# 1812598631/Amos-slam

Measured on AMD Instinct MI355X. Metric: front-end frames/sec (ORB extract+match+mask) at 640x480, higher is better.
Workload: dtype u8 (ORB, gate, matcher) + fp32 (mask network); 1 GPU; configs[2]: 640x480 L8 N1000 full front-end: YOLACT-R50 fp32 mask + ORB detect + gate + describe + match; lanes_per_gpu=2, frames_per_launch=64, width=640, height=480, n_features=1000, n_levels=8, ini_th_fast=20, min_th_fast=7, match=frame k vs k-1, N x N best-2, synthetic_stream_seed=stream = rank, frame k seeded 1000*rank+k (amos-slam_amd/synth.py), parallelism=frames sharded 1 ways, one process per GPU, no data-path collective

## Files before the change

amos-slam_amd/__init__.py:

```python
import ctypes as C
import os

import numpy as np

_HERE = os.path.dirname(os.path.abspath(__file__))
LIB_PATH = os.environ.get("AMOS_FRONTEND_LIB", os.path.join(_HERE, "csrc", "libamos_frontend.so"))

KP_DTYPE = np.dtype([("x", "<f4"), ("y", "<f4"), ("size", "<f4"), ("angle", "<f4"),
                     ("response", "<f4"), ("octave", "<i4"), ("class_id", "<i4")])
BEST2_DTYPE = np.dtype([("best_idx", "<i4"), ("best_dist", "<i4"), ("second_idx", "<i4"),
                        ("second_dist", "<i4")])

TH_HIGH, TH_LOW, HISTO_LENGTH = 100, 50, 30

_v, _i, _z, _f, _d, _q, _u = C.c_void_p, C.c_int, C.c_size_t, C.c_float, C.c_double, C.c_longlong, C.c_uint32
PROTOTYPES = {
    "amos_last_error": (C.c_char_p, ()),
    "amos_device_count": (_i, ()),
    "amos_current_device": (_i, ()),
    "amos_build_variant": (C.c_char_p, ()),
    "amos_orb_create": (_i, (_v, _i, _i, _i, _i, _v, _v)),
    "amos_orb_destroy": (None, (_v,)),
    "amos_orb_geometry_probe": (_i, (_v, _i, _i, _i, _i, _v, _v)),
    "amos_orb_tables": (_i, (_v, _v, _v, _v, _v, _v, _v)),
    "amos_orb_tables_host": (_i, (_v, _v, _v, _v, _v, _v, _v)),
    "amos_orb_level_sizes": (_i, (_v, _i, _i, _v, _v)),
    "amos_orb_detect": (_i, (_v, _v, _z, _i, _i)),
    "amos_orb_level_count": (_i, (_v, _i, _i)),
    "amos_orb_level_keypoints": (_i, (_v, _i, _i, _v, _i)),
    "amos_orb_set_level_keypoints": (_i, (_v, _i, _i, _v, _i)),
    "amos_orb_level_layout": (_i, (_v, _v, _v, _v)),
    "amos_orb_fetch_levels": (_i, (_v, _i, _v, _v, _i)),
    "amos_orb_store_levels": (_i, (_v, _i, _v, _v, _i)),
    "amos_orb_gate": (_i, (_v, _v, _z, _v, _z, _v, _i, _v, _i, _v, _i, _v)),
    "amos_orb_closed_mask": (_i, (_v, _v, _z)),
    "amos_orb_describe": (_i, (_v, _v, _v, _i, _v)),
    "amos_orb_extract": (_i, (_v, _v, _z, _i, _i, _v, _v, _i, _v)),
    "amos_orb_level_image": (_i, (_v, _i, _i, _v, _z, _i)),
    "amos_orb_pyramid_images": (_i, (_v, _i, _v, _v, _i)),
    "amos_orb_blurred_image": (_i, (_v, _i, _i, _v, _z)),
    "amos_orb_level_candidates": (_i, (_v, _i, _i, _v, _i)),
    "amos_orb_extract_batch_device": (_i, (_v, _v, _z, _z, _i, _i, _i)),
    "amos_orb_detect_batch_device": (_i, (_v, _v, _z, _z, _i, _i, _i)),
    "amos_orb_gate_batch_device": (_i, (_v, _v, _z, _z)),
    "amos_orb_gate_labels_batch_device": (_i, (_v, _v, _z, _z, _v, _z, _z, _v, _z, _i, _v, _z, _i, _v)),
    "amos_orb_describe_batch_device": (_i, (_v,)),
    "amos_orb_extract_batch_device_color": (_i, (_v, _v, _z, _z, _i, _i, _i, _i, _i)),
    "amos_frame_rgbd_glue_batch_device": (_i, (_v, _v, _i, _f, _z, _z, _f, _f, _f, _f, _f, _v, _v, _v, _v)),
    "amos_frame_stereo_match": (_i, (_v, _v, _f, _f, _v, _v, _i)),
    "amos_frame_stereo_match_batch_device": (_i, (_v, _v, _i, _f, _f, _v, _v, _v, _v)),
    "amos_frame_stereo_match_arrays_device": (_i, (_v, _v, _i, _v, _v, _v, _i, _v, _v, _v, _i, _f, _f, _v, _v, _v, _v)),
    "amos_frame_undistort_batch_device": (_i, (_v, _f, _f, _f, _f, _v, _i, _v)),
    "amos_frame_image_bounds": (_i, (_i, _i, _f, _f, _f, _f, _v, _i, _v)),
    "amos_orb_batch_results_device": (_i, (_v, _v, _v, _v, _v)),
    "amos_orb_batch_fetch": (_i, (_v, _i, _v, _v, _i, _v)),
    "amos_orb_sync": (_i, (_v,)),
    "amos_orb_timing_enable": (_i, (_v, _i)),
    "amos_orb_timing_collect": (_i, (_v, _v, _v)),
    "amos_orb_stream": (_v, (_v,)),
    "amos_match_create": (_i, (_i, _v, _v)),
    "amos_match_destroy": (None, (_v,)),
    "amos_match_sync": (_i, (_v,)),
    "amos_match_stream": (_v, (_v,)),
    "amos_match_distances": (_i, (_v, _v, _i, _v, _i, _v)),
    "amos_match_list_distances": (_i, (_v, _v, _i, _v, _i, _v, _v, _v)),
    "amos_match_list_best2": (_i, (_v, _v, _i, _v, _i, _v, _v, _i, _v)),
    "amos_match_bruteforce_best2": (_i, (_v, _v, _i, _v, _i, _i, _v)),
    "amos_match_set_bruteforce_kernel": (_i, (_v, _i)),
    "amos_match_bruteforce_best2_batch_device": (_i, (_v, _v, _z, _v, _v, _v, _i, _i, _i, _v)),
    "amos_frame_grid_build_batch_device": (_i, (_v, _v, _v, _i, _i, _v, _v)),
    "amos_match_window_best2_batch_device": (_i, (_v, _v, _v)),
    "amos_match_local_points_batch_device": (_i, (_v, _v)),
    "amos_match_local_points": (_i, (_v, _v, _v, _v, _i, _v, _i, _v, _v, _v, _i, _f, _f, _f, _f, _v, _v, _v, _v)),
    "amos_match_motion_model_batch_device": (_i, (_v, _v)),
    "amos_match_motion_model": (_i, (_v, _v, _v, _v, _i, _v, _i, _v, _v, _i, _f, _f, _f, _f, _v, _v, _v, _v)),
    "amos_bow_create": (_i, (_i, _v, _i, _i, _i, _i, _i, _v, _v, _v, _v, _v)),
    "amos_bow_destroy": (None, (_v,)),
    "amos_bow_sync": (_i, (_v,)),
    "amos_bow_stream": (_v, (_v,)),
    "amos_bow_check": (_i, (_i, _i, _i, _i, _i, _v, _v, _v)),
    "amos_bow_transform_batch_device": (_i, (_v, _v, _v, _i, _i, _i, _v, _v, _v, _v, _v, _v, _v, _v, _v, _v)),
    "amos_bow_transform": (_i, (_v, _v, _i, _i, _v, _v, _v, _v, _v, _v, _v, _v)),
    "amos_match_bow_batch_device": (_i, (_v, _v)),
    "amos_match_bow": (_i, (_v, _v, _v, _f, _i, _v, _v)),
    "amos_match_bow_kf_batch_device": (_i, (_v, _v, _f, _i)),
    "amos_match_triangulation_batch_device": (_i, (_v, _v, _v, _v, _v, _i, _i, _i)),
    "amos_match_bow_kf": (_i, (_v, _v, _v, _f, _i, _v, _v)),
    "amos_match_triangulation": (_i, (_v, _v, _v, _i, _v, _v, _v, _i, _i, _i, _v, _v)),
    "amos_match_fuse_batch_device": (_i, (_v, _v)),
    "amos_match_fuse": (_i, (_v, _v, _i, _v, _i, _i, _v, _v, _v, _v, _v, _v, _i, _v, _v, _i, _i, _i, _v, _v, _v, _v, _v)),
    "amos_mask_pre_create": (_i, (_i, _v, _i, _i, _i, _v)),
    "amos_mask_pre_destroy": (None, (_v,)),
    "amos_mask_pre_stream": (_v, (_v,)),
    "amos_mask_preprocess_batch_device": (_i, (_v, _v, _i, _v)),
    "amos_orb_detect_color_with_mask_pre_batch_device": (_i, (_v, _v, _v, _z, _z, _i, _i, _i, _i, _i, _v)),
    "amos_mask_bias_act_device": (_i, (_v, _v, _v, _v, _z, _i, _i)),
    "amos_mask_bias_relu_maxpool_device": (_i, (_v, _v, _v, _v, _i, _i, _i, _i)),
    "amos_mask_stem_weight_floats": (_i, ()),
    "amos_mask_stem_weights_device": (_i, (_v, _v, _q, _q, _q, _q, _v)),
    "amos_mask_stem_device": (_i, (_v, _v, _q, _q, _q, _q, _v, _v, _v, _i, _i, _i)),
    "amos_mask_conv_supported": (_i, (_i, _i, _i, _i, _i, _i)),
    "amos_mask_conv_device": (_i, (_v, _v, _v, _v, _v, _v, _i, _i, _i, _i, _i, _i, _i, _i, _i, _i)),
    "amos_mask_conv_workspace_bytes": (_z, (_i, _i, _i, _i, _i, _i, _i, _i, _i)),
    "amos_mask_conv_ws_device": (_i, (_v, _v, _v, _v, _v, _v, _i, _i, _i, _i, _i, _i, _i, _i, _i, _i, _v, _z)),
    "amos_mask_conv_tile_mode": (_i, (_i,)),
    "amos_mask_conv_kernel_name": (_i, (_i, _i, _i, _i, _i, _i, _i, _i, _i, _v, _i)),
    "amos_mask_conv_chain_supported": (_i, (_i, _i, _i, _i, _i, _i, _i)),
    "amos_mask_conv_chain_device": (_i, (_v, _v, _v, _v, _v, _v, _v, _v, _i, _i, _i, _i, _i, _i, _i)),
    "amos_mask_conv1x1_supported": (_i, (_i, _i, _i)),
    "amos_mask_winograd_supported": (_i, (_i, _i)),
    "amos_mask_winograd_weight_floats": (_z, (_i, _i)),
    "amos_mask_winograd_weights_device": (_i, (_v, _v, _v, _i, _i)),
    "amos_mask_winograd_conv_device": (_i, (_v, _v, _v, _v, _v, _v, _i, _i, _i, _i, _i, _i)),
    "amos_mask_winograd24_weight_floats": (_z, (_i, _i)),
    "amos_mask_winograd24_weights_device": (_i, (_v, _v, _v, _i, _i)),
    "amos_mask_winograd24_conv_device": (_i, (_v, _v, _v, _v, _v, _v, _i, _i, _i, _i, _i, _i)),
    "amos_mask_winograd24_conv_layout_device": (_i, (_v, _v, _v, _v, _v, _v, _i, _i, _i, _i, _i, _i, _i, _i)),
    "amos_mask_winograd24_persistent_mode": (_i, (_i,)),
    "amos_mask_winograd24_narrow_mode": (_i, (_i,)),
    "amos_mask_conv1x1_device": (_i, (_v, _v, _v, _v, _v, _v, _i, _i, _i, _i, _i, _i, _i)),
    "amos_mask_bilinear_nhwc_device": (_i, (_v, _v, _v, _i, _i, _i, _i, _i, _i, _f, _f)),
    "amos_mask_bilinear_nhwc_act_device": (_i, (_v, _v, _v, _i, _i, _i, _i, _i, _i, _f, _f, _i)),
    "amos_mask_bilinear_x2_mode": (_i, (_i,)),
    "amos_mask_nms_column_max_device": (_i, (_v, _v, _v, _i, _i)),
    "amos_mask_class_scores_device": (_i, (_v, _v, _v, _i, _i, _i, _f)),
    "amos_mask_person_mask_device": (_i, (_v, _v, _v, _v, _i, _i, _i, _i, _i, _i)),
    "amos_mask_head_outputs_device": (_i, (_v, _v, _v, _v, _v, _v, _i, _i, _i, _i, _i, _i, _i, _i)),
    "amos_mask_head_outputs_scores_device": (_i, (_v, _v, _v, _v, _v, _v, _v, _f, _i, _i, _i, _i, _i, _i, _i, _i)),
    "amos_mask_topk_rows_device": (_i, (_v, _v, _v, _v, _i, _i, _i)),
    "amos_mask_topk_rows_sparse_device": (_i, (_v, _v, _v, _v, _i, _i, _i, _f)),
    "amos_mask_post_workspace_bytes": (_z, (_i, _i, _i, _i, _i, _i)),
    "amos_mask_person_masks_device": (_i, (_v, _v, _v, _v, _v, _v, _i, _i, _i, _i, _i, _i, _i, _i, _v, _z, _v, _v)),
    "amos_mask_person_masks_scores_device": (_i, (_v, _v, _v, _v, _v, _v, _i, _i, _i, _i, _i, _i, _i, _i, _v, _z, _v, _v)),
    "amos_mask_coef_at_priors_device": (_i, (_v, _v, _v, _v, _v, _v, _i, _i, _v, _v, _v, _i, _i, _i, _i, _v)),
    "amos_mask_person_masks_at_priors_device": (_i, (_v, _v, _v, _v, _v, _v, _v, _v, _i, _i, _i, _v, _v, _v, _v, _i, _i, _i, _i, _i, _i, _i, _i, _v, _z, _v, _v)),
    "amos_mask_person_masks_scores_at_priors_device": (_i, (_v, _v, _v, _v, _v, _v, _v, _v, _i, _i, _i, _v, _v, _v, _v, _i, _i, _i, _i, _i, _i, _i, _i, _v, _z, _v, _v)),
    "amos_mask_candidates_bytes": (_z, (_i, _i, _i)),
    "amos_mask_candidates_reset_device": (_i, (_v, _v, _i, _i)),
    "amos_mask_head_candidates_device": (_i, (_v, _v, _v, _v, _v, _v, _f, _i, _i, _i, _i, _i, _i, _i, _i)),
    "amos_mask_topk_lists_device": (_i, (_v, _v, _v, _i, _v, _v, _i, _i)),
    "amos_mask_person_masks_candidates_device": (_i, (_v, _v, _v, _v, _v, _v, _i, _i, _i, _i, _i, _i, _i, _i, _v, _z, _v, _v)),
    "amos_mask_person_masks_candidates_at_priors_device": (_i, (_v, _v, _v, _v, _v, _v, _v, _v, _i, _i, _i, _v, _v, _v, _v, _i, _i, _i, _i, _i, _i, _i, _i, _v, _z, _v, _v)),
    "amos_slic_center_count": (_i, (_i, _i, _i, _v, _v)),
    "amos_slic_create": (_i, (_i, _v, _i, _i, _i, _v)),
    "amos_slic_destroy": (None, (_v,)),
    "amos_slic_stream": (_v, (_v,)),
    "amos_slic_run": (_i, (_v, _v, _v, _i, _i, _i, _i, _i, _v, _v, _v)),
    "amos_slic_batch_device": (_i, (_v, _v, _v, _i, _i, _i, _i, _i, _i, _v, _v)),
    "amos_cluster_bgr2lab_batch_device": (_i, (_v, _v, _z, _i, _v)),
    "amos_cluster_kmeans_batch_device": (_i, (_v, _v, _i, _i, _i, _u, _i, _v)),
    "amos_cluster_kmeans": (_i, (_v, _v, _i, _i, _u, _i, _v)),
    "amos_flow_check_device": (_i, (_v, _v, _z, _v, _z, _i, _i, _v, _v, _v, _i, _v)),
    "amos_flow_epipolar_device": (_i, (_v, _v, _v, _v, _v, _i, _v)),
    "amos_flow_scene_flow_device": (_i, (_v, _v, _z, _v, _z, _v, _v, _i, _v, _v)),
    "amos_flow_fundamental_score_device": (_i, (_v, _v, _i, _v, _v, _i, _d, _v, _v, _v)),
    "amos_flow_pnp_score_device": (_i, (_v, _v, _i, _v, _v, _i, _d, _d, _d, _d, _d, _v, _v, _v)),
    "amos_lk_create": (_i, (_i, _v, _i, _i, _i, _i, _v)),
    "amos_lk_destroy": (None, (_v,)),
    "amos_lk_stream": (_v, (_v,)),
    "amos_lk_levels": (_i, (_v,)),
    "amos_lk_track_device": (_i, (_v, _v, _z, _v, _z, _v, _i, _i, _d, _f, _v, _v, _v)),
    "amos_corners_create": (_i, (_i, _v, _i, _i, _v)),
    "amos_corners_destroy": (None, (_v,)),
    "amos_corners_stream": (_v, (_v,)),
    "amos_corners_good_features_device": (_i, (_v, _v, _z, _i, _i, _i, _d, _d, _d, _v, _i, _v, _v)),
    "amos_corners_candidate_count": (_i, (_v, _v)),
    "amos_corners_subpix_device": (_i, (_v, _v, _z, _i, _i, _v, _v, _i, _i, _i, _d)),
    "amos_fmat_create": (_i, (_i, _v, _i, _i, _v)),
    "amos_fmat_destroy": (None, (_v,)),
    "amos_fmat_stream": (_v, (_v,)),
    "amos_fmat_ransac_device": (_i, (_v, _i, _v, _v, _v, _v, _v, _d, _d, _i, _v, _v, _v)),
    "amos_fmat_scene_flow_pair_device": (_i, (_v, _v, _v, _v, _v, _v, _v, _v, _v)),
    "amos_fmat_ransac": (_i, (_v, _i, _v, _v, _d, _d, _i, _v, _v, _v)),
    "amos_pnp_create": (_i, (_i, _v, _i, _i, _v)),
    "amos_pnp_destroy": (None, (_v,)),
    "amos_pnp_stream": (_v, (_v,)),
    "amos_pnp_ransac_device": (_i, (_v, _i, _v, _v, _v, _v, _v, _d, _d, _d, _d, _d, _d, _i, _v, _v, _v)),
# ... 130 lines not shown
        n = _check(self.L.amos_orb_level_count(self.h, frame, level), "amos_orb_level_count")
        out = np.zeros(max(n, 1), KP_DTYPE)
        _check(self.L.amos_orb_level_keypoints(self.h, frame, level, _p(out), len(out)), "amos_orb_level_keypoints")
        return out[:n]

    def set_level_keypoints(self, level, kps, frame=0):
        kps = np.ascontiguousarray(kps, KP_DTYPE)
        _check(self.L.amos_orb_set_level_keypoints(self.h, frame, level, _p(kps), len(kps)), "amos_orb_set_level_keypoints")

    def level_candidates(self, level, frame=0, cap=1 << 20):
        out = np.zeros(cap, KP_DTYPE)
        n = _check(self.L.amos_orb_level_candidates(self.h, frame, level, _p(out), cap), "amos_orb_level_candidates")
        return out[:n].copy()

    def level_image(self, level, padded=False, frame=0):
        lw, lh = self.level_sizes(self.shape[1], self.shape[0])
        w, h = int(lw[level]), int(lh[level])
        if padded:
            w, h = w + 38, h + 38
        out = np.zeros((h, w), np.uint8)
        _check(self.L.amos_orb_level_image(self.h, frame, level, _p(out), w, int(padded)), "amos_orb_level_image")
        return out

    def blurred_image(self, level, frame=0):
        lw, lh = self.level_sizes(self.shape[1], self.shape[0])
        out = np.zeros((int(lh[level]), int(lw[level])), np.uint8)
        _check(self.L.amos_orb_blurred_image(self.h, frame, level, _p(out), out.shape[1]), "amos_orb_blurred_image")
        return out

    def gate(self, mask, labels=None, center_ids=None, rm_vector=None):
        mask = np.ascontiguousarray(mask, np.uint8)
        removed = np.zeros(self.capacity + 1, KP_DTYPE)
        nrem = C.c_int(0)
        if labels is not None:
            labels = np.ascontiguousarray(labels, np.float64)
            center_ids = np.ascontiguousarray(center_ids, np.int32)
            rm_vector = np.ascontiguousarray(rm_vector, np.int32)
            rc = self.L.amos_orb_gate(self.h, _p(mask), mask.strides[0], _p(labels), labels.shape[1], _p(center_ids), len(center_ids), _p(rm_vector), len(rm_vector),
                                      _p(removed), len(removed), C.byref(nrem))
        else:
            rc = self.L.amos_orb_gate(self.h, _p(mask), mask.strides[0], None, 0, None, 0, None, 0, _p(removed), len(removed), C.byref(nrem))
        _check(rc, "amos_orb_gate")
        return removed[:nrem.value].copy()

    def closed_mask(self):
        out = np.zeros(self.shape, np.uint8)
        _check(self.L.amos_orb_closed_mask(self.h, _p(out), out.shape[1]), "amos_orb_closed_mask")
        return out

    def describe(self):
        kps = np.zeros(self.capacity + 1, KP_DTYPE)
        desc = np.zeros((self.capacity + 1, 32), np.uint8)
        n = C.c_int(0)
        _check(self.L.amos_orb_describe(self.h, _p(kps), _p(desc), len(kps), C.byref(n)), "amos_orb_describe")
        return kps[:n.value].copy(), desc[:n.value].copy()

    def extract(self, gray):
        gray = np.ascontiguousarray(gray, np.uint8)
        h, w = gray.shape
        self.shape = (h, w)
        kps = np.zeros(self.capacity + 1, KP_DTYPE)
        desc = np.zeros((self.capacity + 1, 32), np.uint8)
        n = C.c_int(0)
        _check(self.L.amos_orb_extract(self.h, _p(gray), gray.strides[0], w, h, _p(kps), _p(desc), len(kps), C.byref(n)), "amos_orb_extract")
        return kps[:n.value].copy(), desc[:n.value].copy()

    def extract_batch_device(self, d_ptr, frame_stride, row_stride, width, height, n_frames):
        self.shape = (height, width)
        _check(self.L.amos_orb_extract_batch_device(self.h, d_ptr, frame_stride, row_stride, width, height, n_frames), "amos_orb_extract_batch_device")

    def detect_batch_device(self, d_ptr, frame_stride, row_stride, width, height, n_frames):
        self.shape = (height, width)
        _check(self.L.amos_orb_detect_batch_device(self.h, d_ptr, frame_stride, row_stride, width, height, n_frames), "amos_orb_detect_batch_device")

    def gate_batch_device(self, d_masks, mask_frame_stride, mask_row_stride):
        _check(self.L.amos_orb_gate_batch_device(self.h, d_masks, mask_frame_stride, mask_row_stride), "amos_orb_gate_batch_device")

    def gate_labels_batch_device(self, d_masks, mask_frame_stride, mask_row_stride, d_labels, label_frame_stride, label_row_stride, d_centers,
                                 centers_frame_stride, n_centers, d_rm, rm_frame_stride, n_rm, d_status):
        _check(self.L.amos_orb_gate_labels_batch_device(self.h, d_masks, mask_frame_stride, mask_row_stride, d_labels, label_frame_stride, label_row_stride,
                                                        d_centers, centers_frame_stride, n_centers, d_rm, rm_frame_stride, n_rm, d_status),
               "amos_orb_gate_labels_batch_device")

    def describe_batch_device(self):
        _check(self.L.amos_orb_describe_batch_device(self.h), "amos_orb_describe_batch_device")

    def extract_batch_device_color(self, d_ptr, frame_stride, row_stride, width, height, n_frames, channels=3, rgb_order=False):
        self.shape = (height, width)
        _check(self.L.amos_orb_extract_batch_device_color(self.h, d_ptr, frame_stride, row_stride, width, height, n_frames, channels, int(rgb_order)),
               "amos_orb_extract_batch_device_color")

    def detect_color_with_mask_pre_batch_device(self, pre, d_ptr, frame_stride, row_stride, width, height, n_frames, d_net_input, channels=3,
                                                rgb_order=False):
        self.shape = (height, width)
        _check(self.L.amos_orb_detect_color_with_mask_pre_batch_device(self.h, pre.h, d_ptr, frame_stride, row_stride, width, height, n_frames, channels,
                                                                       int(rgb_order), d_net_input), "amos_orb_detect_color_with_mask_pre_batch_device")

    def rgbd_glue_batch_device(self, d_depth, depth_is_u16, depth_map_factor, depth_frame_stride, depth_row_stride, mbf, bounds,
                               d_u_right, d_depth_out, d_grid_cell, d_kps_un=None):
        _check(self.L.amos_frame_rgbd_glue_batch_device(self.h, d_depth, int(depth_is_u16), depth_map_factor, depth_frame_stride, depth_row_stride, mbf, bounds[0],
                                                        bounds[1], bounds[2], bounds[3], d_kps_un, d_u_right, d_depth_out, d_grid_cell),
               "amos_frame_rgbd_glue_batch_device")

    def stereo_match_batch_device(self, right, n_pairs, mbf, min_z, d_u_right, d_depth, d_sad=None, d_status=None):
        r = self if right is None else right
        _check(self.L.amos_frame_stereo_match_batch_device(self.h, r.h, n_pairs, mbf, min_z, d_u_right, d_depth, d_sad, d_status),
               "amos_frame_stereo_match_batch_device")

    def stereo_match(self, right, mbf, min_z, n):
        r = self if right is None else right
        ur, dep = np.zeros(max(n, 1), np.float32), np.zeros(max(n, 1), np.float32)
        _check(self.L.amos_frame_stereo_match(self.h, r.h, mbf, min_z, _p(ur), _p(dep), n), "amos_frame_stereo_match")
        return ur[:n], dep[:n]

    def stereo_match_arrays_device(self, right, n_pairs, d_kps_l, d_desc_l, d_counts_l, capacity_l, d_kps_r, d_desc_r, d_counts_r, capacity_r, mbf, min_z,
                                   d_u_right, d_depth, d_sad=None, d_status=None):
        r = self if right is None else right
        _check(self.L.amos_frame_stereo_match_arrays_device(self.h, r.h, n_pairs, d_kps_l, d_desc_l, d_counts_l, capacity_l, d_kps_r, d_desc_r, d_counts_r,
                                                            capacity_r, mbf, min_z, d_u_right, d_depth, d_sad, d_status),
               "amos_frame_stereo_match_arrays_device")

    def undistort_batch_device(self, fx, fy, cx, cy, dist_coef, d_kps_un):
        dc = np.ascontiguousarray(dist_coef, np.float32)
        _check(self.L.amos_frame_undistort_batch_device(self.h, fx, fy, cx, cy, _p(dc), len(dc), d_kps_un), "amos_frame_undistort_batch_device")

    def batch_results_device(self):
        kps, desc, cnt, cap = C.c_void_p(), C.c_void_p(), C.c_void_p(), C.c_int(0)
        _check(self.L.amos_orb_batch_results_device(self.h, C.byref(kps), C.byref(desc), C.byref(cnt), C.byref(cap)), "amos_orb_batch_results_device")
        return kps.value, desc.value, cnt.value, cap.value

    def batch_fetch(self, frame):
        kps = np.zeros(self.capacity + 1, KP_DTYPE)
        desc = np.zeros((self.capacity + 1, 32), np.uint8)
        n = C.c_int(0)
        _check(self.L.amos_orb_batch_fetch(self.h, frame, _p(kps), _p(desc), len(kps), C.byref(n)), "amos_orb_batch_fetch")
        return kps[:n.value].copy(), desc[:n.value].copy()

    def sync(self):
        _check(self.L.amos_orb_sync(self.h), "amos_orb_sync")

    def pyramid_launches(self):
        return self.n_levels - 1

    STAGES = ("import", "pyramid", "fast", "octree", "orient", "blur", "describe")

    def timing_enable(self, max_records):
        _check(self.L.amos_orb_timing_enable(self.h, max_records), "amos_orb_timing_enable")

    def timing_collect(self):
        ms = np.zeros(len(self.STAGES), np.float32)
        n = C.c_int(0)
        _check(self.L.amos_orb_timing_collect(self.h, _p(ms), C.byref(n)), "amos_orb_timing_collect")
        return dict(zip(self.STAGES, ms.tolist())), n.value


SLIC_CENTER_DTYPE = np.dtype([("x", "<i4"), ("y", "<i4"), ("L", "<i4"), ("A", "<i4"), ("B", "<i4"), ("D", "<i4"), ("label", "<i4"), ("id", "<i4")])


class Slic(_Handle):

    _kind = "slic"

    def __init__(self, max_width=640, max_height=480, max_batch=1, device=0, stream=None):
        self._open(device, stream, max_width, max_height, max_batch)

    @staticmethod
    def center_count(width, height, length=5):
        nx, ny = C.c_int(0), C.c_int(0)
        n = lib().amos_slic_center_count(width, height, length, C.byref(nx), C.byref(ny))
        return n, nx.value, ny.value

    def run(self, lab, depth, length=5, m=10, iterations=5):
        lab = np.ascontiguousarray(lab, np.uint8)
        depth = np.ascontiguousarray(depth, np.uint16)
        h, w = depth.shape
        assert lab.shape == (h, w, 3)
        n = self.center_count(w, h, length)[0]
        labels = np.zeros((h, w), np.float64)
        centers = np.zeros(max(n, 1), SLIC_CENTER_DTYPE)
        nc = C.c_int(0)
        _check(self.L.amos_slic_run(self.h, _p(lab), _p(depth), w, h, length, m, iterations, _p(labels), _p(centers), C.byref(nc)), "amos_slic_run")
        return labels, centers[:nc.value]

    def run_batch_device(self, d_lab, d_depth, width, height, n_frames, d_labels, d_centers, length=5, m=10, iterations=5):
        _check(self.L.amos_slic_batch_device(self.h, d_lab, d_depth, width, height, n_frames, length, m, iterations, d_labels, d_centers), "amos_slic_batch_device")

    def bgr2lab_batch_device(self, d_bgr, n_pixels, d_lab, rgb_order=False):
        _check(self.L.amos_cluster_bgr2lab_batch_device(self.h, d_bgr, n_pixels, int(rgb_order), d_lab), "amos_cluster_bgr2lab_batch_device")

    def kmeans(self, centers, k=15, seed=1, max_iter=1000):
        c = np.ascontiguousarray(centers, SLIC_CENTER_DTYPE).copy()
        passes = C.c_int(0)
        _check(self.L.amos_cluster_kmeans(self.h, _p(c), len(c), k, seed, max_iter, C.byref(passes)), "amos_cluster_kmeans")
        return c, passes.value

    def kmeans_batch_device(self, d_centers, n_centers, n_frames, k=15, seed=1, max_iter=1000, d_passes=None):
        _check(self.L.amos_cluster_kmeans_batch_device(self.h, d_centers, n_centers, n_frames, k, seed, max_iter, d_passes), "amos_cluster_kmeans_batch_device")

    def sync(self):
        import torch
        torch.cuda.ExternalStream(self.stream).synchronize()


class MaskPreprocessor(_Handle):

    _kind = "mask_pre"

    def __init__(self, width=640, height=480, max_batch=16, device=0, stream=None):
        self._open(device, stream, width, height, max_batch)
        self.max_batch, self.shape = max_batch, (height, width)

    def run(self, d_bgr, n_frames, d_out):
        _check(self.L.amos_mask_preprocess_batch_device(self.h, d_bgr, n_frames, d_out), "amos_mask_preprocess_batch_device")


def mask_bias_act(stream_ptr, y_ptr, bias_ptr, residual_ptr, n, channels, relu):
    _check(lib().amos_mask_bias_act_device(stream_ptr, y_ptr, bias_ptr, residual_ptr, n, channels, int(relu)), "amos_mask_bias_act_device")


class SceneFlowCamera(C.Structure):
    _fields_ = [("cx", C.c_float), ("cy", C.c_float), ("invfx", C.c_float), ("invfy", C.c_float), ("Tlw", C.c_float * 12), ("Rwc", C.c_float * 9),
                ("Ow", C.c_float * 3)]


def flow_check(stream, d_last, last_stride, d_cur, cur_stride, cols, rows, d_pre, d_next, d_state_in, n, d_state_out):
    _check(lib().amos_flow_check_device(stream, d_last, last_stride, d_cur, cur_stride, cols, rows, d_pre, d_next, d_state_in, n, d_state_out),
           "amos_flow_check_device")


def flow_epipolar(stream, d_F, d_pre, d_next, d_state, n, d_dd):
    _check(lib().amos_flow_epipolar_device(stream, d_F, d_pre, d_next, d_state, n, d_dd), "amos_flow_epipolar_device")


def flow_scene_flow(stream, d_depth_last, last_stride, d_depth_cur, cur_stride, d_match_pre, d_match_cur, n, cam, d_out):
    _check(lib().amos_flow_scene_flow_device(stream, d_depth_last, last_stride, d_depth_cur, cur_stride, d_match_pre, d_match_cur, n, C.byref(cam), d_out),
           "amos_flow_scene_flow_device")


def flow_fundamental_score(stream, d_F, n_hyp, d_p1, d_p2, n, threshold, d_err, d_inliers, d_mask):
    _check(lib().amos_flow_fundamental_score_device(stream, d_F, n_hyp, d_p1, d_p2, n, threshold, d_err, d_inliers, d_mask), "amos_flow_fundamental_score_device")


def flow_pnp_score(stream, d_Rt, n_hyp, d_obj, d_img, n, fx, fy, cx, cy, reprojection_error, d_err, d_inliers, d_mask):
    _check(lib().amos_flow_pnp_score_device(stream, d_Rt, n_hyp, d_obj, d_img, n, fx, fy, cx, cy, reprojection_error, d_err, d_inliers, d_mask),
           "amos_flow_pnp_score_device")


def mask_bias_relu_maxpool(stream_ptr, x_ptr, bias_ptr, y_ptr, n, in_h, in_w, channels):
    _check(lib().amos_mask_bias_relu_maxpool_device(stream_ptr, x_ptr, bias_ptr, y_ptr, n, in_h, in_w, channels), "amos_mask_bias_relu_maxpool_device")


def mask_stem_weight_floats():
    return int(lib().amos_mask_stem_weight_floats())


def mask_stem_weights(stream_ptr, w_ptr, w_strides, packed_ptr):
    sn, sc, sy, sx = (int(v) for v in w_strides)
    _check(lib().amos_mask_stem_weights_device(stream_ptr, w_ptr, sn, sc, sy, sx, packed_ptr), "amos_mask_stem_weights_device")


def mask_stem(stream_ptr, x_ptr, x_strides, packed_ptr, bias_ptr, y_ptr, batch, height, width):
    sb, sc, sy, sx = (int(v) for v in x_strides)
    _check(lib().amos_mask_stem_device(stream_ptr, x_ptr, sb, sc, sy, sx, packed_ptr, bias_ptr, y_ptr, batch, height, width), "amos_mask_stem_device")


def mask_bilinear_x2_mode(mode=-1):
    return int(lib().amos_mask_bilinear_x2_mode(mode))


def mask_conv1x1_supported(cin, cout, stride):
    return lib().amos_mask_conv1x1_supported(cin, cout, stride) == 0


def mask_conv1x1(stream_ptr, x_ptr, w_ptr, bias_ptr, residual_ptr, y_ptr, batch, in_h, in_w, cin, cout, stride, relu):
    _check(lib().amos_mask_conv1x1_device(stream_ptr, x_ptr, w_ptr, bias_ptr, residual_ptr, y_ptr, batch, in_h, in_w, cin, cout, stride, int(relu)),
           "amos_mask_conv1x1_device")


def mask_conv_supported(cin, cout, kh, kw, stride, pad):
    return lib().amos_mask_conv_supported(cin, cout, kh, kw, stride, pad) == 0


def mask_winograd_supported(cin, cout):
    return lib().amos_mask_winograd_supported(cin, cout) == 0


def mask_winograd_weights(stream_ptr, w_ptr, u_ptr, cin, cout):
    _check(lib().amos_mask_winograd_weights_device(stream_ptr, w_ptr, u_ptr, cin, cout), "amos_mask_winograd_weights_device")


def mask_winograd_conv(stream_ptr, x_ptr, u_ptr, bias_ptr, residual_ptr, y_ptr, batch, h, w, cin, cout, relu):
    _check(lib().amos_mask_winograd_conv_device(stream_ptr, x_ptr, u_ptr, bias_ptr, residual_ptr, y_ptr, batch, h, w, cin, cout, int(relu)),
           "amos_mask_winograd_conv_device")


def mask_winograd24_weights(stream_ptr, w_ptr, u_ptr, cin, cout):
    _check(lib().amos_mask_winograd24_weights_device(stream_ptr, w_ptr, u_ptr, cin, cout), "amos_mask_winograd24_weights_device")


def mask_winograd24_conv(stream_ptr, x_ptr, u_ptr, bias_ptr, residual_ptr, y_ptr, batch, h, w, cin, cout, relu):
    _check(lib().amos_mask_winograd24_conv_device(stream_ptr, x_ptr, u_ptr, bias_ptr, residual_ptr, y_ptr, batch, h, w, cin, cout, int(relu)),
           "amos_mask_winograd24_conv_device")


def mask_winograd24_conv_layout(stream_ptr, x_ptr, u_ptr, bias_ptr, residual_ptr, y_ptr, batch, h, w, cin, cout, relu, in_blocked, out_blocked):
    _check(lib().amos_mask_winograd24_conv_layout_device(stream_ptr, x_ptr, u_ptr, bias_ptr, residual_ptr, y_ptr, batch, h, w, cin, cout, int(relu), int(in_blocked),
                                                         int(out_blocked)), "amos_mask_winograd24_conv_layout_device")


def mask_winograd24_persistent_mode(mode=-2):
    return int(lib().amos_mask_winograd24_persistent_mode(mode))


def mask_winograd24_narrow_mode(mode=-2):
    return int(lib().amos_mask_winograd24_narrow_mode(mode))


def mask_conv_tile_mode(mode=-2):
    return int(lib().amos_mask_conv_tile_mode(mode))


def mask_conv_kernel_name(batch, in_h, in_w, cin, cout, kh, kw, stride, pad):
    buf = C.create_string_buffer(96)
    _check(lib().amos_mask_conv_kernel_name(batch, in_h, in_w, cin, cout, kh, kw, stride, pad, buf, 96), "amos_mask_conv_kernel_name")
    return buf.value.decode()


def mask_conv(stream_ptr, x_ptr, w_ptr, bias_ptr, residual_ptr, y_ptr, batch, in_h, in_w, cin, cout, kh, kw, stride, pad, relu):
    _check(lib().amos_mask_conv_device(stream_ptr, x_ptr, w_ptr, bias_ptr, residual_ptr, y_ptr, batch, in_h, in_w, cin, cout, kh, kw, stride, pad, int(relu)),
           "amos_mask_conv_device")


def mask_conv_chain_supported(batch, in_h, in_w, cin, planes, cout, stride):
    return lib().amos_mask_conv_chain_supported(batch, in_h, in_w, cin, planes, cout, stride) == 0


def mask_conv_chain(stream_ptr, x_ptr, wd_ptr, bd_ptr, yc_ptr, w3_ptr, b3_ptr, y_ptr, batch, in_h, in_w, cin, planes, cout, stride):
    _check(lib().amos_mask_conv_chain_device(stream_ptr, x_ptr, wd_ptr, bd_ptr, yc_ptr, w3_ptr, b3_ptr, y_ptr, batch, in_h, in_w, cin, planes, cout, stride),
           "amos_mask_conv_chain_device")


def mask_conv_workspace_bytes(batch, in_h, in_w, cin, cout, kh, kw, stride, pad):
    return int(lib().amos_mask_conv_workspace_bytes(batch, in_h, in_w, cin, cout, kh, kw, stride, pad))


def mask_conv_ws(stream_ptr, x_ptr, w_ptr, bias_ptr, residual_ptr, y_ptr, batch, in_h, in_w, cin, cout, kh, kw, stride, pad, relu, workspace_ptr, workspace_bytes):
# ... 695 lines not shown
```

amos-slam_amd/csrc/amos_common.h:

```cpp
#pragma once
#include <hip/hip_runtime.h>
#include <stdint.h>
#include <stdio.h>
#include <atomic>
#include <string>

#include "../../include/amos_frontend.h"

namespace amos {

void set_error(const char *fmt, ...);

#define AMOS_HIP_CHECK(expr)                                                                   \
    do {                                                                                       \
        hipError_t _e = (expr);                                                                \
        if (_e != hipSuccess) {                                                                \
            amos::set_error("%s failed: %s (%s:%d)", #expr, hipGetErrorString(_e), __FILE__,   \
                            __LINE__);                                                         \
            (void)hipGetLastError();  \
            return AMOS_ERR_DEVICE;                                                            \
        }                                                                                      \
    } while (0)

struct DeviceOnce {
// ... 61 lines not shown
    int w, h;
    int stride;
    int planeOff;
    int maxBX, maxBY;
    int nCols, nRows, wCell, hCell;
    int cellStart, nCells;
    int ptsOff, ptsCap;
    int quota;
    int nIni;
    int nodeCap;
    int kpOff;
    int tabX, tabY;
    int blurGroups, blurItemStart;
    float scale;
    float patchSize;
};

struct Geom {
    int nLevels;
    int W, H;
    int totalCells;
    int slotTotal;
    int ptsTotal;
    int kpLevelTotal;
    int kpCap;
    int iniTh, minTh;
    int blurItems;
    int fastTileStrideDw, fastTileRows, fastMapRows, fastKeptCap, fastWaveBytes;
    unsigned long long frameBytes;
    LevelGeom lv[AMOS_MAX_LEVELS];
};

struct Cell {
    short level;
    short x0, y0;
    short tw, th;
    short ndw;
    int slotOff;
    unsigned magicDw, magicG;
    short groups;
    short pad[3];
};

struct ResizeTap {
    short ofs;
    short ofs1;
    short a0, a1;
};

constexpr int kMaskMidW = 480, kMaskMidH = 640;
struct FixTap { int s0, s1, a0, a1; };
struct MaskPreStageA {
    const FixTap *tx, *ty;
    const int *firstX, *firstY;
    const float *lut;
    float *mid;
    int width, height, maxBatch;
};

}

struct amos_mask_pre;
namespace amos {
struct OrbStereoView {
    int device;
    hipStream_t stream;
    hipEvent_t event;
    amos_orb_params p;
    int width, height, nFrames;
    bool detected, described;
    const Geom *dGeom;
    const uint8_t *dPyr;
    unsigned long long frameBytes;
    const amos_keypoint *dKps;
    const uint8_t *dDesc;
    const int *dCounts;
    int capacity;
    const float *scale, *invScale;
    int *dSadScratch;
    float *dOutHostForm;
    uint8_t *hStage;
};
int orb_stereo_view(amos_orb *h, size_t sadScratchInts, OrbStereoView *out);
int mask_pre_stage_a(amos_mask_pre *p, MaskPreStageA *out);
int mask_pre_finish(amos_mask_pre *p, hipStream_t stream, int n_frames, float *d_out);
const char *w24_variant_tag();
}
```

amos-slam_amd/csrc/amos_mask_pre.hip:

```cpp
#include "amos_common.h"

#include <cmath>
#include <vector>

namespace amos {

constexpr int kNetSize = 550;
constexpr int kMidW = kMaskMidW, kMidH = kMaskMidH;
constexpr int kBackW = 640, kBackH = 480;

struct FltTap { int s0, s1; float f0, f1; };

__global__ __launch_bounds__(256) void k_mask_pre_a(const uint8_t *__restrict__ bgr, int srcW, int srcH, const FixTap *__restrict__ tx,
                                                   const FixTap *__restrict__ ty, const float *__restrict__ lut, float *__restrict__ mid)
{
    const int p = blockIdx.x * 256 + threadIdx.x, frame = blockIdx.y;
    if (p >= kMidW * kMidH) return;
    const int y = p / kMidW, x = p - y * kMidW;
    const FixTap ax = tx[x], ay = ty[y];
    const uint8_t *r0 = bgr + ((size_t)frame * srcH + ay.s0) * srcW * 3, *r1 = bgr + ((size_t)frame * srcH + ay.s1) * srcW * 3;
    float *o = mid + ((size_t)frame * kMidH * kMidW + p) * 3;
#pragma unroll
    for (int c = 0; c < 3; c++) {
        const int h0 = r0[ax.s0 * 3 + c] * ax.a0 + r0[ax.s1 * 3 + c] * ax.a1;
        const int h1 = r1[ax.s0 * 3 + c] * ax.a0 + r1[ax.s1 * 3 + c] * ax.a1;
        const int v = (((ay.a0 * (h0 >> 4)) >> 16) + ((ay.a1 * (h1 >> 4)) >> 16) + 2) >> 2;
        o[c] = lut[v];
    }
}

__global__ __launch_bounds__(256) void k_mask_pre_b(const float *__restrict__ mid, const FltTap *__restrict__ tx, const FltTap *__restrict__ ty,
                                                   float *__restrict__ back)
{
    const int p = blockIdx.x * 256 + threadIdx.x, frame = blockIdx.y;
    if (p >= kBackW * kBackH) return;
    const int y = p / kBackW, x = p - y * kBackW;
    const FltTap ax = tx[x], ay = ty[y];
    const float *r0 = mid + ((size_t)frame * kMidH + ay.s0) * kMidW * 3, *r1 = mid + ((size_t)frame * kMidH + ay.s1) * kMidW * 3;
    float *o = back + ((size_t)frame * kBackH * kBackW + p) * 3;
#pragma unroll
    for (int c = 0; c < 3; c++) {
        const float h0 = __fadd_rn(__fmul_rn(r0[ax.s0 * 3 + c], ax.f0), __fmul_rn(r0[ax.s1 * 3 + c], ax.f1));
        const float h1 = __fadd_rn(__fmul_rn(r1[ax.s0 * 3 + c], ax.f0), __fmul_rn(r1[ax.s1 * 3 + c], ax.f1));
        o[c] = __fadd_rn(__fmul_rn(h0, ay.f0), __fmul_rn(h1, ay.f1));
    }
}

__global__ __launch_bounds__(256) void k_mask_pre_c(const float *__restrict__ back, float *__restrict__ out)
{
    const int p = blockIdx.x * 256 + threadIdx.x, frame = blockIdx.y;
    if (p >= kNetSize * kNetSize) return;
    const int oy = p / kNetSize, ox = p - oy * kNetSize;
    const float sh = (float)kBackH / (float)kNetSize, sw = (float)kBackW / (float)kNetSize;
    const float hr = fmaxf(__fsub_rn(__fmul_rn(sh, __fadd_rn((float)oy, 0.5f)), 0.5f), 0.f);
    const float wr = fmaxf(__fsub_rn(__fmul_rn(sw, __fadd_rn((float)ox, 0.5f)), 0.5f), 0.f);
    const int h1 = (int)hr, w1 = (int)wr;
    const int h1p = h1 < kBackH - 1 ? 1 : 0, w1p = w1 < kBackW - 1 ? 1 : 0;
    const float hl1 = __fsub_rn(hr, (float)h1), hl0 = __fsub_rn(1.f, hl1);
    const float wl1 = __fsub_rn(wr, (float)w1), wl0 = __fsub_rn(1.f, wl1);
    const float *b = back + (size_t)frame * kBackH * kBackW * 3;
    const float *p00 = b + ((size_t)h1 * kBackW + w1) * 3, *p01 = p00 + w1p * 3, *p10 = p00 + (size_t)h1p * kBackW * 3, *p11 = p10 + w1p * 3;
    const float mean[3] = {103.94f, 116.78f, 123.68f}, stdv[3] = {57.38f, 57.12f, 58.40f};
    float *o = out + (size_t)frame * 3 * kNetSize * kNetSize + p;
#pragma unroll
    for (int c = 0; c < 3; c++) {
        const float top = __fadd_rn(__fmul_rn(wl0, p00[c]), __fmul_rn(wl1, p01[c]));
        const float bot = __fadd_rn(__fmul_rn(wl0, p10[c]), __fmul_rn(wl1, p11[c]));
        const float v = __fadd_rn(__fmul_rn(hl0, top), __fmul_rn(hl1, bot));
        o[(size_t)(2 - c) * kNetSize * kNetSize] = __fdiv_rn(__fsub_rn(v, mean[c]), stdv[c]);
    }
}


template <bool kVec, bool kPow2>
__global__ __launch_bounds__(256) void k_bias_act(float *__restrict__ y, const float *__restrict__ bias, const float *__restrict__ res, size_t n,
                                                 int channels, int relu)
{
    const size_t i = ((size_t)blockIdx.x * 256 + threadIdx.x) * 4;
    if (i >= n) return;
    if (kVec) {
        const unsigned c = kPow2 ? ((unsigned)i & (unsigned)(channels - 1)) : (unsigned)(i % (size_t)channels);
        float4 v = *reinterpret_cast<const float4 *>(y + i);
        const float4 b = *reinterpret_cast<const float4 *>(bias + c);
        v.x = __fadd_rn(v.x, b.x); v.y = __fadd_rn(v.y, b.y); v.z = __fadd_rn(v.z, b.z); v.w = __fadd_rn(v.w, b.w);
        if (res) {
            const float4 r = *reinterpret_cast<const float4 *>(res + i);
            v.x = __fadd_rn(v.x, r.x); v.y = __fadd_rn(v.y, r.y); v.z = __fadd_rn(v.z, r.z); v.w = __fadd_rn(v.w, r.w);
        }
        if (relu) { v.x = fmaxf(v.x, 0.f); v.y = fmaxf(v.y, 0.f); v.z = fmaxf(v.z, 0.f); v.w = fmaxf(v.w, 0.f); }
        *reinterpret_cast<float4 *>(y + i) = v;
    } else {
        for (size_t k = i; k < n && k < i + 4; k++) {
            float v = __fadd_rn(y[k], bias[k % (size_t)channels]);
            if (res) v = __fadd_rn(v, res[k]);
            y[k] = relu ? fmaxf(v, 0.f) : v;
        }
    }
}

template <bool kRelu>
__global__ __launch_bounds__(256) void k_bilinear_nhwc_x2(const float *__restrict__ x, float *__restrict__ y, int inH, int inW, int outH, int outW, int c4,
                                                         float scaleH, float scaleW)
{
    const int t = blockIdx.x * 256 + threadIdx.x, bw = (outW + 1) / 2, bh = (outH + 1) / 2, perRow = bw * c4;
    if (t >= bh * perRow) return;
    const int by = t / perRow, tr = t - by * perRow;
    const int bx = tr / c4, q = tr - bx * c4, n = blockIdx.z;
    int yy[2][2], xx[2][2];
    float wy[2][2], wx[2][2];
#pragma unroll
    for (int e = 0; e < 2; e++) {
        float fy = __fsub_rn(__fmul_rn(scaleH, __fadd_rn((float)(2 * by + e), 0.5f)), 0.5f);
        float fx = __fsub_rn(__fmul_rn(scaleW, __fadd_rn((float)(2 * bx + e), 0.5f)), 0.5f);
        fy = fy < 0.f ? 0.f : fy;
        fx = fx < 0.f ? 0.f : fx;
        yy[e][0] = min((int)fy, inH - 1);
        xx[e][0] = min((int)fx, inW - 1);
        yy[e][1] = yy[e][0] + (yy[e][0] < inH - 1 ? 1 : 0);
        xx[e][1] = xx[e][0] + (xx[e][0] < inW - 1 ? 1 : 0);
        wy[e][1] = __fsub_rn(fy, (float)(int)fy); wy[e][0] = __fsub_rn(1.f, wy[e][1]);
        wx[e][1] = __fsub_rn(fx, (float)(int)fx); wx[e][0] = __fsub_rn(1.f, wx[e][1]);
    }
    const float4 *src = reinterpret_cast<const float4 *>(x) + (size_t)n * inH * inW * c4;
    auto at = [&](int r, int c) { return src[((size_t)r * inW + c) * c4 + q]; };
    float4 s[4][4];
    const bool shareY = yy[1][0] == yy[0][1], shareX = xx[1][0] == xx[0][1];
    const int ry[4] = {yy[0][0], yy[0][1], yy[1][0], yy[1][1]}, cx[4] = {xx[0][0], xx[0][1], xx[1][0], xx[1][1]};
#pragma unroll
    for (int r = 0; r < 4; r++) {
        if (r == 2 && shareY) {
#pragma unroll
            for (int c = 0; c < 4; c++) s[2][c] = s[1][c];
            continue;
        }
#pragma unroll
        for (int c = 0; c < 4; c++) {
            if (c == 2 && shareX) s[r][2] = s[r][1];
            else s[r][c] = at(ry[r], cx[c]);
        }
    }
    float4 *dst = reinterpret_cast<float4 *>(y);
#pragma unroll
    for (int ey = 0; ey < 2; ey++)
#pragma unroll
        for (int ex = 0; ex < 2; ex++) {
            const int oy = 2 * by + ey, ox = 2 * bx + ex;
            if (oy >= outH || ox >= outW) continue;
            const float hy = wy[ey][0], ly = wy[ey][1], hx = wx[ex][0], lx = wx[ex][1];
            const float4 a = s[2 * ey][2 * ex], b = s[2 * ey][2 * ex + 1], c = s[2 * ey + 1][2 * ex], d = s[2 * ey + 1][2 * ex + 1];
            auto mix = [&](float p, float r, float u, float v2) {
                const float v = __fadd_rn(__fmul_rn(hy, __fadd_rn(__fmul_rn(hx, p), __fmul_rn(lx, r))), __fmul_rn(ly, __fadd_rn(__fmul_rn(hx, u), __fmul_rn(lx, v2))));
                return kRelu ? (v < 0.f ? 0.f : v) : v;
// ... 29 lines not shown
    float4 r = {fmaxf(__fadd_rn(m.x, b.x), 0.f), fmaxf(__fadd_rn(m.y, b.y), 0.f), fmaxf(__fadd_rn(m.z, b.z), 0.f), fmaxf(__fadd_rn(m.w, b.w), 0.f)};
    if (nan) {
        float *rp = &r.x;
        for (int e = 0; e < 4; e++) {
            bool cn = false;
            for (int dy = -1; dy <= 1; dy++)
                for (int dx = -1; dx <= 1; dx++) {
                    const int iy = 2 * oy + dy, ix = 2 * ox + dx;
                    if ((unsigned)iy < (unsigned)inH && (unsigned)ix < (unsigned)inW) {
                        const float v = (&src[((size_t)iy * inW + ix) * c4 + q].x)[e];
                        cn = cn || v != v;
                    }
                }
            if (cn) rp[e] = __builtin_nanf("");
        }
    }
    reinterpret_cast<float4 *>(y)[(((size_t)n * outH + oy) * outW + ox) * c4 + q] = r;
}

template <bool kRelu>
__global__ __launch_bounds__(256) void k_bilinear_nhwc(const float *__restrict__ x, float *__restrict__ y, int inH, int inW, int outH, int outW, int c4,
                                                      float scaleH, float scaleW)
{
    const int t = blockIdx.x * 256 + threadIdx.x;
    if (t >= outW * c4) return;
    const int ox = t / c4, q = t - ox * c4, oy = blockIdx.y, n = blockIdx.z;
    float fy = __fsub_rn(__fmul_rn(scaleH, __fadd_rn((float)oy, 0.5f)), 0.5f), fx = __fsub_rn(__fmul_rn(scaleW, __fadd_rn((float)ox, 0.5f)), 0.5f);
    fy = fy < 0.f ? 0.f : fy;
    fx = fx < 0.f ? 0.f : fx;
    const int y0 = (int)fy, x0 = (int)fx;
    const int y1 = y0 + (y0 < inH - 1 ? 1 : 0), x1 = x0 + (x0 < inW - 1 ? 1 : 0);
    const float ly = __fsub_rn(fy, (float)y0), lx = __fsub_rn(fx, (float)x0), hy = __fsub_rn(1.f, ly), hx = __fsub_rn(1.f, lx);
    const float4 *src = reinterpret_cast<const float4 *>(x) + (size_t)n * inH * inW * c4;
    const float4 a = src[((size_t)y0 * inW + x0) * c4 + q], b = src[((size_t)y0 * inW + x1) * c4 + q];
    const float4 c = src[((size_t)y1 * inW + x0) * c4 + q], d = src[((size_t)y1 * inW + x1) * c4 + q];
    auto mix = [&](float p, float r, float s, float u) {
        const float v = __fadd_rn(__fmul_rn(hy, __fadd_rn(__fmul_rn(hx, p), __fmul_rn(lx, r))), __fmul_rn(ly, __fadd_rn(__fmul_rn(hx, s), __fmul_rn(lx, u))));
        return kRelu ? (v < 0.f ? 0.f : v) : v;
    };
    reinterpret_cast<float4 *>(y)[(((size_t)n * outH + oy) * outW + ox) * c4 + q] =
        make_float4(mix(a.x, b.x, c.x, d.x), mix(a.y, b.y, c.y, d.y), mix(a.z, b.z, c.z, d.z), mix(a.w, b.w, c.w, d.w));
}

__global__ __launch_bounds__(256) void k_nms_column_max(const float4 *__restrict__ boxes, float *__restrict__ out, int k)
{
    __shared__ float4 sb[256];
    __shared__ float sarea[256];
    const int j = threadIdx.x;
    const float4 *b = boxes + (size_t)blockIdx.x * k;
    float4 me = {0.f, 0.f, 0.f, 0.f};
    float myArea = 0.f;
    if (j < k) {
        me = b[j];
        myArea = __fmul_rn(__fsub_rn(me.z, me.x), __fsub_rn(me.w, me.y));
        sb[j] = me;
        sarea[j] = myArea;
    }
    __syncthreads();
    if (j >= k) return;
    float best = 0.f;
    bool nan = false;
    for (int i = 0; i < j; i++) {
        const float4 o = sb[i];
        float w = __fsub_rn(fminf(o.z, me.z), fmaxf(o.x, me.x)), h = __fsub_rn(fminf(o.w, me.w), fmaxf(o.y, me.y));
        w = w < 0.f ? 0.f : w;
        h = h < 0.f ? 0.f : h;
        const float inter = __fmul_rn(w, h);
        const float uni = __fsub_rn(__fadd_rn(sarea[i], myArea), inter);
        const float iou = (float)((double)inter / (double)uni);
        nan = nan || iou != iou;
        best = iou > best ? iou : best;
    }
    out[(size_t)blockIdx.x * k + j] = nan ? __builtin_nanf("") : best;
}

}

using namespace amos;

struct amos_mask_pre : StreamHandle {
    int width = 0, height = 0, maxBatch = 0;
    FixTap *dFixX = nullptr, *dFixY = nullptr;
    FltTap *dFltX = nullptr, *dFltY = nullptr;
    float *dLut = nullptr, *dMid = nullptr, *dBack = nullptr;
    int *dFirstX = nullptr, *dFirstY = nullptr;
};

static void axis_taps(int srcN, int dstN, bool clampFraction, std::vector<int> &s0, std::vector<int> &s1, std::vector<float> &f)
{
    const double scale = 1.0 / ((double)dstN / (double)srcN);
    s0.resize(dstN); s1.resize(dstN); f.resize(dstN);
    for (int d = 0; d < dstN; d++) {
        float fx = (float)((d + 0.5) * scale - 0.5);
        int s = (int)std::floor(fx);
        fx -= (float)s;
        if (clampFraction) {
            if (s < 0) { fx = 0; s = 0; }
            if (s >= srcN - 1) { fx = 0; s = srcN - 1; }
        }
        s0[d] = std::min(std::max(s, 0), srcN - 1);
        s1[d] = std::min(std::max(s + 1, 0), srcN - 1);
        f[d] = fx;
    }
}

static int round_even(float v) { return (int)std::nearbyintf(v); }

namespace amos {
int mask_pre_stage_a(amos_mask_pre *p, MaskPreStageA *out)
{
    if (!p || !out) { set_error("mask pre-processing handle missing"); return AMOS_ERR_INVALID; }
    *out = MaskPreStageA{p->dFixX, p->dFixY, p->dFirstX, p->dFirstY, p->dLut, p->dMid, p->width, p->height, p->maxBatch};
    return AMOS_OK;
}
int mask_pre_finish(amos_mask_pre *p, hipStream_t stream, int n_frames, float *d_out)
{
    hipLaunchKernelGGL(k_mask_pre_b, dim3((kBackW * kBackH + 255) / 256, n_frames), dim3(256), 0, stream, p->dMid, p->dFltX, p->dFltY, p->dBack);
    hipLaunchKernelGGL(k_mask_pre_c, dim3((kNetSize * kNetSize + 255) / 256, n_frames), dim3(256), 0, stream, p->dBack, d_out);
    AMOS_HIP_CHECK(hipGetLastError());
    return AMOS_OK;
}
}

extern "C" {

int amos_mask_pre_create(int device, void *stream, int width, int height, int max_batch, amos_mask_pre **out)
{
    if (!out || width < 2 || height < 2 || max_batch < 1) { set_error("amos_mask_pre_create: invalid argument"); return AMOS_ERR_INVALID; }
    amos_mask_pre *p = new amos_mask_pre();
    p->width = width; p->height = height; p->maxBatch = max_batch;
    const int rc = p->open(device, stream);
    if (rc != AMOS_OK) { delete p; return rc; }
    std::vector<int> s0, s1;
    std::vector<float> f;
    auto fix = [&](int srcN, int dstN, bool clamp, FixTap **dst, int **first) -> hipError_t {
        axis_taps(srcN, dstN, clamp, s0, s1, f);
        std::vector<FixTap> t(dstN);
        for (int d = 0; d < dstN; d++) t[d] = FixTap{s0[d], s1[d], round_even((1.f - f[d]) * 2048.f), round_even(f[d] * 2048.f)};
        std::vector<int> inv(srcN + 1);
        for (int X = 0, d = 0; X <= srcN; X++) {
            while (d < dstN && s0[d] < X) d++;
            inv[X] = d;
        }
        hipError_t e = hipMalloc((void **)dst, sizeof(FixTap) * dstN);
        if (e == hipSuccess) e = hipMemcpy(*dst, t.data(), sizeof(FixTap) * dstN, hipMemcpyHostToDevice);
        if (e == hipSuccess) e = hipMalloc((void **)first, sizeof(int) * inv.size());
        if (e == hipSuccess) e = hipMemcpy(*first, inv.data(), sizeof(int) * inv.size(), hipMemcpyHostToDevice);
        return e;
    };
    auto flt = [&](int srcN, int dstN, bool clamp, FltTap **dst) -> hipError_t {
        axis_taps(srcN, dstN, clamp, s0, s1, f);
        std::vector<FltTap> t(dstN);
        for (int d = 0; d < dstN; d++) t[d] = FltTap{s0[d], s1[d], 1.0f - f[d], f[d]};
        hipError_t e = hipMalloc((void **)dst, sizeof(FltTap) * dstN);
        if (e != hipSuccess) return e;
        return hipMemcpy(*dst, t.data(), sizeof(FltTap) * dstN, hipMemcpyHostToDevice);
    };
    float lut[256];
    for (int v = 0; v < 256; v++) lut[v] = (float)((double)v / 255.0) * 255.0f;
    hipError_t e = fix(width, kMidW, true, &p->dFixX, &p->dFirstX);
    if (e == hipSuccess) e = fix(height, kMidH, false, &p->dFixY, &p->dFirstY);
    if (e == hipSuccess) e = flt(kMidW, kBackW, true, &p->dFltX);
    if (e == hipSuccess) e = flt(kMidH, kBackH, false, &p->dFltY);
    if (e == hipSuccess) e = hipMalloc((void **)&p->dLut, sizeof(lut));
    if (e == hipSuccess) e = hipMemcpy(p->dLut, lut, sizeof(lut), hipMemcpyHostToDevice);
    if (e == hipSuccess) e = hipMalloc((void **)&p->dMid, sizeof(float) * 3 * kMidW * kMidH * (size_t)max_batch);
    if (e == hipSuccess) e = hipMalloc((void **)&p->dBack, sizeof(float) * 3 * kBackW * kBackH * (size_t)max_batch);
    if (e != hipSuccess) {
        set_error("amos_mask_pre_create: %s", hipGetErrorString(e));
        amos_mask_pre_destroy(p);
        return AMOS_ERR_DEVICE;
    }
    *out = p;
    return AMOS_OK;
}

void amos_mask_pre_destroy(amos_mask_pre *p)
{
    if (!p) return;
    p->close();
    void *ptrs[] = {p->dFixX, p->dFixY, p->dFltX, p->dFltY, p->dLut, p->dMid, p->dBack, p->dFirstX, p->dFirstY};
    for (void *q : ptrs) if (q) (void)hipFree(q);
    delete p;
}

void *amos_mask_pre_stream(amos_mask_pre *p) { return p ? (void *)p->stream : nullptr; }

int amos_mask_preprocess_batch_device(amos_mask_pre *p, const uint8_t *d_bgr, int n_frames, float *d_out)
{
    if (!p || !d_bgr || !d_out || n_frames < 1) { set_error("amos_mask_preprocess_batch_device: invalid argument"); return AMOS_ERR_INVALID; }
    if (n_frames > p->maxBatch) { set_error("amos_mask_preprocess_batch_device: %d frames, handle made for %d", n_frames, p->maxBatch); return AMOS_ERR_CAPACITY; }
    AMOS_HIP_CHECK(hipSetDevice(p->device));
    hipLaunchKernelGGL(k_mask_pre_a, dim3((kMidW * kMidH + 255) / 256, n_frames), dim3(256), 0, p->stream, d_bgr, p->width, p->height, p->dFixX,
                       p->dFixY, p->dLut, p->dMid);
    hipLaunchKernelGGL(k_mask_pre_b, dim3((kBackW * kBackH + 255) / 256, n_frames), dim3(256), 0, p->stream, p->dMid, p->dFltX, p->dFltY, p->dBack);
    hipLaunchKernelGGL(k_mask_pre_c, dim3((kNetSize * kNetSize + 255) / 256, n_frames), dim3(256), 0, p->stream, p->dBack, d_out);
    AMOS_HIP_CHECK(hipGetLastError());
    return AMOS_OK;
}


int amos_mask_bias_act_device(void *stream, float *d_y, const float *d_bias, const float *d_residual, size_t n, int channels, int relu)
{
    if (!d_y || !d_bias || channels < 1 || n % (size_t)channels != 0) { set_error("amos_mask_bias_act_device: invalid argument"); return AMOS_ERR_INVALID; }
    if (n == 0) return AMOS_OK;
    const bool vec = channels % 4 == 0 && ((uintptr_t)d_y | (uintptr_t)d_bias | (uintptr_t)d_residual) % 16 == 0;
    const dim3 grid((unsigned)((n / 4 + 256) / 256)), block(256);
    const bool pow2 = (channels & (channels - 1)) == 0;
    if (vec && pow2) hipLaunchKernelGGL((k_bias_act<true, true>), grid, block, 0, (hipStream_t)stream, d_y, d_bias, d_residual, n, channels, relu);
    else if (vec) hipLaunchKernelGGL((k_bias_act<true, false>), grid, block, 0, (hipStream_t)stream, d_y, d_bias, d_residual, n, channels, relu);
    else hipLaunchKernelGGL((k_bias_act<false, false>), grid, block, 0, (hipStream_t)stream, d_y, d_bias, d_residual, n, channels, relu);
    AMOS_HIP_CHECK(hipGetLastError());
    return AMOS_OK;
}


int amos_mask_bias_relu_maxpool_device(void *stream, const float *d_x, const float *d_bias, float *d_y, int n, int in_h, int in_w, int channels)
{
    if (!d_x || !d_bias || !d_y || n < 1 || in_h < 1 || in_w < 1 || channels < 4 || channels % 4 != 0 ||
        ((uintptr_t)d_x | (uintptr_t)d_y | (uintptr_t)d_bias) % 16 != 0 || n > 65535 || in_h > 2 * 65535) {
        set_error("amos_mask_bias_relu_maxpool_device: invalid argument (channels % 4 == 0, 16-byte aligned tensors)");
        return AMOS_ERR_INVALID;
    }
    const int oh = (in_h + 2 - 3) / 2 + 1, ow = (in_w + 2 - 3) / 2 + 1, c4 = channels / 4;
    hipLaunchKernelGGL(k_bias_relu_maxpool, dim3((ow * c4 + 255) / 256, oh, n), dim3(256), 0, (hipStream_t)stream, d_x, d_bias, d_y, in_h, in_w, oh, ow, c4);
    AMOS_HIP_CHECK(hipGetLastError());
    return AMOS_OK;
}


static std::atomic<int> g_bilinear_x2{1};
int amos_mask_bilinear_x2_mode(int mode)
{
    const int before = g_bilinear_x2.load();
    if (mode == 0 || mode == 1) g_bilinear_x2.store(mode);
    return before;
}

int amos_mask_bilinear_nhwc_act_device(void *stream, const float *d_x, float *d_y, int n, int in_h, int in_w, int out_h, int out_w, int channels,
                                       float scale_h, float scale_w, int relu)
{
    if (!d_x || !d_y || n < 1 || in_h < 1 || in_w < 1 || out_h < 1 || out_w < 1 || channels < 4 || channels % 4 != 0 ||
        ((uintptr_t)d_x | (uintptr_t)d_y) % 16 != 0 || out_h > 65535 || n > 65535) {
        set_error("amos_mask_bilinear_nhwc_device: invalid argument (channels % 4 == 0, 16-byte aligned tensors)");
        return AMOS_ERR_INVALID;
    }
    const int c4 = channels / 4;
    if (g_bilinear_x2 && out_h == 2 * in_h && out_w == 2 * in_w && scale_h == 0.5f && scale_w == 0.5f) {
        const dim3 grid2((unsigned)(((long long)((out_h + 1) / 2) * ((out_w + 1) / 2) * c4 + 255) / 256), 1, n);
        if (relu) hipLaunchKernelGGL(k_bilinear_nhwc_x2<true>, grid2, dim3(256), 0, (hipStream_t)stream, d_x, d_y, in_h, in_w, out_h, out_w, c4, scale_h, scale_w);
        else hipLaunchKernelGGL(k_bilinear_nhwc_x2<false>, grid2, dim3(256), 0, (hipStream_t)stream, d_x, d_y, in_h, in_w, out_h, out_w, c4, scale_h, scale_w);
        AMOS_HIP_CHECK(hipGetLastError());
        return AMOS_OK;
    }
    const dim3 grid((out_w * c4 + 255) / 256, out_h, n), block(256);
    if (relu) hipLaunchKernelGGL(k_bilinear_nhwc<true>, grid, block, 0, (hipStream_t)stream, d_x, d_y, in_h, in_w, out_h, out_w, c4, scale_h, scale_w);
    else hipLaunchKernelGGL(k_bilinear_nhwc<false>, grid, block, 0, (hipStream_t)stream, d_x, d_y, in_h, in_w, out_h, out_w, c4, scale_h, scale_w);
    AMOS_HIP_CHECK(hipGetLastError());
    return AMOS_OK;
}

int amos_mask_bilinear_nhwc_device(void *stream, const float *d_x, float *d_y, int n, int in_h, int in_w, int out_h, int out_w, int channels,
                                   float scale_h, float scale_w)
{
    return amos_mask_bilinear_nhwc_act_device(stream, d_x, d_y, n, in_h, in_w, out_h, out_w, channels, scale_h, scale_w, 0);
}

int amos_mask_nms_column_max_device(void *stream, const float *d_boxes, float *d_out, int n_lists, int k)
{
    if (!d_boxes || !d_out || n_lists < 0 || k < 1 || k > 256 || (uintptr_t)d_boxes % 16 != 0) {
        set_error("amos_mask_nms_column_max_device: invalid argument (1 <= k <= 256, 16-byte aligned boxes)");
        return AMOS_ERR_INVALID;
    }
    if (n_lists == 0) return AMOS_OK;
    hipLaunchKernelGGL(k_nms_column_max, dim3(n_lists), dim3(256), 0, (hipStream_t)stream, reinterpret_cast<const float4 *>(d_boxes), d_out, k);
// ... 6 lines not shown
```

amos-slam_amd/csrc/amos_orb.hip:

```cpp
#include "orb_kernels.h"

#include <cmath>
#include <cstdlib>
#include <cstdarg>
#include <cstring>
#include <vector>

#ifndef AMOS_FAST_LDS_PAD
#define AMOS_FAST_LDS_PAD 0
#endif
namespace amos {

static thread_local std::string g_error;

void set_error(const char *fmt, ...)
{
    char buf[512];
    va_list ap;
    va_start(ap, fmt);
    vsnprintf(buf, sizeof(buf), fmt, ap);
    va_end(ap);
    g_error = buf;
}

static inline int align_up(int v, int a) { return (v + a - 1) / a * a; }
static inline size_t align_up_sz(size_t v, size_t a) { return (v + a - 1) / a * a; }
static inline int cv_round(float v) { return (int)lrintf(v); }

constexpr int kTimingEvents = 9;

}

using namespace amos;

struct amos_orb : StreamHandle {
    amos_orb_params p{};
    int maxW = 0, maxH = 0, maxB = 0;
    hipStream_t streamB = nullptr;
    hipEvent_t evFork = nullptr, evJoin = nullptr, evBlur0 = nullptr, evBlur1 = nullptr;
    hipEvent_t evStereo = nullptr;
    bool blurDone = false;
    size_t octLdsAttr = 0;
    float scale[AMOS_MAX_LEVELS]{}, invScale[AMOS_MAX_LEVELS]{}, sigma2[AMOS_MAX_LEVELS]{}, invSigma2[AMOS_MAX_LEVELS]{};
    int quota[AMOS_MAX_LEVELS]{};
    int umax[16]{};
    Geom geom{};
    std::vector<Cell> cells;
    std::vector<ResizeTap> taps;
    int curW = 0, curH = 0;
    Geom capGeom{};
    size_t capCells = 0, capTaps = 0;
    int octNC = 0, octSC = 0;
    Geom *dGeom = nullptr;
    Cell *dCells = nullptr;
    ResizeTap *dTaps = nullptr;
    uint8_t *dPyr = nullptr, *dBlur = nullptr, *dInput = nullptr;
    int *dSlotCount = nullptr;
    uint32_t *dSlots = nullptr, *dPts = nullptr;
    uint16_t *dNodeOf = nullptr;
    uint8_t *dQuadOf = nullptr;
    int *dCandCount = nullptr, *dLvCount = nullptr, *dOutCount = nullptr;
    amos_keypoint *dLvKps = nullptr, *dOutKps = nullptr, *dRemoved = nullptr, *dScratchKps = nullptr;
    uint8_t *dOutDesc = nullptr;
    int *dStereoSad = nullptr;
    float *dStereoOut = nullptr;
    uint8_t *dMask = nullptr, *dMaskTmp = nullptr, *dMaskClosed = nullptr;
    uint8_t *hStage = nullptr;
    uint8_t *hPyrStage = nullptr;
    double *dLabels = nullptr;
    int *dCenterIds = nullptr, *dRm = nullptr, *dNRemoved = nullptr, *dErr = nullptr;
    int capCenters = 0, capRm = 0;
    int inputPitch = 0, maskPitch = 0;
    int nFrames = 0;
    std::vector<hipEvent_t> events;
    int maxRecords = 0, nRecords = 0;
    bool detected = false, described = false, gated = false;
};

static int build_tables(amos_orb *h)
{
    const int L = h->p.n_levels;
    h->scale[0] = 1.0f;
    h->sigma2[0] = 1.0f;
    for (int i = 1; i < L; i++) {
        h->scale[i] = h->scale[i - 1] * h->p.scale_factor;
        h->sigma2[i] = h->scale[i] * h->scale[i];
    }
    for (int i = 0; i < L; i++) {
        h->invScale[i] = 1.0f / h->scale[i];
        h->invSigma2[i] = 1.0f / h->sigma2[i];
    }
    const float factor = 1.0f / h->p.scale_factor;
    float nDesired = (float)h->p.n_features * (1.0f - factor) / (1.0f - (float)std::pow((double)factor, (double)L));
    int sum = 0;
    for (int l = 0; l < L - 1; l++) {
        h->quota[l] = cv_round(nDesired);
        sum += h->quota[l];
        nDesired *= factor;
    }
    h->quota[L - 1] = std::max(h->p.n_features - sum, 0);
    const int vmax = (int)std::floor(kHalfPatch * std::sqrt(2.f) / 2 + 1);
    const int vmin = (int)std::ceil(kHalfPatch * std::sqrt(2.f) / 2);
    const double hp2 = kHalfPatch * kHalfPatch;
    for (int v = 0; v <= vmax; ++v) h->umax[v] = (int)lrint(std::sqrt(hp2 - v * v));
    for (int v = kHalfPatch, v0 = 0; v >= vmin; --v) {
        while (h->umax[v0] == h->umax[v0 + 1]) ++v0;
        h->umax[v] = v0;
        ++v0;
    }
    return AMOS_OK;
}

static void build_taps(int srcN, int dstN, bool horizontal, ResizeTap *out)
{
    const double inv_scale = (double)dstN / srcN;
    const double scale = 1. / inv_scale;
    for (int d = 0; d < dstN; d++) {
        float f = (float)((d + 0.5) * scale - 0.5);
        int s = (int)std::floor(f);
        f -= s;
        int s0 = s, s1 = s + 1;
        if (horizontal) {
            if (s < 0) { f = 0; s = 0; }
            if (s >= srcN - 1) { f = 0; s = srcN - 1; }
            s0 = s;
            s1 = std::min(s + 1, srcN - 1);
        } else {
            s0 = std::min(std::max(s0, 0), srcN - 1);
            s1 = std::min(std::max(s1, 0), srcN - 1);
        }
        auto sat = [](float v) { int i = cv_round(v); return (short)std::min(std::max(i, -32768), 32767); };
        out[d].ofs = (short)s0;
        out[d].ofs1 = (short)s1;
        out[d].a0 = sat((1.f - f) * 2048);
        out[d].a1 = sat(f * 2048);
    }
}

static int build_geometry(const amos_orb *h, int W, int Hh, Geom &g, std::vector<Cell> *cells,
                          std::vector<ResizeTap> *taps)
{
    const int L = h->p.n_levels;
    std::memset(&g, 0, sizeof(g));
    g.nLevels = L;
    g.W = W;
    g.H = Hh;
    g.iniTh = h->p.ini_th_fast;
    g.minTh = h->p.min_th_fast;
    size_t off = 0;
    int cellIdx = 0, slotOff = 0, ptsOff = 0, kpOff = 0, tabOff = 0, blurOff = 0, maxTw = 1, maxTh = 1;
    if (cells) cells->clear();
    if (taps) taps->clear();
    for (int l = 0; l < L; l++) {
        LevelGeom &lg = g.lv[l];
        lg.w = cv_round((float)W * h->invScale[l]);
        lg.h = cv_round((float)Hh * h->invScale[l]);
        if (lg.w > 4000 || lg.h > 4000) { set_error("level %d too large (%dx%d)", l, lg.w, lg.h); return AMOS_ERR_INVALID; }
        lg.stride = align_up(kPadLeft + lg.w + kEdge, 128);
        lg.planeOff = (int)off;
// ... 98 lines not shown
    }
    g.fastTileStrideDw = fastStrideNeeded <= 16 ? 16 : 20;
    g.fastTileRows = maxTh + 6;
    g.fastMapRows = maxTh + 2;
    g.fastKeptCap = ((maxTw + 1) / 2) * ((maxTh + 1) / 2);
    g.fastWaveBytes = (int)align_up_sz(align_up_sz((size_t)g.fastTileRows * g.fastTileStrideDw * 4, 16) + (size_t)g.fastMapRows * kFastMapStride +
                                       fast_list_bytes(g.fastKeptCap) + AMOS_FAST_LDS_PAD, 16);
    return AMOS_OK;
}

static int compute_capacity(amos_orb *h)
{
    const int max_width = h->maxW, max_height = h->maxH;
    std::vector<Cell> cells;
    std::vector<ResizeTap> taps;
    int rc = build_geometry(h, max_width, max_height, h->capGeom, &cells, &taps);
    if (rc != AMOS_OK) return rc;
    {
        Geom &cg = h->capGeom;
        long long slots = 0, ncell = 0, kpl = 0;
        const int nIniMax = std::max(1, (int)std::lround((double)max_width / 48.0));
        for (int l = 0; l < cg.nLevels; l++) {
            const long long w = cg.lv[l].w, hh = cg.lv[l].h;
            slots += (w * hh * 27 + 99) / 100 + 64;
            ncell += (w / 30 + 2) * (hh / 30 + 2);
            kpl += std::max(cg.lv[l].quota, 4 * nIniMax) + 4;
        }
        cg.slotTotal = (int)std::max<long long>(cg.slotTotal, slots);
        cg.ptsTotal = (int)std::max<long long>(cg.ptsTotal, slots);
        cg.kpLevelTotal = (int)std::max<long long>(cg.kpLevelTotal, kpl);
        cg.kpCap = cg.kpLevelTotal;
        h->capCells = (size_t)std::max<long long>((long long)cells.size(), ncell) + 64;
        cg.totalCells = (int)h->capCells;
    }
    h->capTaps = taps.size() + 64 + 8 * (size_t)h->capGeom.nLevels;
    return AMOS_OK;
}

static bool geometry_fits(const amos_orb *h, const Geom &g, size_t nTaps)
{
    const Geom &c = h->capGeom;
    return g.frameBytes <= c.frameBytes && g.totalCells <= c.totalCells && (size_t)g.totalCells <= h->capCells && g.slotTotal <= c.slotTotal &&
           g.ptsTotal <= c.ptsTotal && g.kpLevelTotal <= c.kpLevelTotal && nTaps <= h->capTaps;
}

static int set_geometry(amos_orb *h, int W, int Hh)
{
    if (W == h->curW && Hh == h->curH) return AMOS_OK;
    if (W > h->maxW || Hh > h->maxH) { set_error("frame %dx%d exceeds the handle's %dx%d", W, Hh, h->maxW, h->maxH); return AMOS_ERR_CAPACITY; }
    Geom g;
    std::vector<Cell> cells;
    std::vector<ResizeTap> taps;
    int rc = build_geometry(h, W, Hh, g, &cells, &taps);
    if (rc != AMOS_OK) return rc;
    AMOS_HIP_CHECK(hipStreamSynchronize(h->streamB));
    const Geom &c = h->capGeom;
    if (!geometry_fits(h, g, taps.size())) {
        set_error("frame %dx%d needs more scratch than the handle's %dx%d allocation", W, Hh, h->maxW, h->maxH);
        return AMOS_ERR_CAPACITY;
    }
    int nc = 0, sc = 0;
    for (int l = 0; l < g.nLevels; l++) { nc = std::max(nc, g.lv[l].nodeCap); sc = std::max(sc, g.lv[l].nCells); }
    g.kpCap = c.kpCap;
    h->octNC = align_up(nc, 4);
    h->octSC = align_up(std::max(sc, h->octNC), 4);
    {
        const size_t lds = oct_lds_bytes(h->octNC, h->octSC);
        if (lds > 160 * 1024) { set_error("quad-tree needs %zu B of LDS for a %dx%d frame", lds, W, Hh); return AMOS_ERR_INVALID; }
        if (lds > 48 * 1024 && lds > h->octLdsAttr) {
            AMOS_HIP_CHECK(hipFuncSetAttribute(reinterpret_cast<const void *>(k_octree), hipFuncAttributeMaxDynamicSharedMemorySize, (int)lds));
            h->octLdsAttr = lds;
        }
    }
    h->geom = g;
    h->cells.swap(cells);
    h->taps.swap(taps);
    AMOS_HIP_CHECK(hipMemcpyAsync(h->dGeom, &h->geom, sizeof(Geom), hipMemcpyHostToDevice, h->stream));
    AMOS_HIP_CHECK(hipMemcpyAsync(h->dCells, h->cells.data(), sizeof(Cell) * h->cells.size(), hipMemcpyHostToDevice, h->stream));
    if (!h->taps.empty())
        AMOS_HIP_CHECK(hipMemcpyAsync(h->dTaps, h->taps.data(), sizeof(ResizeTap) * h->taps.size(), hipMemcpyHostToDevice, h->stream));
    AMOS_HIP_CHECK(hipStreamSynchronize(h->stream));
    h->curW = W;
    h->curH = Hh;
    h->detected = h->described = h->gated = false;
    return AMOS_OK;
}

static int launch_detect(amos_orb *h, const uint8_t *dSrc, size_t frameStride, size_t rowStride, int nFrames, int channels = 1, int rgbOrder = 0,
                         const MaskPreStageA *fuse = nullptr)
{
    const Geom &g = h->geom;
    hipEvent_t *ev = (h->maxRecords > 0 && h->nRecords < h->maxRecords) ? &h->events[(size_t)h->nRecords * (kTimingEvents)] : nullptr;
    if (h->blurDone) AMOS_HIP_CHECK(hipStreamWaitEvent(h->stream, h->evJoin, 0));
    if (ev) (void)hipEventRecord(ev[0], h->stream);
    for (int l = 0; l < g.nLevels; l++) {
        const LevelGeom &lg = g.lv[l];
        const int groups = (kPadLeft + lg.w + kEdge + 3) / 4;
        dim3 grid((groups + 63) / 64, (lg.h + 2 * kEdge + 4 * kPyrRows - 1) / (4 * kPyrRows), nFrames), block(64, 4);
        if (l == 0 && fuse)
            hipLaunchKernelGGL(k_import_color_mask, dim3((lg.w + kFuseTileW - 1) / kFuseTileW, (lg.h + kFuseTileH - 1) / kFuseTileH, nFrames), dim3(256), 0,
                               h->stream, dSrc, frameStride, rowStride, h->dPyr, h->dGeom, channels, rgbOrder, *fuse);
        else if (l == 0 && channels > 1)
            hipLaunchKernelGGL(k_pyramid_level0_color, grid, block, 0, h->stream, dSrc, frameStride, rowStride, h->dPyr, h->dGeom, channels, rgbOrder);
        else if (l == 0) {
            hipLaunchKernelGGL(k_pyramid_level0_wide, dim3((import_threads(lg.w, lg.h) + 255) / 256, 1, nFrames), dim3(256), 0, h->stream, dSrc,
                               frameStride, rowStride, h->dPyr, h->dGeom);
        }
        else if (h->p.scale_factor < 1.99f)
            hipLaunchKernelGGL(k_pyramid_level<true>, dim3(xcd_grid((int)(grid.x * grid.y), nFrames)), block, 0, h->stream, h->dPyr, h->dGeom, h->dTaps, l, nFrames);
        else
            hipLaunchKernelGGL(k_pyramid_level<false>, dim3(xcd_grid((int)(grid.x * grid.y), nFrames)), block, 0, h->stream, h->dPyr, h->dGeom, h->dTaps, l, nFrames);
        if (ev && l == 0) (void)hipEventRecord(ev[1], h->stream);
    }
    if (ev) (void)hipEventRecord(ev[2], h->stream);
    AMOS_HIP_CHECK(hipEventRecord(h->evFork, h->stream));
    AMOS_HIP_CHECK(hipStreamWaitEvent(h->streamB, h->evFork, 0));
    if (ev) (void)hipEventRecord(h->evBlur0, h->streamB);
    hipLaunchKernelGGL(k_blur, dim3(xcd_grid((g.blurItems + 255) / 256, nFrames)), dim3(256), 0, h->streamB, h->dPyr, h->dBlur, h->dGeom, nFrames);
    if (ev) (void)hipEventRecord(h->evBlur1, h->streamB);
    AMOS_HIP_CHECK(hipEventRecord(h->evJoin, h->streamB));
    h->blurDone = true;
    if (ev) (void)hipEventRecord(ev[3], h->stream);
    {
        const dim3 fgrid(xcd_grid((g.totalCells + kFastCellsPerGroup - 1) / kFastCellsPerGroup, nFrames)), fblock(64 * kFastCellsPerGroup);
        const size_t flds = kFastCellsPerGroup * (size_t)g.fastWaveBytes;
        if (g.fastTileStrideDw == 16)
            hipLaunchKernelGGL(k_fast_cells<16>, fgrid, fblock, flds, h->stream, h->dPyr, h->dGeom, h->dCells, h->dSlotCount, h->dSlots, nFrames);
        else
            hipLaunchKernelGGL(k_fast_cells<20>, fgrid, fblock, flds, h->stream, h->dPyr, h->dGeom, h->dCells, h->dSlotCount, h->dSlots, nFrames);
    }
    if (ev) (void)hipEventRecord(ev[4], h->stream);
    const size_t lds = oct_lds_bytes(h->octNC, h->octSC);
    hipLaunchKernelGGL(k_octree, dim3(nFrames * g.nLevels), dim3(256), lds, h->stream, h->dGeom, h->dCells, h->dSlotCount,
                       h->dSlots, h->dPts, h->dNodeOf, h->dQuadOf, h->dCandCount, h->dLvKps, h->dLvCount, h->octNC, h->octSC);
    if (ev) (void)hipEventRecord(ev[5], h->stream);
    hipLaunchKernelGGL(k_orient, dim3(xcd_grid((g.kpLevelTotal + 15) / 16, nFrames)), dim3(256), 0, h->stream, h->dPyr, h->dGeom,
                       h->dLvKps, h->dLvCount, nFrames);
    if (ev) (void)hipEventRecord(ev[6], h->stream);
    AMOS_HIP_CHECK(hipGetLastError());
    h->nFrames = nFrames;
    h->detected = true;
    h->described = h->gated = false;
    return AMOS_OK;
}

static int launch_describe(amos_orb *h, int nFrames)
{
    const Geom &g = h->geom;
    hipEvent_t *ev = (h->maxRecords > 0 && h->nRecords < h->maxRecords) ? &h->events[(size_t)h->nRecords * (kTimingEvents)] : nullptr;
    AMOS_HIP_CHECK(hipStreamWaitEvent(h->stream, h->evJoin, 0));
    if (ev) (void)hipEventRecord(ev[7], h->stream);
    hipLaunchKernelGGL(k_describe, dim3(xcd_grid((g.kpLevelTotal + kDescKps - 1) / kDescKps, nFrames)), dim3(kDescKps * 16), 0, h->stream, h->dBlur, h->dGeom,
                       h->dLvKps, h->dLvCount, h->dOutKps, h->dOutDesc, h->dOutCount, nFrames);
    if (ev) { (void)hipEventRecord(ev[8], h->stream); h->nRecords++; }
    AMOS_HIP_CHECK(hipGetLastError());
    h->described = true;
    return AMOS_OK;
}

static int fetch_frame(amos_orb *h, int frame, amos_keypoint *kps, uint8_t *desc, int cap, int *n)
{
    const size_t kc = (size_t)h->geom.kpCap, base = (size_t)frame * kc;
    uint8_t *st = h->hStage;
    int *stCount = reinterpret_cast<int *>(st);
    amos_keypoint *stKps = reinterpret_cast<amos_keypoint *>(st + 16);
    uint8_t *stDesc = st + 16 + kc * sizeof(amos_keypoint);
    AMOS_HIP_CHECK(hipMemcpyAsync(stCount, h->dOutCount + frame, sizeof(int), hipMemcpyDeviceToHost, h->stream));
    if (kps) AMOS_HIP_CHECK(hipMemcpyAsync(stKps, h->dOutKps + base, sizeof(amos_keypoint) * kc, hipMemcpyDeviceToHost, h->stream));
    if (desc) AMOS_HIP_CHECK(hipMemcpyAsync(stDesc, h->dOutDesc + base * 32, (size_t)32 * kc, hipMemcpyDeviceToHost, h->stream));
    AMOS_HIP_CHECK(hipStreamSynchronize(h->stream));
    const int count = *stCount;
    if (n) *n = count;
    if (count > cap) { set_error("result holds %d keypoints, caller capacity %d", count, cap); return AMOS_ERR_CAPACITY; }
    if (count > 0) {
        if (kps) std::memcpy(kps, stKps, sizeof(amos_keypoint) * count);
        if (desc) std::memcpy(desc, stDesc, (size_t)32 * count);
    }
    return AMOS_OK;
}

template <typename T>
static int dev_alloc(T **p, size_t count)
{
    AMOS_HIP_CHECK(hipMalloc((void **)p, std::max<size_t>(count, 1) * sizeof(T)));
    return AMOS_OK;
}

int amos::orb_stereo_view(amos_orb *h, size_t sadScratchInts, OrbStereoView *v)
{
    if (!h || !v) { set_error("orb_stereo_view: invalid argument"); return AMOS_ERR_INVALID; }
    if (sadScratchInts > (size_t)h->maxB * h->capGeom.kpCap) {
        set_error("stereo match without d_sad needs %zu ints of scratch, the handle holds %zu: pass d_sad", sadScratchInts, (size_t)h->maxB * h->capGeom.kpCap);
        return AMOS_ERR_CAPACITY;
    }
    v->device = h->device;
    v->stream = h->stream;
    v->event = h->evStereo;
    v->p = h->p;
    v->width = h->curW;
    v->height = h->curH;
    v->nFrames = h->nFrames;
    v->detected = h->detected;
    v->described = h->described;
    v->dGeom = h->dGeom;
    v->dPyr = h->dPyr;
    v->frameBytes = h->geom.frameBytes;
    v->dKps = h->dOutKps;
    v->dDesc = h->dOutDesc;
    v->dCounts = h->dOutCount;
    v->capacity = h->capGeom.kpCap;
    v->scale = h->scale;
    v->invScale = h->invScale;
    v->dSadScratch = h->dStereoSad;
    v->dOutHostForm = h->dStereoOut;
    v->hStage = h->hStage;
    return AMOS_OK;
}

extern "C" {

const char *amos_last_error(void) { return g_error.c_str(); }

int amos_device_count(void)
{
    int n = 0;
// ... 19 lines not shown
        tag = t.empty() ? "default" : t.substr(1);
    }
    return tag.c_str();
}

int amos_orb_tables_host(const amos_orb_params *params, float *scale_factor, float *inv_scale_factor, float *level_sigma2,
                         float *inv_level_sigma2, int32_t *features_per_level, int32_t *umax)
{
    if (!params || params->n_levels < 1 || params->n_levels > AMOS_MAX_LEVELS || params->n_features < 1 || !(params->scale_factor > 1.0f)) {
        set_error("amos_orb_tables_host: invalid argument");
        return AMOS_ERR_INVALID;
    }
    amos_orb h;
    h.p = *params;
    build_tables(&h);
    return amos_orb_tables(&h, scale_factor, inv_scale_factor, level_sigma2, inv_level_sigma2, features_per_level, umax);
}

int amos_orb_geometry_probe(const amos_orb_params *params, int max_width, int max_height, int width, int height, int32_t need[6], int32_t cap[6])
{
    if (!params || max_width < 1 || max_height < 1 || width < 1 || height < 1 || params->n_levels < 1 || params->n_levels > AMOS_MAX_LEVELS ||
        params->n_features < 1 || !(params->scale_factor > 1.0f) || !(params->scale_factor <= 2.0f)) {
        set_error("amos_orb_geometry_probe: invalid argument");
        return AMOS_ERR_INVALID;
    }
    amos_orb h;
    h.p = *params;
    h.maxW = max_width;
    h.maxH = max_height;
    build_tables(&h);
    int rc = compute_capacity(&h);
    if (rc != AMOS_OK) return rc;
    if (width > max_width || height > max_height) { set_error("frame %dx%d exceeds %dx%d", width, height, max_width, max_height); return AMOS_ERR_CAPACITY; }
    Geom g;
    std::vector<Cell> cells;
    std::vector<ResizeTap> taps;
    rc = build_geometry(&h, width, height, g, &cells, &taps);
    if (rc != AMOS_OK) return rc;
    const Geom &c = h.capGeom;
    const long long n[6] = {(long long)g.totalCells, g.slotTotal, g.ptsTotal, g.kpLevelTotal, (long long)taps.size(), (long long)(g.frameBytes >> 8)};
    const long long k[6] = {(long long)c.totalCells, c.slotTotal, c.ptsTotal, c.kpLevelTotal, (long long)h.capTaps, (long long)(c.frameBytes >> 8)};
    for (int i = 0; i < 6; i++) {
        if (need) need[i] = (int32_t)n[i];
        if (cap) cap[i] = (int32_t)k[i];
    }
    return geometry_fits(&h, g, taps.size()) ? AMOS_OK : AMOS_ERR_CAPACITY;
}

int amos_orb_create(const amos_orb_params *params, int max_width, int max_height, int max_batch, int device,
                    void *stream, amos_orb **out)
{
    if (!params || !out || max_width < 1 || max_height < 1 || max_batch < 1 || params->n_levels < 1 ||
        params->n_levels > AMOS_MAX_LEVELS || params->n_features < 1 || !(params->scale_factor > 1.0f) ||
        !(params->scale_factor <= 2.0f)) {
        set_error("amos_orb_create: invalid argument");
        return AMOS_ERR_INVALID;
    }
    amos_orb *h = new amos_orb();
    h->p = *params;
    h->maxW = max_width;
    h->maxH = max_height;
    h->maxB = max_batch;
    int rc = h->open(device, stream);
    if (rc != AMOS_OK) { delete h; return rc; }
    build_tables(h);
    static const int kUmax[16] = {15, 15, 15, 15, 14, 14, 14, 13, 13, 12, 11, 10, 9, 8, 6, 3};
    if (std::memcmp(kUmax, h->umax, sizeof(kUmax)) != 0) { set_error("umax table mismatch"); amos_orb_destroy(h); return AMOS_ERR_INVALID; }
    rc = compute_capacity(h);
    if (rc != AMOS_OK) { amos_orb_destroy(h); return rc; }
    const Geom &c = h->capGeom;
    if (hipStreamCreateWithFlags(&h->streamB, hipStreamNonBlocking) != hipSuccess ||
        hipEventCreateWithFlags(&h->evFork, hipEventDisableTiming) != hipSuccess ||
        hipEventCreateWithFlags(&h->evJoin, hipEventDisableTiming) != hipSuccess ||
        hipEventCreateWithFlags(&h->evStereo, hipEventDisableTiming) != hipSuccess || hipEventCreate(&h->evBlur0) != hipSuccess ||
        hipEventCreate(&h->evBlur1) != hipSuccess) {
        set_error("side stream / event creation failed");
        amos_orb_destroy(h);
        return AMOS_ERR_DEVICE;
    }
    const size_t B = (size_t)max_batch;
    const size_t slack = 4096;
    h->inputPitch = align_up(max_width, 128);
    h->maskPitch = align_up(max_width, 128);
#define ALLOC(ptr, count) do { rc = dev_alloc(&(ptr), (count)); if (rc != AMOS_OK) { amos_orb_destroy(h); return rc; } } while (0)
    ALLOC(h->dGeom, 1);
    ALLOC(h->dCells, h->capCells);
    ALLOC(h->dTaps, h->capTaps);
    ALLOC(h->dPyr, B * c.frameBytes + slack);
    ALLOC(h->dBlur, B * c.frameBytes + slack);
    ALLOC(h->dInput, (size_t)h->inputPitch * max_height);
    ALLOC(h->dSlotCount, B * c.totalCells);
    ALLOC(h->dSlots, B * c.slotTotal);
    ALLOC(h->dPts, B * c.ptsTotal);
    ALLOC(h->dNodeOf, B * c.ptsTotal);
    ALLOC(h->dQuadOf, B * c.ptsTotal);
    ALLOC(h->dCandCount, B * c.nLevels);
    ALLOC(h->dLvCount, B * c.nLevels);
    ALLOC(h->dOutCount, B);
    ALLOC(h->dLvKps, B * c.kpLevelTotal);
    ALLOC(h->dOutKps, B * c.kpCap);
    ALLOC(h->dOutDesc, B * c.kpCap * 32);
    ALLOC(h->dStereoSad, B * c.kpCap);
    ALLOC(h->dStereoOut, (size_t)2 * c.kpCap);
    ALLOC(h->dRemoved, B * c.kpLevelTotal);
    ALLOC(h->dScratchKps, (size_t)c.ptsTotal);
    ALLOC(h->dMask, (size_t)h->maskPitch * max_height);
    ALLOC(h->dMaskTmp, B * (size_t)h->maskPitch * max_height);
    ALLOC(h->dMaskClosed, B * (size_t)h->maskPitch * max_height);
    ALLOC(h->dLabels, (size_t)max_width * max_height);
    ALLOC(h->dNRemoved, B);
    ALLOC(h->dErr, 1);
#undef ALLOC
    if (hipHostMalloc((void **)&h->hStage, 16 + (size_t)c.kpCap * (sizeof(amos_keypoint) + 32), hipHostMallocDefault) != hipSuccess) {
        set_error("hipHostMalloc (result staging) failed");
        amos_orb_destroy(h);
        return AMOS_ERR_DEVICE;
    }
    (void)hipMemsetAsync(h->dPyr, 0, B * c.frameBytes + slack, h->stream);
    (void)hipMemsetAsync(h->dBlur, 0, B * c.frameBytes + slack, h->stream);
    (void)hipMemsetAsync(h->dLvCount, 0, sizeof(int) * B * c.nLevels, h->stream);
    (void)hipMemsetAsync(h->dOutCount, 0, sizeof(int) * B, h->stream);
    signed char pat[1024];
    std::memcpy(pat, amos_orb_pattern, 1024);
    int dx[31];
    {
        const int r = 15, cc = 15;
        const double inv_r2 = 1. / ((double)r * r);
        for (int i = 0; i < 31; i++) {
            const int dy = i - r;
            dx[i] = (int)lrint(cc * std::sqrt((r * r - dy * dy) * inv_r2));
        }
    }
    for (int i = 0; i < 31; i++)
        if (dx[i] != kMorphDx[std::abs(i - 15)]) { set_error("ellipse row %d: half-width %d, kernel expects %d", i, dx[i], kMorphDx[std::abs(i - 15)]); amos_orb_destroy(h); return AMOS_ERR_INVALID; }
    if (hipMemcpyToSymbol(HIP_SYMBOL(c_pattern), pat, sizeof(pat)) != hipSuccess ||
        hipMemcpyToSymbol(HIP_SYMBOL(c_umax), h->umax, sizeof(int) * 16) != hipSuccess ||
        hipMemcpyToSymbol(HIP_SYMBOL(c_ellipse_dx), dx, sizeof(dx)) != hipSuccess) {
        set_error("hipMemcpyToSymbol failed");
        amos_orb_destroy(h);
        return AMOS_ERR_DEVICE;
    }
    int maxNC = 0, maxSC = 0;
    for (int l = 0; l < c.nLevels; l++) { maxNC = std::max(maxNC, c.lv[l].nodeCap); maxSC = std::max(maxSC, c.lv[l].nCells); }
    const size_t maxLds = oct_lds_bytes(align_up(maxNC, 4), align_up(std::max(maxSC, maxNC), 4));
    if (maxLds > 160 * 1024) { set_error("quad-tree needs %zu B of LDS (n_features too large)", maxLds); amos_orb_destroy(h); return AMOS_ERR_INVALID; }
    if (maxLds > 48 * 1024) {
        hipError_t e = hipFuncSetAttribute(reinterpret_cast<const void *>(k_octree), hipFuncAttributeMaxDynamicSharedMemorySize, (int)maxLds);
        if (e != hipSuccess) { set_error("hipFuncSetAttribute: %s", hipGetErrorString(e)); amos_orb_destroy(h); return AMOS_ERR_DEVICE; }
        h->octLdsAttr = maxLds;
    }
    hipError_t e = hipStreamSynchronize(h->stream);
    if (e != hipSuccess) { set_error("create sync: %s", hipGetErrorString(e)); amos_orb_destroy(h); return AMOS_ERR_DEVICE; }
    *out = h;
    return AMOS_OK;
}

void amos_orb_destroy(amos_orb *h)
{
    if (!h) return;
    h->close();
    void *ptrs[] = {h->dGeom, h->dCells, h->dTaps, h->dPyr, h->dBlur, h->dInput, h->dSlotCount, h->dSlots, h->dPts,
                    h->dNodeOf, h->dQuadOf, h->dCandCount, h->dLvCount, h->dOutCount, h->dLvKps, h->dOutKps, h->dOutDesc,
                    h->dRemoved, h->dScratchKps, h->dMask, h->dMaskTmp, h->dMaskClosed, h->dLabels, h->dCenterIds, h->dRm,
                    h->dNRemoved, h->dErr, h->dStereoSad, h->dStereoOut};
    for (void *p : ptrs) if (p) (void)hipFree(p);
    if (h->hStage) (void)hipHostFree(h->hStage);
    if (h->hPyrStage) (void)hipHostFree(h->hPyrStage);
    for (hipEvent_t e : h->events) (void)hipEventDestroy(e);
    if (h->streamB) { (void)hipStreamSynchronize(h->streamB); (void)hipStreamDestroy(h->streamB); }
    for (hipEvent_t e : {h->evFork, h->evJoin, h->evBlur0, h->evBlur1, h->evStereo}) if (e) (void)hipEventDestroy(e);
    delete h;
}

int amos_orb_tables(const amos_orb *h, float *scale_factor, float *inv_scale_factor, float *level_sigma2,
                    float *inv_level_sigma2, int32_t *features_per_level, int32_t *umax)
{
    if (!h) return AMOS_ERR_INVALID;
    for (int i = 0; i < h->p.n_levels; i++) {
        if (scale_factor) scale_factor[i] = h->scale[i];
        if (inv_scale_factor) inv_scale_factor[i] = h->invScale[i];
        if (level_sigma2) level_sigma2[i] = h->sigma2[i];
        if (inv_level_sigma2) inv_level_sigma2[i] = h->invSigma2[i];
        if (features_per_level) features_per_level[i] = h->quota[i];
    }
    if (umax) for (int i = 0; i < 16; i++) umax[i] = h->umax[i];
    return AMOS_OK;
}

int amos_orb_level_sizes(const amos_orb *h, int width, int height, int32_t *level_w, int32_t *level_h)
{
    if (!h) return AMOS_ERR_INVALID;
    for (int l = 0; l < h->p.n_levels; l++) {
        if (level_w) level_w[l] = cv_round((float)width * h->invScale[l]);
        if (level_h) level_h[l] = cv_round((float)height * h->invScale[l]);
    }
    return h->p.n_levels;
}

int amos_orb_detect(amos_orb *h, const uint8_t *gray, size_t stride, int width, int height)
{
    if (!h || !gray || width < 1 || height < 1 || stride < (size_t)width) { set_error("amos_orb_detect: invalid argument"); return AMOS_ERR_INVALID; }
    AMOS_HIP_CHECK(hipSetDevice(h->device));
    int rc = set_geometry(h, width, height);
    if (rc != AMOS_OK) return rc;
    AMOS_HIP_CHECK(hipMemcpy2DAsync(h->dInput, h->inputPitch, gray, stride, width, height, hipMemcpyHostToDevice, h->stream));
    rc = launch_detect(h, h->dInput, 0, h->inputPitch, 1);
    if (rc != AMOS_OK) return rc;
    AMOS_HIP_CHECK(hipStreamSynchronize(h->stream));
    AMOS_HIP_CHECK(hipStreamSynchronize(h->streamB));
    return AMOS_OK;
}

int amos_orb_level_count(amos_orb *h, int frame, int level)
{
    if (!h || !h->detected || frame < 0 || frame >= h->nFrames || level < 0 || level >= h->geom.nLevels) { set_error("amos_orb_level_count: invalid argument or state"); return AMOS_ERR_INVALID; }
    int n = 0;
    AMOS_HIP_CHECK(hipMemcpyAsync(&n, h->dLvCount + frame * h->geom.nLevels + level, sizeof(int), hipMemcpyDeviceToHost, h->stream));
    AMOS_HIP_CHECK(hipStreamSynchronize(h->stream));
    return n;
}

int amos_orb_level_keypoints(amos_orb *h, int frame, int level, amos_keypoint *out, int cap)
{
    const int n = amos_orb_level_count(h, frame, level);
    if (n < 0) return n;
    if (n > cap || (!out && n > 0)) { set_error("level holds %d keypoints, caller capacity %d", n, cap); return AMOS_ERR_CAPACITY; }
    if (n > 0) {
        AMOS_HIP_CHECK(hipMemcpyAsync(out, h->dLvKps + (size_t)frame * h->geom.kpLevelTotal + h->geom.lv[level].kpOff,
                                      sizeof(amos_keypoint) * n, hipMemcpyDeviceToHost, h->stream));
        AMOS_HIP_CHECK(hipStreamSynchronize(h->stream));
    }
    return n;
}

int amos_orb_set_level_keypoints(amos_orb *h, int frame, int level, const amos_keypoint *kps, int n)
{
    if (!h || !h->detected || frame < 0 || frame >= h->nFrames || level < 0 || level >= h->geom.nLevels || n < 0 || (n > 0 && !kps)) {
        set_error("amos_orb_set_level_keypoints: invalid argument or state");
        return AMOS_ERR_INVALID;
    }
    if (n > h->geom.lv[level].nodeCap) { set_error("level %d list capacity %d < %d", level, h->geom.lv[level].nodeCap, n); return AMOS_ERR_CAPACITY; }
    if (n > 0)
        AMOS_HIP_CHECK(hipMemcpyAsync(h->dLvKps + (size_t)frame * h->geom.kpLevelTotal + h->geom.lv[level].kpOff, kps,
                                      sizeof(amos_keypoint) * n, hipMemcpyHostToDevice, h->stream));
    AMOS_HIP_CHECK(hipMemcpyAsync(h->dLvCount + frame * h->geom.nLevels + level, &n, sizeof(int), hipMemcpyHostToDevice, h->stream));
    AMOS_HIP_CHECK(hipStreamSynchronize(h->stream));
// ... 5 lines not shown
    if (!h || h->curW == 0) { set_error("amos_orb_level_layout: no frame geometry yet"); return AMOS_ERR_STATE; }
    for (int l = 0; l < h->geom.nLevels; l++) {
        if (offsets) offsets[l] = h->geom.lv[l].kpOff;
        if (caps) caps[l] = h->geom.lv[l].nodeCap;
    }
    if (total) *total = h->geom.kpLevelTotal;
    return AMOS_OK;
}

int amos_orb_fetch_levels(amos_orb *h, int frame, int32_t *counts, amos_keypoint *buf, int buf_len)
{
    if (!h || !h->detected || !counts || !buf || frame < 0 || frame >= h->nFrames) { set_error("amos_orb_fetch_levels: invalid argument or state"); return AMOS_ERR_INVALID; }
    if (buf_len < h->geom.kpLevelTotal) { set_error("amos_orb_fetch_levels: buffer holds %d keypoints, need %d", buf_len, h->geom.kpLevelTotal); return AMOS_ERR_CAPACITY; }
    AMOS_HIP_CHECK(hipMemcpyAsync(counts, h->dLvCount + frame * h->geom.nLevels, sizeof(int) * h->geom.nLevels, hipMemcpyDeviceToHost, h->stream));
    AMOS_HIP_CHECK(hipMemcpyAsync(buf, h->dLvKps + (size_t)frame * h->geom.kpLevelTotal, sizeof(amos_keypoint) * h->geom.kpLevelTotal,
                                  hipMemcpyDeviceToHost, h->stream));
    AMOS_HIP_CHECK(hipStreamSynchronize(h->stream));
    return AMOS_OK;
}

int amos_orb_store_levels(amos_orb *h, int frame, const int32_t *counts, const amos_keypoint *buf, int buf_len)
{
    if (!h || !h->detected || !counts || !buf || frame < 0 || frame >= h->nFrames) { set_error("amos_orb_store_levels: invalid argument or state"); return AMOS_ERR_INVALID; }
    if (buf_len < h->geom.kpLevelTotal) { set_error("amos_orb_store_levels: buffer holds %d keypoints, need %d", buf_len, h->geom.kpLevelTotal); return AMOS_ERR_CAPACITY; }
    for (int l = 0; l < h->geom.nLevels; l++)
        if (counts[l] < 0 || counts[l] > h->geom.lv[l].nodeCap) { set_error("level %d: %d keypoints exceed capacity %d", l, counts[l], h->geom.lv[l].nodeCap); return AMOS_ERR_CAPACITY; }
    AMOS_HIP_CHECK(hipMemcpyAsync(h->dLvCount + frame * h->geom.nLevels, counts, sizeof(int) * h->geom.nLevels, hipMemcpyHostToDevice, h->stream));
    AMOS_HIP_CHECK(hipMemcpyAsync(h->dLvKps + (size_t)frame * h->geom.kpLevelTotal, buf, sizeof(amos_keypoint) * h->geom.kpLevelTotal,
                                  hipMemcpyHostToDevice, h->stream));
    AMOS_HIP_CHECK(hipStreamSynchronize(h->stream));
    return AMOS_OK;
}

int amos_orb_level_candidates(amos_orb *h, int frame, int level, amos_keypoint *out, int cap)
{
    if (!h || !h->detected || frame < 0 || frame >= h->nFrames || level < 0 || level >= h->geom.nLevels) { set_error("amos_orb_level_candidates: invalid argument or state"); return AMOS_ERR_INVALID; }
    int n = 0;
    AMOS_HIP_CHECK(hipMemcpyAsync(&n, h->dCandCount + frame * h->geom.nLevels + level, sizeof(int), hipMemcpyDeviceToHost, h->stream));
    AMOS_HIP_CHECK(hipStreamSynchronize(h->stream));
    if (n > cap) { set_error("level holds %d candidates, caller capacity %d", n, cap); return AMOS_ERR_CAPACITY; }
    if (n > 0) {
        hipLaunchKernelGGL(k_unpack_candidates, dim3((n + 255) / 256), dim3(256), 0, h->stream,
                           h->dPts + (size_t)frame * h->geom.ptsTotal + h->geom.lv[level].ptsOff, n, h->dScratchKps);
        AMOS_HIP_CHECK(hipMemcpyAsync(out, h->dScratchKps, sizeof(amos_keypoint) * n, hipMemcpyDeviceToHost, h->stream));
        AMOS_HIP_CHECK(hipStreamSynchronize(h->stream));
    }
    return n;
}

int amos_orb_gate(amos_orb *h, const uint8_t *mask, size_t mask_stride, const double *labels, size_t lstride,
                  const int32_t *center_ids, int n_centers, const int32_t *rm_vector, int n_rm, amos_keypoint *removed,
                  int cap, int *n_removed)
{
    if (!h || !mask || !n_removed) { set_error("amos_orb_gate: invalid argument"); return AMOS_ERR_INVALID; }
    if (!h->detected) { set_error("amos_orb_gate before amos_orb_detect"); return AMOS_ERR_STATE; }
    if (labels && (!center_ids || !rm_vector || n_centers < 1 || n_rm < 1)) { set_error("amos_orb_gate: label gate needs center ids and rm_vector"); return AMOS_ERR_INVALID; }
    AMOS_HIP_CHECK(hipSetDevice(h->device));
    const Geom &g = h->geom;
    AMOS_HIP_CHECK(hipMemcpy2DAsync(h->dMask, h->maskPitch, mask, mask_stride, g.W, g.H, hipMemcpyHostToDevice, h->stream));
    if (labels) {
        AMOS_HIP_CHECK(hipMemcpy2DAsync(h->dLabels, sizeof(double) * g.W, labels, sizeof(double) * lstride, sizeof(double) * g.W, g.H,
                                        hipMemcpyHostToDevice, h->stream));
        if (n_centers > h->capCenters) {
            if (h->dCenterIds) (void)hipFree(h->dCenterIds);
            h->dCenterIds = nullptr;
            int rc = dev_alloc(&h->dCenterIds, n_centers);
            if (rc != AMOS_OK) return rc;
            h->capCenters = n_centers;
        }
        if (n_rm > h->capRm) {
            if (h->dRm) (void)hipFree(h->dRm);
            h->dRm = nullptr;
            int rc = dev_alloc(&h->dRm, n_rm);
            if (rc != AMOS_OK) return rc;
            h->capRm = n_rm;
        }
        AMOS_HIP_CHECK(hipMemcpyAsync(h->dCenterIds, center_ids, sizeof(int) * n_centers, hipMemcpyHostToDevice, h->stream));
        AMOS_HIP_CHECK(hipMemcpyAsync(h->dRm, rm_vector, sizeof(int) * n_rm, hipMemcpyHostToDevice, h->stream));
    }
    AMOS_HIP_CHECK(hipMemsetAsync(h->dErr, 0, sizeof(int), h->stream));
    dim3 grid((g.W + kMorphTileW - 1) / kMorphTileW, (g.H + kMorphTileH - 1) / kMorphTileH);
    hipLaunchKernelGGL(k_morph31<true>, grid, dim3(256), 0, h->stream, h->dMask, (size_t)0, h->maskPitch, h->dMaskTmp, (size_t)0, h->maskPitch, g.W, g.H);
    hipLaunchKernelGGL(k_morph31<false>, grid, dim3(256), 0, h->stream, h->dMaskTmp, (size_t)0, h->maskPitch, h->dMaskClosed, (size_t)0, h->maskPitch, g.W, g.H);
    hipLaunchKernelGGL(k_gate, dim3(1), dim3(256), 0, h->stream, h->dGeom, h->dLvKps, h->dLvCount, h->dMaskClosed, (size_t)0, h->maskPitch,
                       labels ? h->dLabels : nullptr, g.W, h->dCenterIds, n_centers, h->dRm, n_rm, h->dRemoved, h->dNRemoved, h->dErr);
    AMOS_HIP_CHECK(hipGetLastError());
    int nrem = 0, err = 0;
    AMOS_HIP_CHECK(hipMemcpyAsync(&nrem, h->dNRemoved, sizeof(int), hipMemcpyDeviceToHost, h->stream));
    AMOS_HIP_CHECK(hipMemcpyAsync(&err, h->dErr, sizeof(int), hipMemcpyDeviceToHost, h->stream));
    AMOS_HIP_CHECK(hipStreamSynchronize(h->stream));
    h->gated = true;
    if (err) { set_error("amos_orb_gate: %s", (err & 1) ? "keypoint outside the mask" : "label / cluster id out of range"); return AMOS_ERR_INVALID; }
    *n_removed = nrem;
    if (removed) {
        if (nrem > cap) { set_error("%d keypoints removed, caller capacity %d", nrem, cap); return AMOS_ERR_CAPACITY; }
        if (nrem > 0) {
            AMOS_HIP_CHECK(hipMemcpyAsync(removed, h->dRemoved, sizeof(amos_keypoint) * nrem, hipMemcpyDeviceToHost, h->stream));
            AMOS_HIP_CHECK(hipStreamSynchronize(h->stream));
        }
    }
    return AMOS_OK;
}

int amos_orb_closed_mask(amos_orb *h, uint8_t *dst, size_t dst_stride)
{
    if (!h || !dst || !h->gated) { set_error("amos_orb_closed_mask: no gate has run"); return AMOS_ERR_STATE; }
    AMOS_HIP_CHECK(hipMemcpy2DAsync(dst, dst_stride, h->dMaskClosed, h->maskPitch, h->geom.W, h->geom.H, hipMemcpyDeviceToHost, h->stream));
    AMOS_HIP_CHECK(hipStreamSynchronize(h->stream));
    return AMOS_OK;
}

int amos_orb_describe(amos_orb *h, amos_keypoint *kps, uint8_t *desc, int cap, int *n)
{
    if (!h || !n) { set_error("amos_orb_describe: invalid argument"); return AMOS_ERR_INVALID; }
    if (!h->detected) { set_error("amos_orb_describe before amos_orb_detect"); return AMOS_ERR_STATE; }
    AMOS_HIP_CHECK(hipSetDevice(h->device));
    int rc = launch_describe(h, 1);
    if (rc != AMOS_OK) return rc;
    return fetch_frame(h, 0, kps, desc, cap, n);
}

int amos_orb_extract(amos_orb *h, const uint8_t *gray, size_t stride, int width, int height, amos_keypoint *kps,
                     uint8_t *desc, int cap, int *n)
{
    if (!h || !gray || !n || width < 1 || height < 1 || stride < (size_t)width) { set_error("amos_orb_extract: invalid argument"); return AMOS_ERR_INVALID; }
    AMOS_HIP_CHECK(hipSetDevice(h->device));
    int rc = set_geometry(h, width, height);
    if (rc != AMOS_OK) return rc;
    AMOS_HIP_CHECK(hipMemcpy2DAsync(h->dInput, h->inputPitch, gray, stride, width, height, hipMemcpyHostToDevice, h->stream));
    rc = launch_detect(h, h->dInput, 0, h->inputPitch, 1);
    if (rc != AMOS_OK) return rc;
    rc = launch_describe(h, 1);
    if (rc != AMOS_OK) return rc;
    return fetch_frame(h, 0, kps, desc, cap, n);
}

static int pyr_stage(amos_orb *h)
{
    if (h->hPyrStage) return AMOS_OK;
    if (hipHostMalloc((void **)&h->hPyrStage, (size_t)h->capGeom.frameBytes + 4096, hipHostMallocDefault) != hipSuccess) {
        (void)hipGetLastError();
        set_error("hipHostMalloc (pyramid staging) failed");
        return AMOS_ERR_DEVICE;
    }
    return AMOS_OK;
}

static void cut_plane(const amos_orb *h, int level, const uint8_t *stagedPlane, uint8_t *dst, size_t dst_stride, int padded)
{
    const LevelGeom &lg = h->geom.lv[level];
    const uint8_t *origin = stagedPlane + (size_t)kEdge * lg.stride + kPadLeft;
    const int rows = padded ? lg.h + 2 * kEdge : lg.h, cols = padded ? lg.w + 2 * kEdge : lg.w;
    const uint8_t *src = padded ? origin - (size_t)kEdge * lg.stride - kEdge : origin;
    for (int y = 0; y < rows; y++) std::memcpy(dst + (size_t)y * dst_stride, src + (size_t)y * lg.stride, (size_t)cols);
}

static int copy_plane(amos_orb *h, const uint8_t *dBase, int frame, int level, uint8_t *dst, size_t dst_stride, int padded)
{
    const Geom &g = h->geom;
    const LevelGeom &lg = g.lv[level];
    int rc = pyr_stage(h);
    if (rc != AMOS_OK) return rc;
    const size_t bytes = (size_t)lg.stride * (lg.h + 2 * kEdge);
    AMOS_HIP_CHECK(hipMemcpyAsync(h->hPyrStage, dBase + (size_t)frame * g.frameBytes + lg.planeOff, bytes, hipMemcpyDeviceToHost, h->stream));
    AMOS_HIP_CHECK(hipStreamSynchronize(h->stream));
    cut_plane(h, level, h->hPyrStage, dst, dst_stride, padded);
    return AMOS_OK;
}

int amos_orb_pyramid_images(amos_orb *h, int frame, uint8_t *const *dst, const size_t *dst_strides, int padded)
{
    if (!h || !dst || !dst_strides || !h->detected || frame < 0 || frame >= h->nFrames) { set_error("amos_orb_pyramid_images: invalid argument or state"); return AMOS_ERR_INVALID; }
    AMOS_HIP_CHECK(hipSetDevice(h->device));
    const Geom &g = h->geom;
    int rc = pyr_stage(h);
    if (rc != AMOS_OK) return rc;
    AMOS_HIP_CHECK(hipMemcpyAsync(h->hPyrStage, h->dPyr + (size_t)frame * g.frameBytes, (size_t)g.frameBytes, hipMemcpyDeviceToHost, h->stream));
    AMOS_HIP_CHECK(hipStreamSynchronize(h->stream));
    for (int l = 0; l < g.nLevels; l++)
        if (dst[l]) cut_plane(h, l, h->hPyrStage + g.lv[l].planeOff, dst[l], dst_strides[l], padded);
    return AMOS_OK;
}

int amos_orb_level_image(amos_orb *h, int frame, int level, uint8_t *dst, size_t dst_stride, int padded)
{
    if (!h || !dst || !h->detected || frame < 0 || frame >= h->nFrames || level < 0 || level >= h->geom.nLevels) { set_error("amos_orb_level_image: invalid argument or state"); return AMOS_ERR_INVALID; }
    return copy_plane(h, h->dPyr, frame, level, dst, dst_stride, padded);
}

int amos_orb_blurred_image(amos_orb *h, int frame, int level, uint8_t *dst, size_t dst_stride)
{
    if (!h || !dst || !h->described || frame < 0 || frame >= h->nFrames || level < 0 || level >= h->geom.nLevels) { set_error("amos_orb_blurred_image: invalid argument or state"); return AMOS_ERR_INVALID; }
    return copy_plane(h, h->dBlur, frame, level, dst, dst_stride, 0);
}

int amos_orb_extract_batch_device(amos_orb *h, const uint8_t *d_gray, size_t frame_stride, size_t row_stride, int width,
                                  int height, int n_frames)
{
    if (!h || !d_gray || n_frames < 1 || width < 1 || height < 1 || row_stride < (size_t)width) { set_error("amos_orb_extract_batch_device: invalid argument"); return AMOS_ERR_INVALID; }
    if (n_frames > h->maxB) { set_error("batch of %d frames exceeds the handle's max_batch %d", n_frames, h->maxB); return AMOS_ERR_CAPACITY; }
    AMOS_HIP_CHECK(hipSetDevice(h->device));
    int rc = set_geometry(h, width, height);
    if (rc != AMOS_OK) return rc;
    rc = launch_detect(h, d_gray, frame_stride, row_stride, n_frames);
    if (rc != AMOS_OK) return rc;
    return launch_describe(h, n_frames);
}

int amos_orb_detect_batch_device(amos_orb *h, const uint8_t *d_gray, size_t frame_stride, size_t row_stride, int width,
                                 int height, int n_frames)
{
    if (!h || !d_gray || n_frames < 1 || width < 1 || height < 1 || row_stride < (size_t)width) { set_error("amos_orb_detect_batch_device: invalid argument"); return AMOS_ERR_INVALID; }
    if (n_frames > h->maxB) { set_error("batch of %d frames exceeds the handle's max_batch %d", n_frames, h->maxB); return AMOS_ERR_CAPACITY; }
    AMOS_HIP_CHECK(hipSetDevice(h->device));
    int rc = set_geometry(h, width, height);
    if (rc != AMOS_OK) return rc;
    return launch_detect(h, d_gray, frame_stride, row_stride, n_frames);
}

int amos_orb_gate_batch_device(amos_orb *h, const uint8_t *d_masks, size_t mask_frame_stride, size_t mask_row_stride)
{
    if (!h || !d_masks || mask_row_stride < 1) { set_error("amos_orb_gate_batch_device: invalid argument"); return AMOS_ERR_INVALID; }
    if (!h->detected) { set_error("amos_orb_gate_batch_device before detect"); return AMOS_ERR_STATE; }
    AMOS_HIP_CHECK(hipSetDevice(h->device));
    const Geom &g = h->geom;
    const size_t planeStride = (size_t)h->maskPitch * h->maxH;
    dim3 grid((g.W + kMorphTileW - 1) / kMorphTileW, (g.H + kMorphTileH - 1) / kMorphTileH, h->nFrames);
    AMOS_HIP_CHECK(hipMemsetAsync(h->dErr, 0, sizeof(int), h->stream));
    hipLaunchKernelGGL(k_morph31<true>, grid, dim3(256), 0, h->stream, d_masks, mask_frame_stride, (int)mask_row_stride, h->dMaskTmp, planeStride,
                       h->maskPitch, g.W, g.H);
    hipLaunchKernelGGL(k_morph31<false>, grid, dim3(256), 0, h->stream, h->dMaskTmp, planeStride, h->maskPitch, h->dMaskClosed, planeStride,
                       h->maskPitch, g.W, g.H);
    hipLaunchKernelGGL(k_gate, dim3(h->nFrames), dim3(256), 0, h->stream, h->dGeom, h->dLvKps, h->dLvCount, h->dMaskClosed, planeStride, h->maskPitch,
                       (const double *)nullptr, 0, (const int *)nullptr, 0, (const int *)nullptr, 0, h->dRemoved, h->dNRemoved, h->dErr);
    AMOS_HIP_CHECK(hipGetLastError());
    h->gated = true;
    return AMOS_OK;
}

int amos_orb_gate_labels_batch_device(amos_orb *h, const uint8_t *d_masks, size_t mask_frame_stride, size_t mask_row_stride, const double *d_labels,
                                      size_t label_frame_stride, size_t label_row_stride, const amos_slic_center *d_centers,
                                      size_t centers_frame_stride, int n_centers, const int32_t *d_rm, size_t rm_frame_stride, int n_rm, int32_t *d_status)
{
    if (!h || !d_masks || mask_row_stride < 1 || !d_labels || !d_centers || !d_rm || !d_status || n_centers < 1 || n_rm < 1 ||
        label_row_stride > (size_t)INT32_MAX) {
        set_error("amos_orb_gate_labels_batch_device: invalid argument");
        return AMOS_ERR_INVALID;
    }
    if (!h->detected) { set_error("amos_orb_gate_labels_batch_device before detect"); return AMOS_ERR_STATE; }
    const Geom &g = h->geom;
    if (label_row_stride < (size_t)g.W) { set_error("amos_orb_gate_labels_batch_device: label rows shorter than the frame"); return AMOS_ERR_INVALID; }
    AMOS_HIP_CHECK(hipSetDevice(h->device));
    const size_t planeStride = (size_t)h->maskPitch * h->maxH;
    dim3 grid((g.W + kMorphTileW - 1) / kMorphTileW, (g.H + kMorphTileH - 1) / kMorphTileH, h->nFrames);
    AMOS_HIP_CHECK(hipMemsetAsync(d_status, 0, sizeof(int32_t) * h->nFrames, h->stream));
    hipLaunchKernelGGL(k_morph31<true>, grid, dim3(256), 0, h->stream, d_masks, mask_frame_stride, (int)mask_row_stride, h->dMaskTmp, planeStride,
                       h->maskPitch, g.W, g.H);
    hipLaunchKernelGGL(k_morph31<false>, grid, dim3(256), 0, h->stream, h->dMaskTmp, planeStride, h->maskPitch, h->dMaskClosed, planeStride,
                       h->maskPitch, g.W, g.H);
    GateLabelStrides ls;
    constexpr int kRecInts = (int)(sizeof(amos_slic_center) / sizeof(int32_t));
    ls.labelFrame = label_frame_stride;
    ls.centerFrame = centers_frame_stride * kRecInts;
    ls.rmFrame = rm_frame_stride;
    ls.errFrame = 1;
    ls.centerStride = kRecInts;
    const int *ids = (const int *)d_centers + offsetof(amos_slic_center, id) / sizeof(int32_t);
    hipLaunchKernelGGL(k_gate, dim3(h->nFrames), dim3(256), 0, h->stream, h->dGeom, h->dLvKps, h->dLvCount, h->dMaskClosed, planeStride, h->maskPitch,
                       d_labels, (int)label_row_stride, ids, n_centers, (const int *)d_rm, n_rm, h->dRemoved, h->dNRemoved, (int *)d_status, ls);
    AMOS_HIP_CHECK(hipGetLastError());
    h->gated = true;
    return AMOS_OK;
}

int amos_orb_describe_batch_device(amos_orb *h)
{
    if (!h || !h->detected) { set_error("amos_orb_describe_batch_device before detect"); return AMOS_ERR_STATE; }
    AMOS_HIP_CHECK(hipSetDevice(h->device));
    return launch_describe(h, h->nFrames);
}

int amos_orb_extract_batch_device_color(amos_orb *h, const uint8_t *d_color, size_t frame_stride, size_t row_stride, int width,
                                        int height, int n_frames, int channels, int rgb_order)
{
    if (!h || !d_color || n_frames < 1 || width < 1 || height < 1 || (channels != 3 && channels != 4) || row_stride < (size_t)width * channels) {
        set_error("amos_orb_extract_batch_device_color: invalid argument");
        return AMOS_ERR_INVALID;
    }
    if (n_frames > h->maxB) { set_error("batch of %d frames exceeds the handle's max_batch %d", n_frames, h->maxB); return AMOS_ERR_CAPACITY; }
    AMOS_HIP_CHECK(hipSetDevice(h->device));
    int rc = set_geometry(h, width, height);
    if (rc != AMOS_OK) return rc;
    rc = launch_detect(h, d_color, frame_stride, row_stride, n_frames, channels, rgb_order != 0);
    if (rc != AMOS_OK) return rc;
    return launch_describe(h, n_frames);
}

int amos_orb_detect_color_with_mask_pre_batch_device(amos_orb *h, amos_mask_pre *pre, const uint8_t *d_color, size_t frame_stride, size_t row_stride,
                                                     int width, int height, int n_frames, int channels, int rgb_order, float *d_net_input)
{
    if (!h || !pre || !d_color || !d_net_input || n_frames < 1 || width < 1 || height < 1 || (channels != 3 && channels != 4) ||
        row_stride < (size_t)width * channels) {
        set_error("amos_orb_detect_color_with_mask_pre_batch_device: invalid argument");
        return AMOS_ERR_INVALID;
    }
    if (n_frames > h->maxB) { set_error("batch of %d frames exceeds the handle's max_batch %d", n_frames, h->maxB); return AMOS_ERR_CAPACITY; }
    MaskPreStageA a;
    int rc = mask_pre_stage_a(pre, &a);
    if (rc != AMOS_OK) return rc;
    if (a.width != width || a.height != height) { set_error("mask pre-processing handle made for %dx%d frames, got %dx%d", a.width, a.height, width, height); return AMOS_ERR_INVALID; }
    if (n_frames > a.maxBatch) { set_error("mask pre-processing handle made for %d frames, got %d", a.maxBatch, n_frames); return AMOS_ERR_CAPACITY; }
    if (width <= 2 * kEdge + 1 || height <= 2 * kEdge + 1) { set_error("frame too small for the fused import"); return AMOS_ERR_INVALID; }
    AMOS_HIP_CHECK(hipSetDevice(h->device));
    rc = set_geometry(h, width, height);
    if (rc != AMOS_OK) return rc;
    rc = launch_detect(h, d_color, frame_stride, row_stride, n_frames, channels, rgb_order != 0, &a);
    if (rc != AMOS_OK) return rc;
    return mask_pre_finish(pre, h->stream, n_frames, d_net_input);
}

static int make_undistort_args(float fx, float fy, float cx, float cy, const float *dist_coef, int n_dist, UndistortArgs &a, const char *who)
{
    if (!(fx != 0.f) || !(fy != 0.f) || n_dist < 0 || n_dist > 5 || (n_dist > 0 && !dist_coef)) { set_error("%s: invalid camera", who); return AMOS_ERR_INVALID; }
    a.fx = fx; a.fy = fy; a.cx = cx; a.cy = cy;
    for (int i = 0; i < 5; i++) a.k[i] = i < n_dist ? (double)dist_coef[i] : 0.;
    a.identity = n_dist == 0 || dist_coef[0] == 0.0f;
    return AMOS_OK;
}

int amos_frame_undistort_batch_device(amos_orb *h, float fx, float fy, float cx, float cy, const float *dist_coef, int n_dist,
                                      amos_keypoint *d_kps_un)
{
    if (!h || !d_kps_un) { set_error("amos_frame_undistort_batch_device: invalid argument"); return AMOS_ERR_INVALID; }
    if (!h->described) { set_error("amos_frame_undistort_batch_device before an extraction"); return AMOS_ERR_STATE; }
    UndistortArgs a;
    const int rc = make_undistort_args(fx, fy, cx, cy, dist_coef, n_dist, a, "amos_frame_undistort_batch_device");
    if (rc != AMOS_OK) return rc;
    AMOS_HIP_CHECK(hipSetDevice(h->device));
    hipLaunchKernelGGL(k_undistort, dim3((h->geom.kpCap + 255) / 256, h->nFrames), dim3(256), 0, h->stream, h->dGeom, h->dOutKps, h->dOutCount, a,
                       d_kps_un);
    AMOS_HIP_CHECK(hipGetLastError());
    return AMOS_OK;
}

int amos_frame_image_bounds(int width, int height, float fx, float fy, float cx, float cy, const float *dist_coef, int n_dist, float bounds[4])
{
    if (!bounds || width < 1 || height < 1) { set_error("amos_frame_image_bounds: invalid argument"); return AMOS_ERR_INVALID; }
    UndistortArgs a;
    const int rc = make_undistort_args(fx, fy, cx, cy, dist_coef, n_dist, a, "amos_frame_image_bounds");
    if (rc != AMOS_OK) return rc;
    if (a.identity) { bounds[0] = 0.f; bounds[1] = (float)width; bounds[2] = 0.f; bounds[3] = (float)height; return AMOS_OK; }
    const float px[4] = {0.f, (float)width, 0.f, (float)width}, py[4] = {0.f, 0.f, (float)height, (float)height};
    float ux[4], uy[4];
    for (int i = 0; i < 4; i++) undistort_point(px[i], py[i], a.fx, a.fy, a.cx, a.cy, a.k, ux[i], uy[i]);
    bounds[0] = std::min(ux[0], ux[2]);
    bounds[1] = std::max(ux[1], ux[3]);
    bounds[2] = std::min(uy[0], uy[1]);
    bounds[3] = std::max(uy[2], uy[3]);
    return AMOS_OK;
}

int amos_frame_rgbd_glue_batch_device(amos_orb *h, const void *d_depth, int depth_is_u16, float depth_map_factor,
                                      size_t depth_frame_stride_bytes, size_t depth_row_stride_bytes, float mbf, float min_x, float max_x,
                                      float min_y, float max_y, const amos_keypoint *d_kps_un, float *d_u_right, float *d_depth_out,
                                      int32_t *d_grid_cell)
{
    if (!h || !d_grid_cell || (d_depth && (!d_u_right || !d_depth_out)) || !(max_x > min_x) || !(max_y > min_y)) { set_error("amos_frame_rgbd_glue_batch_device: invalid argument"); return AMOS_ERR_INVALID; }
    if (!h->described) { set_error("amos_frame_rgbd_glue_batch_device before an extraction"); return AMOS_ERR_STATE; }
    AMOS_HIP_CHECK(hipSetDevice(h->device));
    const float wInv = static_cast<float>(AMOS_FRAME_GRID_COLS) / static_cast<float>(max_x - min_x);
    const float hInv = static_cast<float>(AMOS_FRAME_GRID_ROWS) / static_cast<float>(max_y - min_y);
    hipLaunchKernelGGL(k_rgbd_glue, dim3((h->geom.kpCap + 255) / 256, h->nFrames), dim3(256), 0, h->stream, h->dGeom, h->dOutKps, d_kps_un, h->dOutCount,
                       (const uint8_t *)d_depth, depth_is_u16, depth_map_factor, depth_frame_stride_bytes, depth_row_stride_bytes, mbf, min_x, min_y,
                       wInv, hInv, d_u_right, d_depth_out, d_grid_cell);
    AMOS_HIP_CHECK(hipGetLastError());
    return AMOS_OK;
}

int amos_orb_batch_results_device(amos_orb *h, const amos_keypoint **d_kps, const uint8_t **d_desc, const int32_t **d_counts,
                                  int *capacity)
{
    if (!h) return AMOS_ERR_INVALID;
    if (d_kps) *d_kps = h->dOutKps;
    if (d_desc) *d_desc = h->dOutDesc;
    if (d_counts) *d_counts = h->dOutCount;
    if (capacity) *capacity = h->capGeom.kpCap;
    return AMOS_OK;
}

int amos_orb_batch_fetch(amos_orb *h, int frame, amos_keypoint *kps, uint8_t *desc, int cap, int *n)
{
    if (!h || !h->described || frame < 0 || frame >= h->nFrames) { set_error("amos_orb_batch_fetch: invalid argument or state"); return AMOS_ERR_INVALID; }
    AMOS_HIP_CHECK(hipSetDevice(h->device));
    return fetch_frame(h, frame, kps, desc, cap, n);
}

int amos_orb_sync(amos_orb *h)
{
    if (!h) return AMOS_ERR_INVALID;
    AMOS_HIP_CHECK(hipStreamSynchronize(h->stream));
// ... 50 lines not shown
```

amos-slam_amd/csrc/orb_kernels.h:

```cpp
#pragma once
#include <type_traits>

#include "amos_common.h"
#include "amos_undistort.h"
#include "../../include/amos_orb_pattern.h"
#include "../../include/amos_host_types.h"

#ifndef AMOS_LATENCY_PRIO
#define AMOS_LATENCY_PRIO 0
#endif
#define AMOS_SET_LATENCY_PRIO() do { if (AMOS_LATENCY_PRIO > 0) __builtin_amdgcn_s_setprio(AMOS_LATENCY_PRIO); } while (0)

namespace amos {

__constant__ signed char c_pattern[1024];
__constant__ int c_umax[16];

__device__ __forceinline__ int reflect101(int i, int n)
{
    if (i < 0) i = -i;
    if (i >= n) i = 2 * n - 2 - i;
    return i;
}

// ... 1255 lines not shown
        if (j == 0) {
            amos_keypoint o = *kpSrc;
            if (level != 0) {
                o.x = __fmul_rn(o.x, lg.scale);
                o.y = __fmul_rn(o.y, lg.scale);
            }
            outKps[(size_t)frame * g->kpCap + dstIdx] = o;
        }
    }
}

__constant__ int c_ellipse_dx[31];

__device__ constexpr int kMorphDx[16] = {15, 15, 15, 15, 14, 14, 14, 13, 13, 12, 11, 10, 9, 7, 5, 0};
__device__ constexpr int kMorphPlane[16] = {8, 8, 8, 8, 7, 7, 7, 6, 6, 5, 4, 3, 2, 1, 0, -1};
constexpr int kMorphTileW = 64, kMorphTileH = 32, kMorphRows = kMorphTileH + 30, kMorphPitch = 96;

template <bool kDilate>
__global__ __launch_bounds__(256) void k_morph31(const uint8_t *__restrict__ src, size_t srcFrameStride, int srcStride,
                                                uint8_t *__restrict__ dst, size_t dstFrameStride, int stride, int w, int h)
{
    __shared__ __align__(16) uint8_t tile[kMorphRows][kMorphPitch];
    __shared__ __align__(16) uint8_t plane[9][kMorphRows][kMorphTileW];
    const int tid = threadIdx.x;
    const int x0 = blockIdx.x * kMorphTileW, y0 = blockIdx.y * kMorphTileH;
    src += (size_t)blockIdx.z * srcFrameStride;
    dst += (size_t)blockIdx.z * dstFrameStride;
    const int neutral = kDilate ? 0 : 255;
    auto pick = [](int a, int b, int c) { return kDilate ? max(a, max(b, c)) : min(a, min(b, c)); };
    __shared__ int sLo, sHi;
    if (tid == 0) { sLo = 255; sHi = 0; }
    __syncthreads();
    int lo = 255, hi = 0;
    for (int idx = tid; idx < kMorphRows * (kMorphTileW + 30); idx += 256) {
        const int r = idx / (kMorphTileW + 30), c = idx - r * (kMorphTileW + 30);
        const int y = y0 - 15 + r, x = x0 - 15 + c;
        const bool in = y >= 0 && y < h && x >= 0 && x < w;
        const int v = in ? src[(size_t)y * srcStride + x] : neutral;
        tile[r][c] = (uint8_t)v;
        lo = in ? min(lo, v) : lo;
        hi = in ? max(hi, v) : hi;
    }
#pragma unroll
    for (int d = 32; d > 0; d >>= 1) {
        lo = min(lo, __shfl_xor(lo, d, 64));
        hi = max(hi, __shfl_xor(hi, d, 64));
    }
    if ((tid & 63) == 0) { atomicMin(&sLo, lo); atomicMax(&sHi, hi); }
    __syncthreads();
    const int lx = tid & 63;
    if (sLo >= sHi) {
        const int v0 = sLo;
        for (int ly = tid >> 6; ly < kMorphTileH; ly += 4) {
            const int x = x0 + lx, y = y0 + ly;
            if (x < w && y < h) dst[(size_t)y * stride + x] = (uint8_t)v0;
        }
        return;
    }
    for (int r = tid >> 6; r < kMorphRows; r += 4) {
        const uint8_t *c = &tile[r][lx + 15];
        int m = pick(c[0], pick(c[-1], c[1], c[-2]), pick(c[2], c[-3], c[3]));
        m = pick(m, pick(c[-4], c[4], c[-5]), c[5]);
        plane[0][r][lx] = (uint8_t)m;
        m = pick(m, pick(c[-6], c[6], c[-7]), c[7]);
        plane[1][r][lx] = (uint8_t)m;
        m = pick(m, pick(c[-8], c[8], c[-9]), c[9]);
        plane[2][r][lx] = (uint8_t)m;
#pragma unroll
        for (int k = 10; k <= 15; k++) {
            m = pick(m, c[-k], c[k]);
            plane[k - 7][r][lx] = (uint8_t)m;
        }
    }
    __syncthreads();
    for (int ly = tid >> 6; ly < kMorphTileH; ly += 4) {
        const int x = x0 + lx, y = y0 + ly;
        int acc = pick(plane[8][ly + 15][lx], tile[ly][lx + 15], tile[ly + 30][lx + 15]);
#pragma unroll
        for (int dy = 1; dy <= 14; dy++) acc = pick(acc, plane[kMorphPlane[dy]][ly + 15 - dy][lx], plane[kMorphPlane[dy]][ly + 15 + dy][lx]);
        if (x < w && y < h) dst[(size_t)y * stride + x] = (uint8_t)acc;
    }
}

struct GateLabelStrides {
    size_t labelFrame = 0, centerFrame = 0, rmFrame = 0, errFrame = 0;
    int centerStride = 1;
};

__global__ __launch_bounds__(256) void k_gate(const Geom *__restrict__ g, amos_keypoint *__restrict__ lvKps,
                                             int *__restrict__ lvCount, const uint8_t *__restrict__ closedBase,
                                             size_t closedFrameStride, int maskStride, const double *__restrict__ labelBase,
                                             int labelStride,
                                             const int *__restrict__ centerIdBase, int nCenters,
                                             const int *__restrict__ rmBase, int nRm,
                                             amos_keypoint *__restrict__ removed, int *__restrict__ nRemoved,
                                             int *__restrict__ errBase, const GateLabelStrides ls = GateLabelStrides())
{
    __shared__ int wkeep[4], wrem[4];
    const int tid = threadIdx.x, lane = tid & 63, wave = tid >> 6;
    const int frame = blockIdx.x;
    const uint8_t *closed = closedBase + (size_t)frame * closedFrameStride;
    const double *labels = labelBase ? labelBase + (size_t)frame * ls.labelFrame : nullptr;
    const int *centerIds = centerIdBase ? centerIdBase + (size_t)frame * ls.centerFrame : nullptr;
    const int *rm = rmBase ? rmBase + (size_t)frame * ls.rmFrame : nullptr;
    int *errFlag = errBase + (size_t)frame * ls.errFrame;
    int remBase = 0;
    for (int level = 0; level < g->nLevels; level++) {
        const LevelGeom &lg = g->lv[level];
        amos_keypoint *kps = lvKps + (size_t)frame * g->kpLevelTotal + lg.kpOff;
        const int n = lvCount[frame * g->nLevels + level];
        const float scale = level != 0 ? lg.scale : 1.f;
        int keepBase = 0;
        for (int i0 = 0; i0 < n; i0 += 256) {
            const int i = i0 + tid;
            amos_keypoint kp;
            bool valid = i < n, drop = false;
            if (valid) {
                kp = kps[i];
                const int ix = (int)__fmul_rn(kp.x, scale), iy = (int)__fmul_rn(kp.y, scale);
                if (ix < 0 || iy < 0 || ix >= g->W || iy >= g->H) {
                    atomicOr(errFlag, 1);
                } else {
                    if (labels) {
                        const long ci = (long)(labels[(size_t)iy * labelStride + ix] - 1);
                        if (ci < 0 || ci >= nCenters) atomicOr(errFlag, 2);
                        else {
                            const int id = centerIds[(size_t)ci * ls.centerStride];
                            if (id < 0 || id >= nRm) atomicOr(errFlag, 2);
                            else if (rm[id] == 1) drop = true;
                        }
                    }
                    if (closed[(size_t)iy * maskStride + ix] != 0) drop = true;
                }
            }
            const unsigned long long bk = __ballot(valid && !drop), br = __ballot(valid && drop);
            if (lane == 0) { wkeep[wave] = __popcll(bk); wrem[wave] = __popcll(br); }
            __syncthreads();
            int ko = keepBase, ro = remBase;
            for (int w = 0; w < wave; w++) { ko += wkeep[w]; ro += wrem[w]; }
            const unsigned long long below = (1ull << lane) - 1ull;
            if (valid && !drop) kps[ko + __popcll(bk & below)] = kp;
            if (valid && drop) removed[(size_t)frame * g->kpLevelTotal + ro + __popcll(br & below)] = kp;
            keepBase += wkeep[0] + wkeep[1] + wkeep[2] + wkeep[3];
            remBase += wrem[0] + wrem[1] + wrem[2] + wrem[3];
            __syncthreads();
        }
        if (tid == 0) lvCount[frame * g->nLevels + level] = keepBase;
    }
    if (tid == 0) nRemoved[frame] = remBase;
}

struct UndistortArgs {
    double fx, fy, cx, cy;
    double k[5];
    int identity;
};

__global__ __launch_bounds__(256) void k_undistort(const Geom *__restrict__ g, const amos_keypoint *__restrict__ outKps,
                                                  const int *__restrict__ outCount, const UndistortArgs a,
                                                  amos_keypoint *__restrict__ kpsUn)
{
    const int i = blockIdx.x * 256 + threadIdx.x, frame = blockIdx.y;
    if (i >= outCount[frame] || i >= g->kpCap) return;
    const size_t o = (size_t)frame * g->kpCap + i;
    amos_keypoint kp = outKps[o];
    if (!a.identity) undistort_point(kp.x, kp.y, a.fx, a.fy, a.cx, a.cy, a.k, kp.x, kp.y);
    kpsUn[o] = kp;
}

__global__ __launch_bounds__(256) void k_rgbd_glue(const Geom *__restrict__ g, const amos_keypoint *__restrict__ outKps,
                                                  const amos_keypoint *__restrict__ kpsUn,
                                                  const int *__restrict__ outCount, const uint8_t *__restrict__ depth,
                                                  int depthIsU16, float depthFactor, size_t depthFrameStride,
                                                  size_t depthRowStride, float mbf, float minX, float minY,
                                                  float gridWInv, float gridHInv, float *__restrict__ uRight,
                                                  float *__restrict__ depthOut, int *__restrict__ gridCell)
{
    const int i = blockIdx.x * 256 + threadIdx.x, frame = blockIdx.y;
    if (i >= outCount[frame] || i >= g->kpCap) return;
    const size_t o = (size_t)frame * g->kpCap + i;
    const amos_keypoint kp = outKps[o];
    const amos_keypoint kpU = kpsUn ? kpsUn[o] : kp;
    const int u = (int)kp.x, v = (int)kp.y;
    float d = -1.f;
    if (depth != nullptr && u >= 0 && v >= 0 && u < g->W && v < g->H) {
        const uint8_t *row = depth + (size_t)frame * depthFrameStride + (size_t)v * depthRowStride;
        d = depthIsU16 ? __fmul_rn((float)reinterpret_cast<const uint16_t *>(row)[u], depthFactor)
                       : reinterpret_cast<const float *>(row)[u];
    }
    const bool ok = d > 0;
    if (depthOut) depthOut[o] = ok ? d : -1.f;
    if (uRight) uRight[o] = ok ? __fsub_rn(kpU.x, __fdiv_rn(mbf, d)) : -1.f;
    const int px = (int)roundf(__fmul_rn(__fsub_rn(kpU.x, minX), gridWInv));
    const int py = (int)roundf(__fmul_rn(__fsub_rn(kpU.y, minY), gridHInv));
    gridCell[o] = (px < 0 || px >= AMOS_FRAME_GRID_COLS || py < 0 || py >= AMOS_FRAME_GRID_ROWS) ? -1 : px * AMOS_FRAME_GRID_ROWS + py;
}

__global__ void k_unpack_candidates(const uint32_t *__restrict__ pts, int n, amos_keypoint *__restrict__ out)
{
    const int i = blockIdx.x * blockDim.x + threadIdx.x;
    if (i >= n) return;
    const uint32_t p = pts[i];
    amos_keypoint kp;
    kp.x = (float)(p & 0xfff);
    kp.y = (float)((p >> 12) & 0xfff);
    kp.size = 7.f;
    kp.angle = -1.f;
    kp.response = (float)(p >> 24);
    kp.octave = 0;
    kp.class_id = -1;
    out[i] = kp;
}

}
```

include/amos_frontend.h:

```cpp
#ifndef AMOS_FRONTEND_H
#define AMOS_FRONTEND_H

#include <stddef.h>
#include <stdint.h>

#ifdef __cplusplus
extern "C" {
#endif

#define AMOS_OK 0
#define AMOS_ERR_INVALID (-1)
#define AMOS_ERR_DEVICE (-2)
#define AMOS_ERR_CAPACITY (-3)
#define AMOS_ERR_STATE (-4)

#define AMOS_EDGE_THRESHOLD 19
#define AMOS_MAX_LEVELS 16
#define AMOS_FRAME_GRID_ROWS 48
#define AMOS_FRAME_GRID_COLS 64
#define AMOS_TH_HIGH 100
#define AMOS_TH_LOW 50
#define AMOS_HISTO_LENGTH 30

typedef struct amos_keypoint {
// ... 3 lines not shown
    float response;
    int32_t octave;
    int32_t class_id;
} amos_keypoint;

typedef struct amos_orb_params {
    int32_t n_features;
    float scale_factor;
    int32_t n_levels;
    int32_t ini_th_fast;
    int32_t min_th_fast;
} amos_orb_params;

typedef struct amos_orb amos_orb;
typedef struct amos_match amos_match;
typedef struct amos_mask_pre amos_mask_pre;

typedef struct amos_best2 {
    int32_t best_idx;
    int32_t best_dist;
    int32_t second_idx;
    int32_t second_dist;
} amos_best2;

const char *amos_last_error(void);
int amos_device_count(void);
int amos_current_device(void);
const char *amos_build_variant(void);


int amos_orb_create(const amos_orb_params *params, int max_width, int max_height, int max_batch,
                    int device, void *stream, amos_orb **out);
void amos_orb_destroy(amos_orb *h);

int amos_orb_geometry_probe(const amos_orb_params *params, int max_width, int max_height, int width,
                            int height, int32_t need[6], int32_t cap[6]);

int amos_orb_tables(const amos_orb *h, float *scale_factor, float *inv_scale_factor,
                    float *level_sigma2, float *inv_level_sigma2, int32_t *features_per_level,
                    int32_t *umax);
int amos_orb_tables_host(const amos_orb_params *params, float *scale_factor, float *inv_scale_factor,
                         float *level_sigma2, float *inv_level_sigma2, int32_t *features_per_level, int32_t *umax);
int amos_orb_level_sizes(const amos_orb *h, int width, int height, int32_t *level_w, int32_t *level_h);

int amos_orb_detect(amos_orb *h, const uint8_t *gray, size_t stride, int width, int height);

int amos_orb_level_count(amos_orb *h, int frame, int level);
int amos_orb_level_keypoints(amos_orb *h, int frame, int level, amos_keypoint *out, int cap);
int amos_orb_set_level_keypoints(amos_orb *h, int frame, int level, const amos_keypoint *kps, int n);

int amos_orb_level_layout(amos_orb *h, int32_t *offsets, int32_t *caps, int32_t *total);
int amos_orb_fetch_levels(amos_orb *h, int frame, int32_t *counts, amos_keypoint *buf, int buf_len);
int amos_orb_store_levels(amos_orb *h, int frame, const int32_t *counts, const amos_keypoint *buf, int buf_len);

int amos_orb_gate(amos_orb *h, const uint8_t *mask, size_t mask_stride, const double *labels,
                  size_t lstride, const int32_t *center_ids, int n_centers,
                  const int32_t *rm_vector, int n_rm, amos_keypoint *removed, int cap,
                  int *n_removed);
int amos_orb_closed_mask(amos_orb *h, uint8_t *dst, size_t dst_stride);

int amos_orb_describe(amos_orb *h, amos_keypoint *kps, uint8_t *desc, int cap, int *n);

int amos_orb_extract(amos_orb *h, const uint8_t *gray, size_t stride, int width, int height,
                     amos_keypoint *kps, uint8_t *desc, int cap, int *n);

int amos_orb_level_image(amos_orb *h, int frame, int level, uint8_t *dst, size_t dst_stride,
                         int padded);
int amos_orb_pyramid_images(amos_orb *h, int frame, uint8_t *const *dst, const size_t *dst_strides, int padded);
int amos_orb_blurred_image(amos_orb *h, int frame, int level, uint8_t *dst, size_t dst_stride);
int amos_orb_level_candidates(amos_orb *h, int frame, int level, amos_keypoint *out, int cap);

int amos_orb_extract_batch_device(amos_orb *h, const uint8_t *d_gray, size_t frame_stride,
                                  size_t row_stride, int width, int height, int n_frames);
int amos_orb_detect_batch_device(amos_orb *h, const uint8_t *d_gray, size_t frame_stride, size_t row_stride,
                                 int width, int height, int n_frames);
int amos_orb_gate_batch_device(amos_orb *h, const uint8_t *d_masks, size_t mask_frame_stride,
                               size_t mask_row_stride);
struct amos_slic_center;
int amos_orb_gate_labels_batch_device(amos_orb *h, const uint8_t *d_masks, size_t mask_frame_stride, size_t mask_row_stride,
                                      const double *d_labels, size_t label_frame_stride, size_t label_row_stride,
                                      const struct amos_slic_center *d_centers, size_t centers_frame_stride, int n_centers,
                                      const int32_t *d_rm, size_t rm_frame_stride, int n_rm, int32_t *d_status);
int amos_orb_describe_batch_device(amos_orb *h);

int amos_orb_extract_batch_device_color(amos_orb *h, const uint8_t *d_color, size_t frame_stride, size_t row_stride,
                                        int width, int height, int n_frames, int channels, int rgb_order);
int amos_frame_rgbd_glue_batch_device(amos_orb *h, const void *d_depth, int depth_is_u16, float depth_map_factor,
                                      size_t depth_frame_stride_bytes, size_t depth_row_stride_bytes, float mbf,
                                      float min_x, float max_x, float min_y, float max_y,
                                      const amos_keypoint *d_kps_un, float *d_u_right, float *d_depth_out,
                                      int32_t *d_grid_cell);
int amos_frame_stereo_match_batch_device(amos_orb *left, amos_orb *right, int n_pairs, float mbf, float min_z, float *d_u_right,
                                         float *d_depth, int32_t *d_sad, int32_t *d_status);
int amos_frame_stereo_match_arrays_device(amos_orb *left, amos_orb *right, int n_pairs, const amos_keypoint *d_kps_l,
                                          const uint8_t *d_desc_l, const int32_t *d_counts_l, int capacity_l,
                                          const amos_keypoint *d_kps_r, const uint8_t *d_desc_r, const int32_t *d_counts_r,
                                          int capacity_r, float mbf, float min_z, float *d_u_right, float *d_depth, int32_t *d_sad,
                                          int32_t *d_status);
int amos_frame_stereo_match(amos_orb *left, amos_orb *right, float mbf, float min_z, float *u_right, float *depth, int n);
int amos_frame_undistort_batch_device(amos_orb *h, float fx, float fy, float cx, float cy, const float *dist_coef,
                                      int n_dist, amos_keypoint *d_kps_un);
int amos_frame_image_bounds(int width, int height, float fx, float fy, float cx, float cy, const float *dist_coef,
                            int n_dist, float bounds[4]);

int amos_orb_batch_results_device(amos_orb *h, const amos_keypoint **d_kps, const uint8_t **d_desc,
                                  const int32_t **d_counts, int *capacity);
int amos_orb_batch_fetch(amos_orb *h, int frame, amos_keypoint *kps, uint8_t *desc, int cap, int *n);
int amos_orb_sync(amos_orb *h);

#define AMOS_ORB_STAGES 7
int amos_orb_timing_enable(amos_orb *h, int max_records);
int amos_orb_timing_collect(amos_orb *h, float *avg_ms, int *n_records);
void *amos_orb_stream(amos_orb *h);


int amos_match_create(int device, void *stream, amos_match **out);
void amos_match_destroy(amos_match *m);
int amos_match_sync(amos_match *m);
void *amos_match_stream(amos_match *m);

int amos_match_distances(amos_match *m, const uint8_t *q, int nq, const uint8_t *t, int nt,
                         uint16_t *out);
int amos_match_list_distances(amos_match *m, const uint8_t *q, int nq, const uint8_t *t, int nt,
                              const int32_t *cand_off, const int32_t *cand_idx, uint16_t *out);
int amos_match_list_best2(amos_match *m, const uint8_t *q, int nq, const uint8_t *t, int nt,
                          const int32_t *cand_off, const int32_t *cand_idx, int init_dist,
                          amos_best2 *out);
int amos_match_bruteforce_best2(amos_match *m, const uint8_t *q, int nq, const uint8_t *t, int nt,
                                int init_dist, amos_best2 *out);
int amos_match_set_bruteforce_kernel(amos_match *m, int mode);
int amos_match_bruteforce_best2_batch_device(amos_match *m, const uint8_t *d_desc,
                                             size_t frame_stride_bytes, const int32_t *d_counts,
                                             const int32_t *d_pairs_q, const int32_t *d_pairs_t,
                                             int n_pairs, int capacity, int init_dist,
                                             amos_best2 *d_out);


int amos_frame_grid_build_batch_device(amos_match *m, const int32_t *d_grid_cell, const int32_t *d_counts,
                                       int n_frames, int capacity, int32_t *d_cell_start,
                                       int32_t *d_items);

typedef struct amos_window_search {
    const amos_keypoint *d_kps;
    const uint8_t *d_desc;
    const int32_t *d_counts;
    const int32_t *d_cell_start;
    const int32_t *d_items;
    const float *d_query_uv;
    const float *d_query_invz;
    const float *d_u_right;
    const int32_t *d_pairs_q, *d_pairs_t;
    const float *scale_factors;
    int32_t n_pairs, capacity, n_levels;
    int32_t mode, init_dist;
    float th, mbf;
    float min_x, max_x, min_y, max_y;
} amos_window_search;
int amos_match_window_best2_batch_device(amos_match *m, const amos_window_search *w, amos_best2 *d_out);


typedef struct amos_map_point {
    float pos[3];
    float normal[3];
    float min_distance, max_distance;
    int32_t flags;
    uint8_t desc[32];
// ... 157 lines not shown
struct amos_bow_view;
int amos_match_bow(amos_match *m, const struct amos_bow_view *kf, const struct amos_bow_view *f, float nn_ratio, int check_orientation,
                   int32_t *matches_f, amos_bow_search_stats *stats);

typedef struct amos_kf_pair_search {
    const amos_keypoint *d_kps;
    const uint8_t *d_desc;
    const int32_t *d_counts;
    const int32_t *d_n_nodes;
    const uint32_t *d_node_ids;
    const int32_t *d_node_off;
    const int32_t *d_node_idx;
    const uint8_t *d_has_point;
    const float *d_u_right;
    const int32_t *d_pairs_1, *d_pairs_2;
    int32_t *d_match12;
    amos_bow_search_stats *d_stats;
    int32_t n_pairs, capacity;
} amos_kf_pair_search;
typedef struct amos_kf_geometry {
    float f12[9];
    float ex, ey;
} amos_kf_geometry;
int amos_match_bow_kf_batch_device(amos_match *m, const amos_kf_pair_search *s, float nn_ratio, int check_orientation);
int amos_match_triangulation_batch_device(amos_match *m, const amos_kf_pair_search *s, const amos_kf_geometry *d_geometry,
                                          const float *d_scale_factors, const float *d_level_sigma2, int n_levels, int only_stereo,
                                          int check_orientation);
int amos_match_bow_kf(amos_match *m, const struct amos_bow_view *k1, const struct amos_bow_view *k2, float nn_ratio, int check_orientation,
                      int32_t *match12, amos_bow_search_stats *stats);
int amos_match_triangulation(amos_match *m, const struct amos_bow_view *k1, const struct amos_bow_view *const *k2s, int n2,
                             const amos_kf_geometry *geometry, const float *scale_factors, const float *level_sigma2, int n_levels,
                             int only_stereo, int check_orientation, int32_t *match12, amos_bow_search_stats *stats);


#define AMOS_FUSE_LOCAL 0
#define AMOS_FUSE_SIM3 1
typedef struct amos_fuse_camera {
    float Rcw[9], tcw[3], Ow[3];
    float fx, fy, cx, cy, mbf;
    float th;
} amos_fuse_camera;
typedef struct amos_fuse_stats {
    int32_t n_in_view;
    int32_t n_accepted;
} amos_fuse_stats;
struct amos_window_query;
struct amos_frame_view;
typedef struct amos_fuse_search {
    const amos_keypoint *d_kps;
    const uint8_t *d_desc;
    const int32_t *d_counts;
    const int32_t *d_cell_start;
    const int32_t *d_items;
    const float *d_u_right;
    const float *scale_factors;
    const float *inv_level_sigma2;
    const amos_map_point *d_points;
    const int32_t *pair_frame;
    const int32_t *point_first, *point_count;
    const int32_t *out_off;
    const amos_fuse_camera *cameras;
    const uint8_t *d_skip;
    struct amos_window_query *d_query;
    uint8_t *d_in_view;
    int32_t *d_best_idx;
    int32_t *d_best_dist;
    amos_fuse_stats *d_stats;
    int32_t n_frames, n_pairs, n_points, capacity, n_levels;
    int32_t mode, max_dist;
    float min_x, max_x, min_y, max_y;
} amos_fuse_search;
int amos_match_fuse_batch_device(amos_match *m, const amos_fuse_search *s);
int amos_match_fuse(amos_match *m, const struct amos_frame_view *kfs, int n_kfs, const amos_map_point *points, int n_points, int n_pairs,
                    const int32_t *pair_frame, const int32_t *point_first, const int32_t *point_count, const int32_t *out_off,
                    const amos_fuse_camera *cameras, const uint8_t *skip, int n_out, const float *scale_factors, const float *inv_level_sigma2,
                    int n_levels, int mode, int max_dist, struct amos_window_query *query, uint8_t *in_view, int32_t *best_idx, int32_t *best_dist,
                    amos_fuse_stats *stats);


int amos_mask_pre_create(int device, void *stream, int width, int height, int max_batch, amos_mask_pre **out);
void amos_mask_pre_destroy(amos_mask_pre *p);
void *amos_mask_pre_stream(amos_mask_pre *p);
int amos_mask_preprocess_batch_device(amos_mask_pre *p, const uint8_t *d_bgr, int n_frames, float *d_out);

int amos_orb_detect_color_with_mask_pre_batch_device(amos_orb *h, amos_mask_pre *pre, const uint8_t *d_color,
                                                     size_t frame_stride, size_t row_stride, int width, int height,
                                                     int n_frames, int channels, int rgb_order, float *d_net_input);

int amos_mask_bias_act_device(void *stream, float *d_y, const float *d_bias, const float *d_residual, size_t n,
                              int channels, int relu);

int amos_mask_bias_relu_maxpool_device(void *stream, const float *d_x, const float *d_bias, float *d_y, int n, int in_h, int in_w,
                                       int channels);

int amos_mask_stem_weight_floats(void);
int amos_mask_stem_weights_device(void *stream, const float *d_w, long long stride_n, long long stride_c, long long stride_y, long long stride_x,
                                  float *d_packed);
int amos_mask_stem_device(void *stream, const float *d_x, long long stride_b, long long stride_c, long long stride_y, long long stride_x,
                          const float *d_packed, const float *d_bias, float *d_y, int batch, int height, int width);

int amos_mask_conv_supported(int cin, int cout, int kh, int kw, int stride, int pad);
int amos_mask_conv_device(void *stream, const float *d_x, const float *d_w, const float *d_bias, const float *d_residual,
                          float *d_y, int batch, int in_h, int in_w, int cin, int cout, int kh, int kw, int stride, int pad,
                          int relu);
size_t amos_mask_conv_workspace_bytes(int batch, int in_h, int in_w, int cin, int cout, int kh, int kw, int stride, int pad);
int amos_mask_conv_ws_device(void *stream, const float *d_x, const float *d_w, const float *d_bias, const float *d_residual, float *d_y,
                             int batch, int in_h, int in_w, int cin, int cout, int kh, int kw, int stride, int pad, int relu,
                             void *d_workspace, size_t workspace_bytes);
int amos_mask_conv_tile_mode(int mode);
int amos_mask_conv_kernel_name(int batch, int in_h, int in_w, int cin, int cout, int kh, int kw, int stride, int pad, char *name,
                               int name_len);
int amos_mask_conv_chain_supported(int batch, int in_h, int in_w, int cin, int planes, int cout, int stride);
int amos_mask_conv_chain_device(void *stream, const float *d_x, const float *d_wd, const float *d_bd, const float *d_yc, const float *d_w3,
                                const float *d_b3, float *d_y, int batch, int in_h, int in_w, int cin, int planes, int cout, int stride);
int amos_mask_conv1x1_supported(int cin, int cout, int stride);

int amos_mask_winograd_supported(int cin, int cout);
size_t amos_mask_winograd_weight_floats(int cin, int cout);
int amos_mask_winograd_weights_device(void *stream, const float *d_w, float *d_u, int cin, int cout);
int amos_mask_winograd_conv_device(void *stream, const float *d_x, const float *d_u, const float *d_bias, const float *d_residual,
                                   float *d_y, int batch, int h, int w, int cin, int cout, int relu);
size_t amos_mask_winograd24_weight_floats(int cin, int cout);
int amos_mask_winograd24_weights_device(void *stream, const float *d_w, float *d_u, int cin, int cout);
int amos_mask_winograd24_conv_device(void *stream, const float *d_x, const float *d_u, const float *d_bias, const float *d_residual,
                                     float *d_y, int batch, int h, int w, int cin, int cout, int relu);
int amos_mask_winograd24_conv_layout_device(void *stream, const float *d_x, const float *d_u, const float *d_bias, const float *d_residual,
                                            float *d_y, int batch, int h, int w, int cin, int cout, int relu, int in_blocked, int out_blocked);
int amos_mask_winograd24_persistent_mode(int mode);
int amos_mask_winograd24_narrow_mode(int mode);
int amos_mask_conv1x1_device(void *stream, const float *d_x, const float *d_w, const float *d_bias, const float *d_residual,
                             float *d_y, int batch, int in_h, int in_w, int cin, int cout, int stride, int relu);

int amos_mask_bilinear_nhwc_device(void *stream, const float *d_x, float *d_y, int n, int in_h, int in_w, int out_h,
                                   int out_w, int channels, float scale_h, float scale_w);

int amos_mask_bilinear_nhwc_act_device(void *stream, const float *d_x, float *d_y, int n, int in_h, int in_w, int out_h,
                                       int out_w, int channels, float scale_h, float scale_w, int relu);

int amos_mask_bilinear_x2_mode(int mode);

int amos_mask_nms_column_max_device(void *stream, const float *d_boxes, float *d_out, int n_lists, int k);

int amos_mask_class_scores_device(void *stream, const float *d_conf, float *d_scores, int batch, int n_priors,
                                  int n_classes_with_background, float threshold);

int amos_mask_person_mask_device(void *stream, const float *d_masks, const uint8_t *d_flags, uint8_t *d_out, int batch, int n_det,
                                 int mask_h, int mask_w, int out_h, int out_w);

int amos_mask_head_outputs_device(void *stream, const float *d_raw, const float *d_bias, float *d_loc, float *d_conf, float *d_coef,
                                  int batch, int cells, int channels_padded, int anchors, int n_classes_with_background, int mask_dim,
                                  int n_priors_total, int prior_offset);
int amos_mask_head_outputs_scores_device(void *stream, const float *d_raw, const float *d_bias, float *d_loc, float *d_conf, float *d_coef, float *d_scores,
                                         float threshold, int batch, int cells, int channels_padded, int anchors, int n_classes_with_background,
                                         int mask_dim, int n_priors_total, int prior_offset);

int amos_mask_topk_rows_device(void *stream, const float *d_x, float *d_values, long long *d_indices, int rows, int n, int k);
int amos_mask_topk_rows_sparse_device(void *stream, const float *d_x, float *d_values, long long *d_indices, int rows, int n, int k, float fill);

#define AMOS_MASK_NMS_TOP_K 200
#define AMOS_MASK_NMS_THRESH 0.5f
#define AMOS_MASK_CONF_THRESH 0.05f
#define AMOS_MASK_SCORE_THRESHOLD 0.15f
#define AMOS_MASK_TOP_K_DISPLAY 15
#define AMOS_MASK_PERSON_CLASS 0
size_t amos_mask_post_workspace_bytes(int batch, int n_priors, int n_classes_with_background, int mask_dim, int proto_h, int proto_w);
int amos_mask_person_masks_device(void *stream, const float *d_loc, const float *d_conf, const float *d_coef, const float *d_priors,
// ... 195 lines not shown
```

Measured before the change: 1646 frames/s.

## Fuse mask preprocessing into one tiled kernel and bit-pack gate closing mask

Adds a single-pass mask preprocessing kernel that loads a source window into LDS and performs the fixed-point resize, LUT, float resize and final normalized resize per 32x32 output tile. This replaces the multi-kernel chain that goes through mid and back intermediate buffers in global memory. The chain buffers are now allocated lazily, and the fused path is enabled by default when the windows fit in LDS. It also adds bit-packed mask and dilation kernels so the gate can evaluate the morphological closing per keypoint from bitmasks, along with mode switches and a removed-keypoint query.

```diff
diff --git a/amos-slam_amd/__init__.py b/amos-slam_amd/__init__.py
--- a/amos-slam_amd/__init__.py
+++ b/amos-slam_amd/__init__.py
@@ -44,6 +44,8 @@
     "amos_orb_detect_batch_device": (_i, (_v, _v, _z, _z, _i, _i, _i)),
     "amos_orb_gate_batch_device": (_i, (_v, _v, _z, _z)),
     "amos_orb_gate_labels_batch_device": (_i, (_v, _v, _z, _z, _v, _z, _z, _v, _z, _i, _v, _z, _i, _v)),
+    "amos_orb_gate_mode": (_i, (_i,)),
+    "amos_orb_batch_removed": (_i, (_v, _i, _v, _i, _v)),
     "amos_orb_describe_batch_device": (_i, (_v,)),
     "amos_orb_extract_batch_device_color": (_i, (_v, _v, _z, _z, _i, _i, _i, _i, _i)),
     "amos_frame_rgbd_glue_batch_device": (_i, (_v, _v, _i, _f, _z, _z, _f, _f, _f, _f, _f, _v, _v, _v, _v)),
@@ -93,6 +95,8 @@
     "amos_mask_pre_destroy": (None, (_v,)),
     "amos_mask_pre_stream": (_v, (_v,)),
     "amos_mask_preprocess_batch_device": (_i, (_v, _v, _i, _v)),
+    "amos_mask_pre_mode": (_i, (_i,)),
+    "amos_mask_pre_one_pass": (_i, (_v, _v)),
     "amos_orb_detect_color_with_mask_pre_batch_device": (_i, (_v, _v, _v, _z, _z, _i, _i, _i, _i, _i, _v)),
     "amos_mask_bias_act_device": (_i, (_v, _v, _v, _v, _z, _i, _i)),
     "amos_mask_bias_relu_maxpool_device": (_i, (_v, _v, _v, _v, _i, _i, _i, _i)),
@@ -389,6 +393,13 @@
                                                         d_centers, centers_frame_stride, n_centers, d_rm, rm_frame_stride, n_rm, d_status),
                "amos_orb_gate_labels_batch_device")
 
+    def batch_removed(self, frame):
+        total, n = C.c_int32(0), C.c_int(0)
+        _check(self.L.amos_orb_level_layout(self.h, None, None, C.byref(total)), "amos_orb_level_layout")
+        removed = np.zeros(total.value + 1, KP_DTYPE)
+        _check(self.L.amos_orb_batch_removed(self.h, frame, _p(removed), len(removed), C.byref(n)), "amos_orb_batch_removed")
+        return removed[:n.value].copy()
+
     def describe_batch_device(self):
         _check(self.L.amos_orb_describe_batch_device(self.h), "amos_orb_describe_batch_device")
 
@@ -520,6 +531,14 @@
     def run(self, d_bgr, n_frames, d_out):
         _check(self.L.amos_mask_preprocess_batch_device(self.h, d_bgr, n_frames, d_out), "amos_mask_preprocess_batch_device")
 
+    def one_pass(self):
+        need = C.c_int(0)
+        return bool(_check(self.L.amos_mask_pre_one_pass(self.h, C.byref(need)), "amos_mask_pre_one_pass")), need.value
+
+
+def mask_pre_mode(mode=-1):
+    return int(lib().amos_mask_pre_mode(mode))
+
 
 def mask_bias_act(stream_ptr, y_ptr, bias_ptr, residual_ptr, n, channels, relu):
     _check(lib().amos_mask_bias_act_device(stream_ptr, y_ptr, bias_ptr, residual_ptr, n, channels, int(relu)), "amos_mask_bias_act_device")
@@ -569,6 +588,10 @@
 def mask_stem(stream_ptr, x_ptr, x_strides, packed_ptr, bias_ptr, y_ptr, batch, height, width):
     sb, sc, sy, sx = (int(v) for v in x_strides)
     _check(lib().amos_mask_stem_device(stream_ptr, x_ptr, sb, sc, sy, sx, packed_ptr, bias_ptr, y_ptr, batch, height, width), "amos_mask_stem_device")
+
+
+def orb_gate_mode(mode=-1):
+    return int(lib().amos_orb_gate_mode(mode))
 
 
 def mask_bilinear_x2_mode(mode=-1):
diff --git a/amos-slam_amd/csrc/amos_common.h b/amos-slam_amd/csrc/amos_common.h
--- a/amos-slam_amd/csrc/amos_common.h
+++ b/amos-slam_amd/csrc/amos_common.h
@@ -167,7 +167,10 @@
     uint8_t *hStage;
 };
 int orb_stereo_view(amos_orb *h, size_t sadScratchInts, OrbStereoView *out);
-int mask_pre_stage_a(amos_mask_pre *p, MaskPreStageA *out);
+int mask_pre_stage_a(amos_mask_pre *p, MaskPreStageA *out, bool withChain);
 int mask_pre_finish(amos_mask_pre *p, hipStream_t stream, int n_frames, float *d_out);
+bool mask_pre_one_pass(const amos_mask_pre *p);
+int mask_pre_run_one_pass(amos_mask_pre *p, hipStream_t stream, const uint8_t *d_color, size_t frame_stride, size_t row_stride, int channels,
+                          int n_frames, float *d_out);
 const char *w24_variant_tag();
 }
diff --git a/amos-slam_amd/csrc/amos_mask_pre.hip b/amos-slam_amd/csrc/amos_mask_pre.hip
--- a/amos-slam_amd/csrc/amos_mask_pre.hip
+++ b/amos-slam_amd/csrc/amos_mask_pre.hip
@@ -1,6 +1,8 @@
 #include "amos_common.h"
 
+#include <algorithm>
 #include <cmath>
+#include <cstdlib>
 #include <vector>
 
 namespace amos {
@@ -68,6 +70,143 @@
         const float bot = __fadd_rn(__fmul_rn(wl0, p10[c]), __fmul_rn(wl1, p11[c]));
         const float v = __fadd_rn(__fmul_rn(hl0, top), __fmul_rn(hl1, bot));
         o[(size_t)(2 - c) * kNetSize * kNetSize] = __fdiv_rn(__fsub_rn(v, mean[c]), stdv[c]);
+    }
+}
+
+
+constexpr int kPreTile = 32, kPreBRows = 30, kPreBCols = 39, kPreARows = 41, kPreACols = 31, kPreSrcBytes = 16 * 1024;
+
+__host__ __device__ inline int pre_src_pitch(int cols) { return (cols * 3 + 3) & ~3; }
+
+struct PreTables { const FixTap *fixX, *fixY; const FltTap *fltX, *fltY; const float *lut; };
+
+__host__ __device__ inline void pre_c_tap(int o, float scale, int inN, int &i0, int &step, float &l0, float &l1)
+{
+#ifdef __HIP_DEVICE_COMPILE__
+    const float r = fmaxf(__fsub_rn(__fmul_rn(scale, __fadd_rn((float)o, 0.5f)), 0.5f), 0.f);
+    i0 = (int)r; step = i0 < inN - 1 ? 1 : 0;
+    l1 = __fsub_rn(r, (float)i0); l0 = __fsub_rn(1.f, l1);
+#else
+    volatile float a = (float)o + 0.5f, b = scale * a, c = b - 0.5f;
+    const float r = c > 0.f ? c : 0.f;
+    i0 = (int)r; step = i0 < inN - 1 ? 1 : 0;
+    l1 = r - (float)i0; l0 = 1.f - l1;
+#endif
+}
+
+struct PreAxisWindow { int b0, b1, m0, m1, s0, s1; };
+__host__ __device__ inline PreAxisWindow pre_axis_window(int o0, int o1, int backN, float scale, const FltTap *flt, const FixTap *fix)
+{
+    PreAxisWindow w;
+    int i, st;
+    float l0, l1;
+    pre_c_tap(o0, scale, backN, i, st, l0, l1);
+    w.b0 = i;
+    pre_c_tap(o1, scale, backN, i, st, l0, l1);
+    w.b1 = i + st;
+    w.m0 = flt[w.b0].s0; w.m1 = flt[w.b1].s1;
+    w.s0 = fix[w.m0].s0; w.s1 = fix[w.m1].s1;
+    return w;
+}
+
+__global__ __launch_bounds__(256) void k_mask_pre_fused(const uint8_t *__restrict__ src, size_t frameStride, size_t rowStride, int channels,
+                                                       const PreTables t, float *__restrict__ out)
+{
+    __shared__ __align__(16) uint8_t sSrc[kPreSrcBytes];
+    __shared__ float sA[kPreARows * kPreACols * 3];
+    __shared__ float sLut[256];
+    static_assert(kPreBRows * kPreBCols * 3 * sizeof(float) <= kPreSrcBytes, "B's window takes the source window's place");
+    float *sB = reinterpret_cast<float *>(sSrc);
+    const int tid = threadIdx.x, frame = blockIdx.z;
+    const int ox0 = blockIdx.x * kPreTile, oy0 = blockIdx.y * kPreTile;
+    const float sh = (float)kBackH / (float)kNetSize, sw = (float)kBackW / (float)kNetSize;
+    const PreAxisWindow wx = pre_axis_window(ox0, min(ox0 + kPreTile, kNetSize) - 1, kBackW, sw, t.fltX, t.fixX);
+    const PreAxisWindow wy = pre_axis_window(oy0, min(oy0 + kPreTile, kNetSize) - 1, kBackH, sh, t.fltY, t.fixY);
+    const int nSC = wx.s1 - wx.s0 + 1, nSR = wy.s1 - wy.s0 + 1, pitch = pre_src_pitch(nSC);
+    const int nAC = wx.m1 - wx.m0 + 1, nAR = wy.m1 - wy.m0 + 1, nBC = wx.b1 - wx.b0 + 1, nBR = wy.b1 - wy.b0 + 1;
+    auto magic = [](int n) { return n > 1 ? 0xffffffffu / (unsigned)n + 1u : 0u; };
+    auto div = [](int idx, unsigned m) { return m ? (int)__umulhi((unsigned)idx, m) : idx; };
+    sLut[tid] = t.lut[tid];
+    const uint8_t *s0 = src + (size_t)frame * frameStride + (size_t)wy.s0 * rowStride + (size_t)wx.s0 * channels;
+    if (channels == 3) {
+        const int nb = nSC * 3, nd = pitch >> 2;
+        const unsigned m = magic(nd);
+        for (int idx = tid; idx < nSR * nd; idx += 256) {
+            const int r = div(idx, m), j = 4 * (idx - r * nd);
+            const uint8_t *g = s0 + (size_t)r * rowStride + j;
+            unsigned v = 0;
+            if (j + 4 <= nb) __builtin_memcpy(&v, g, 4);
+            else
+                for (int k = 0; j + k < nb; k++) v |= (unsigned)g[k] << (8 * k);
+            *reinterpret_cast<unsigned *>(sSrc + r * pitch + j) = v;
+        }
+    } else {
+        const unsigned m = magic(nSC);
+        for (int idx = tid; idx < nSR * nSC; idx += 256) {
+            const int r = div(idx, m), c = idx - r * nSC;
+            unsigned v;
+            __builtin_memcpy(&v, s0 + (size_t)r * rowStride + (size_t)c * 4, 4);
+            uint8_t *d = sSrc + r * pitch + 3 * c;
+            d[0] = (uint8_t)v; d[1] = (uint8_t)(v >> 8); d[2] = (uint8_t)(v >> 16);
+        }
+    }
+    __syncthreads();
+    static_assert(kPreACols <= 32 && kPreBRows <= 32 && kPreTile == 32, "the thread layouts below");
+    const int lo = tid & 31, hi = tid >> 5;
+    if (lo < nAC) {
+        const FixTap ax = t.fixX[wx.m0 + lo];
+        const int xa = 3 * (ax.s0 - wx.s0), xb = 3 * (ax.s1 - wx.s0);
+        for (int r = hi; r < nAR; r += 8) {
+            const FixTap ay = t.fixY[wy.m0 + r];
+            const uint8_t *r0 = sSrc + (ay.s0 - wy.s0) * pitch, *r1 = sSrc + (ay.s1 - wy.s0) * pitch;
+            float *o = sA + (r * nAC + lo) * 3;
+#pragma unroll
+            for (int k = 0; k < 3; k++) {
+                const int h0 = r0[xa + k] * ax.a0 + r0[xb + k] * ax.a1;
+                const int h1 = r1[xa + k] * ax.a0 + r1[xb + k] * ax.a1;
+                const int v = (((ay.a0 * (h0 >> 4)) >> 16) + ((ay.a1 * (h1 >> 4)) >> 16) + 2) >> 2;
+                o[k] = sLut[v];
+            }
+        }
+    }
+    __syncthreads();
+    if (lo < nBR) {
+        const FltTap ay = t.fltY[wy.b0 + lo];
+        const float *r0 = sA + (ay.s0 - wy.m0) * nAC * 3, *r1 = sA + (ay.s1 - wy.m0) * nAC * 3;
+        for (int c = hi; c < nBC; c += 8) {
+            const FltTap ax = t.fltX[wx.b0 + c];
+            const int xa = 3 * (ax.s0 - wx.m0), xb = 3 * (ax.s1 - wx.m0);
+            float *o = sB + (lo * nBC + c) * 3;
+#pragma unroll
+            for (int k = 0; k < 3; k++) {
+                const float h0 = __fadd_rn(__fmul_rn(r0[xa + k], ax.f0), __fmul_rn(r0[xb + k], ax.f1));
+                const float h1 = __fadd_rn(__fmul_rn(r1[xa + k], ax.f0), __fmul_rn(r1[xb + k], ax.f1));
+                o[k] = __fadd_rn(__fmul_rn(h0, ay.f0), __fmul_rn(h1, ay.f1));
+            }
+        }
+    }
+    __syncthreads();
+    const int ox = ox0 + lo;
+    if (ox < kNetSize) {
+        const float mean[3] = {103.94f, 116.78f, 123.68f}, stdv[3] = {57.38f, 57.12f, 58.40f};
+        int w1, w1p;
+        float wl0, wl1;
+        pre_c_tap(ox, sw, kBackW, w1, w1p, wl0, wl1);
+        const float *col = sB + (w1 - wx.b0) * 3;
+        for (int oy = oy0 + hi; oy < min(oy0 + kPreTile, kNetSize); oy += 8) {
+            int h1, h1p;
+            float hl0, hl1;
+            pre_c_tap(oy, sh, kBackH, h1, h1p, hl0, hl1);
+            const float *p00 = col + (h1 - wy.b0) * nBC * 3, *p01 = p00 + w1p * 3, *p10 = p00 + h1p * nBC * 3, *p11 = p10 + w1p * 3;
+            float *o = out + (size_t)frame * 3 * kNetSize * kNetSize + (size_t)oy * kNetSize + ox;
+#pragma unroll
+            for (int k = 0; k < 3; k++) {
+                const float top = __fadd_rn(__fmul_rn(wl0, p00[k]), __fmul_rn(wl1, p01[k]));
+                const float bot = __fadd_rn(__fmul_rn(wl0, p10[k]), __fmul_rn(wl1, p11[k]));
+                const float v = __fadd_rn(__fmul_rn(hl0, top), __fmul_rn(hl1, bot));
+                o[(size_t)(2 - k) * kNetSize * kNetSize] = __fdiv_rn(__fsub_rn(v, mean[k]), stdv[k]);
+            }
+        }
     }
 }
 
@@ -263,9 +402,40 @@
     int width = 0, height = 0, maxBatch = 0;
     FixTap *dFixX = nullptr, *dFixY = nullptr;
     FltTap *dFltX = nullptr, *dFltY = nullptr;
-    float *dLut = nullptr, *dMid = nullptr, *dBack = nullptr;
+    float *dLut = nullptr;
+    float *dMid = nullptr, *dBack = nullptr;
     int *dFirstX = nullptr, *dFirstY = nullptr;
+    bool onePassFits = false;
+    int srcWindowBytes = 0;
 };
+
+static int g_pre_fused = -1;
+
+static int pre_fused_mode()
+{
+    if (g_pre_fused < 0) {
+        const char *env = getenv("AMOS_MASK_PRE_FUSED");
+        g_pre_fused = env && env[0] == '0' ? 0 : 1;
+    }
+    return g_pre_fused;
+}
+
+static int pre_chain_buffers(amos_mask_pre *p)
+{
+    if (p->dMid && p->dBack) return AMOS_OK;
+    AMOS_HIP_CHECK(hipSetDevice(p->device));
+    if (!p->dMid) AMOS_HIP_CHECK(hipMalloc((void **)&p->dMid, sizeof(float) * 3 * kMidW * kMidH * (size_t)p->maxBatch));
+    if (!p->dBack) AMOS_HIP_CHECK(hipMalloc((void **)&p->dBack, sizeof(float) * 3 * kBackW * kBackH * (size_t)p->maxBatch));
+    return AMOS_OK;
+}
+
+static void launch_pre_fused(amos_mask_pre *p, hipStream_t stream, const uint8_t *src, size_t frameStride, size_t rowStride, int channels, int n_frames,
+                             float *d_out)
+{
+    const PreTables t{p->dFixX, p->dFixY, p->dFltX, p->dFltY, p->dLut};
+    const int tiles = (kNetSize + kPreTile - 1) / kPreTile;
+    hipLaunchKernelGGL(k_mask_pre_fused, dim3(tiles, tiles, n_frames), dim3(256), 0, stream, src, frameStride, rowStride, channels, t, d_out);
+}
 
 static void axis_taps(int srcN, int dstN, bool clampFraction, std::vector<int> &s0, std::vector<int> &s1, std::vector<float> &f)
 {
@@ -288,10 +458,22 @@
 static int round_even(float v) { return (int)std::nearbyintf(v); }
 
 namespace amos {
-int mask_pre_stage_a(amos_mask_pre *p, MaskPreStageA *out)
+int mask_pre_stage_a(amos_mask_pre *p, MaskPreStageA *out, bool withChain)
 {
     if (!p || !out) { set_error("mask pre-processing handle missing"); return AMOS_ERR_INVALID; }
+    if (withChain) {
+        const int rc = pre_chain_buffers(p);
+        if (rc != AMOS_OK) return rc;
+    }
     *out = MaskPreStageA{p->dFixX, p->dFixY, p->dFirstX, p->dFirstY, p->dLut, p->dMid, p->width, p->height, p->maxBatch};
+    return AMOS_OK;
+}
+bool mask_pre_one_pass(const amos_mask_pre *p) { return p && p->onePassFits && pre_fused_mode() == 1; }
+int mask_pre_run_one_pass(amos_mask_pre *p, hipStream_t stream, const uint8_t *d_color, size_t frame_stride, size_t row_stride, int channels, int n_frames,
+                          float *d_out)
+{
+    launch_pre_fused(p, stream, d_color, frame_stride, row_stride, channels, n_frames, d_out);
+    AMOS_HIP_CHECK(hipGetLastError());
     return AMOS_OK;
 }
 int mask_pre_finish(amos_mask_pre *p, hipStream_t stream, int n_frames, float *d_out)
@@ -314,9 +496,12 @@
     if (rc != AMOS_OK) { delete p; return rc; }
     std::vector<int> s0, s1;
     std::vector<float> f;
+    std::vector<FixTap> hFix[2];
+    std::vector<FltTap> hFlt[2];
     auto fix = [&](int srcN, int dstN, bool clamp, FixTap **dst, int **first) -> hipError_t {
         axis_taps(srcN, dstN, clamp, s0, s1, f);
-        std::vector<FixTap> t(dstN);
+        std::vector<FixTap> &t = hFix[clamp ? 0 : 1];
+        t.resize(dstN);
         for (int d = 0; d < dstN; d++) t[d] = FixTap{s0[d], s1[d], round_even((1.f - f[d]) * 2048.f), round_even(f[d] * 2048.f)};
         std::vector<int> inv(srcN + 1);
         for (int X = 0, d = 0; X <= srcN; X++) {
@@ -331,7 +516,8 @@
     };
     auto flt = [&](int srcN, int dstN, bool clamp, FltTap **dst) -> hipError_t {
         axis_taps(srcN, dstN, clamp, s0, s1, f);
-        std::vector<FltTap> t(dstN);
+        std::vector<FltTap> &t = hFlt[clamp ? 0 : 1];
+        t.resize(dstN);
         for (int d = 0; d < dstN; d++) t[d] = FltTap{s0[d], s1[d], 1.0f - f[d], f[d]};
         hipError_t e = hipMalloc((void **)dst, sizeof(FltTap) * dstN);
         if (e != hipSuccess) return e;
@@ -345,12 +531,29 @@
     if (e == hipSuccess) e = flt(kMidH, kBackH, false, &p->dFltY);
     if (e == hipSuccess) e = hipMalloc((void **)&p->dLut, sizeof(lut));
     if (e == hipSuccess) e = hipMemcpy(p->dLut, lut, sizeof(lut), hipMemcpyHostToDevice);
-    if (e == hipSuccess) e = hipMalloc((void **)&p->dMid, sizeof(float) * 3 * kMidW * kMidH * (size_t)max_batch);
-    if (e == hipSuccess) e = hipMalloc((void **)&p->dBack, sizeof(float) * 3 * kBackW * kBackH * (size_t)max_batch);
     if (e != hipSuccess) {
         set_error("amos_mask_pre_create: %s", hipGetErrorString(e));
         amos_mask_pre_destroy(p);
         return AMOS_ERR_DEVICE;
+    }
+    {
+        bool fits = true;
+        auto rising = [&](auto &t) {
+            for (size_t d = 1; d < t.size(); d++) fits = fits && t[d].s0 >= t[d - 1].s0 && t[d].s1 >= t[d - 1].s1 && t[d].s1 >= t[d].s0;
+        };
+        rising(hFix[0]); rising(hFix[1]); rising(hFlt[0]); rising(hFlt[1]);
+        const float sh = (float)kBackH / (float)kNetSize, sw = (float)kBackW / (float)kNetSize;
+        int srcRows = 0, srcCols = 0;
+        for (int o0 = 0; fits && o0 < kNetSize; o0 += kPreTile) {
+            const int o1 = std::min(o0 + kPreTile, kNetSize) - 1;
+            const PreAxisWindow wx = pre_axis_window(o0, o1, kBackW, sw, hFlt[0].data(), hFix[0].data());
+            const PreAxisWindow wy = pre_axis_window(o0, o1, kBackH, sh, hFlt[1].data(), hFix[1].data());
+            fits = wx.b1 - wx.b0 < kPreBCols && wy.b1 - wy.b0 < kPreBRows && wx.m1 - wx.m0 < kPreACols && wy.m1 - wy.m0 < kPreARows;
+            srcCols = std::max(srcCols, wx.s1 - wx.s0 + 1);
+            srcRows = std::max(srcRows, wy.s1 - wy.s0 + 1);
+        }
+        p->srcWindowBytes = srcRows * pre_src_pitch(srcCols);
+        p->onePassFits = fits && p->srcWindowBytes <= kPreSrcBytes;
     }
     *out = p;
     return AMOS_OK;
@@ -367,11 +570,29 @@
 
 void *amos_mask_pre_stream(amos_mask_pre *p) { return p ? (void *)p->stream : nullptr; }
 
+int amos_mask_pre_mode(int mode)
+{
+    const int before = pre_fused_mode();
+    if (mode == 0 || mode == 1) g_pre_fused = mode;
+    return before;
+}
+
+int amos_mask_pre_one_pass(const amos_mask_pre *p, int *source_window_bytes)
+{
+    if (!p) { set_error("amos_mask_pre_one_pass: invalid argument"); return AMOS_ERR_INVALID; }
+    if (source_window_bytes) *source_window_bytes = p->srcWindowBytes;
+    return mask_pre_one_pass(p) ? 1 : 0;
+}
+
 int amos_mask_preprocess_batch_device(amos_mask_pre *p, const uint8_t *d_bgr, int n_frames, float *d_out)
 {
     if (!p || !d_bgr || !d_out || n_frames < 1) { set_error("amos_mask_preprocess_batch_device: invalid argument"); return AMOS_ERR_INVALID; }
     if (n_frames > p->maxBatch) { set_error("amos_mask_preprocess_batch_device: %d frames, handle made for %d", n_frames, p->maxBatch); return AMOS_ERR_CAPACITY; }
     AMOS_HIP_CHECK(hipSetDevice(p->device));
+    if (mask_pre_one_pass(p))
+        return mask_pre_run_one_pass(p, p->stream, d_bgr, (size_t)p->width * p->height * 3, (size_t)p->width * 3, 3, n_frames, d_out);
+    const int rc = pre_chain_buffers(p);
+    if (rc != AMOS_OK) return rc;
     hipLaunchKernelGGL(k_mask_pre_a, dim3((kMidW * kMidH + 255) / 256, n_frames), dim3(256), 0, p->stream, d_bgr, p->width, p->height, p->dFixX,
                        p->dFixY, p->dLut, p->dMid);
     hipLaunchKernelGGL(k_mask_pre_b, dim3((kBackW * kBackH + 255) / 256, n_frames), dim3(256), 0, p->stream, p->dMid, p->dFltX, p->dFltY, p->dBack);
diff --git a/amos-slam_amd/csrc/amos_orb.hip b/amos-slam_amd/csrc/amos_orb.hip
--- a/amos-slam_amd/csrc/amos_orb.hip
+++ b/amos-slam_amd/csrc/amos_orb.hip
@@ -65,6 +65,8 @@
     int *dStereoSad = nullptr;
     float *dStereoOut = nullptr;
     uint8_t *dMask = nullptr, *dMaskTmp = nullptr, *dMaskClosed = nullptr;
+    unsigned long long *dMaskBits = nullptr, *dMaskBitsDil = nullptr;
+    int maskWords = 0;
     uint8_t *hStage = nullptr;
     uint8_t *hPyrStage = nullptr;
     double *dLabels = nullptr;
@@ -75,6 +77,7 @@
     std::vector<hipEvent_t> events;
     int maxRecords = 0, nRecords = 0;
     bool detected = false, described = false, gated = false;
+    bool gatedBits = false;
 };
 
 static int build_tables(amos_orb *h)
@@ -339,7 +342,7 @@
     AMOS_HIP_CHECK(hipStreamSynchronize(h->stream));
     h->curW = W;
     h->curH = Hh;
-    h->detected = h->described = h->gated = false;
+    h->detected = h->described = h->gated = h->gatedBits = false;
     return AMOS_OK;
 }
 
@@ -397,7 +400,7 @@
     AMOS_HIP_CHECK(hipGetLastError());
     h->nFrames = nFrames;
     h->detected = true;
-    h->described = h->gated = false;
+    h->described = h->gated = h->gatedBits = false;
     return AMOS_OK;
 }
 
@@ -583,6 +586,7 @@
     const size_t slack = 4096;
     h->inputPitch = align_up(max_width, 128);
     h->maskPitch = align_up(max_width, 128);
+    h->maskWords = (max_width + 63) / 64;
 #define ALLOC(ptr, count) do { rc = dev_alloc(&(ptr), (count)); if (rc != AMOS_OK) { amos_orb_destroy(h); return rc; } } while (0)
     ALLOC(h->dGeom, 1);
     ALLOC(h->dCells, h->capCells);
@@ -608,6 +612,8 @@
     ALLOC(h->dMask, (size_t)h->maskPitch * max_height);
     ALLOC(h->dMaskTmp, B * (size_t)h->maskPitch * max_height);
     ALLOC(h->dMaskClosed, B * (size_t)h->maskPitch * max_height);
+    ALLOC(h->dMaskBits, B * (size_t)h->maskWords * max_height);
+    ALLOC(h->dMaskBitsDil, B * (size_t)h->maskWords * max_height);
     ALLOC(h->dLabels, (size_t)max_width * max_height);
     ALLOC(h->dNRemoved, B);
     ALLOC(h->dErr, 1);
@@ -662,7 +668,7 @@
     h->close();
     void *ptrs[] = {h->dGeom, h->dCells, h->dTaps, h->dPyr, h->dBlur, h->dInput, h->dSlotCount, h->dSlots, h->dPts,
                     h->dNodeOf, h->dQuadOf, h->dCandCount, h->dLvCount, h->dOutCount, h->dLvKps, h->dOutKps, h->dOutDesc,
-                    h->dRemoved, h->dScratchKps, h->dMask, h->dMaskTmp, h->dMaskClosed, h->dLabels, h->dCenterIds, h->dRm,
+                    h->dRemoved, h->dScratchKps, h->dMask, h->dMaskTmp, h->dMaskClosed, h->dMaskBits, h->dMaskBitsDil, h->dLabels, h->dCenterIds, h->dRm,
                     h->dNRemoved, h->dErr, h->dStereoSad, h->dStereoOut};
     for (void *p : ptrs) if (p) (void)hipFree(p);
     if (h->hStage) (void)hipHostFree(h->hStage);
@@ -834,7 +840,7 @@
     dim3 grid((g.W + kMorphTileW - 1) / kMorphTileW, (g.H + kMorphTileH - 1) / kMorphTileH);
     hipLaunchKernelGGL(k_morph31<true>, grid, dim3(256), 0, h->stream, h->dMask, (size_t)0, h->maskPitch, h->dMaskTmp, (size_t)0, h->maskPitch, g.W, g.H);
     hipLaunchKernelGGL(k_morph31<false>, grid, dim3(256), 0, h->stream, h->dMaskTmp, (size_t)0, h->maskPitch, h->dMaskClosed, (size_t)0, h->maskPitch, g.W, g.H);
-    hipLaunchKernelGGL(k_gate, dim3(1), dim3(256), 0, h->stream, h->dGeom, h->dLvKps, h->dLvCount, h->dMaskClosed, (size_t)0, h->maskPitch,
+    hipLaunchKernelGGL(k_gate<false>, dim3(1), dim3(256), 0, h->stream, h->dGeom, h->dLvKps, h->dLvCount, h->dMaskClosed, (size_t)0, h->maskPitch,
                        labels ? h->dLabels : nullptr, g.W, h->dCenterIds, n_centers, h->dRm, n_rm, h->dRemoved, h->dNRemoved, h->dErr);
     AMOS_HIP_CHECK(hipGetLastError());
     int nrem = 0, err = 0;
@@ -842,6 +848,7 @@
     AMOS_HIP_CHECK(hipMemcpyAsync(&err, h->dErr, sizeof(int), hipMemcpyDeviceToHost, h->stream));
     AMOS_HIP_CHECK(hipStreamSynchronize(h->stream));
     h->gated = true;
+    h->gatedBits = false;
     if (err) { set_error("amos_orb_gate: %s", (err & 1) ? "keypoint outside the mask" : "label / cluster id out of range"); return AMOS_ERR_INVALID; }
     *n_removed = nrem;
     if (removed) {
@@ -857,6 +864,7 @@
 int amos_orb_closed_mask(amos_orb *h, uint8_t *dst, size_t dst_stride)
 {
     if (!h || !dst || !h->gated) { set_error("amos_orb_closed_mask: no gate has run"); return AMOS_ERR_STATE; }
+    if (h->gatedBits) { set_error("amos_orb_closed_mask: the last gate was a batch gate on bit planes (amos_orb_gate_mode 1): there is no grey closed mask"); return AMOS_ERR_STATE; }
     AMOS_HIP_CHECK(hipMemcpy2DAsync(dst, dst_stride, h->dMaskClosed, h->maskPitch, h->geom.W, h->geom.H, hipMemcpyDeviceToHost, h->stream));
     AMOS_HIP_CHECK(hipStreamSynchronize(h->stream));
     return AMOS_OK;
@@ -970,6 +978,46 @@
     return launch_detect(h, d_gray, frame_stride, row_stride, n_frames);
 }
 
+static int g_gate_bits = -1;
+
+static int gate_bits_mode()
+{
+    if (g_gate_bits < 0) {
+        const char *env = getenv("AMOS_GATE_BITS");
+        g_gate_bits = env && env[0] == '0' ? 0 : 1;
+    }
+    return g_gate_bits;
+}
+
+int amos_orb_gate_mode(int mode)
+{
+    const int before = gate_bits_mode();
+    if (mode == 0 || mode == 1) g_gate_bits = mode;
+    return before;
+}
+
+static bool launch_batch_closing(amos_orb *h, const uint8_t *d_masks, size_t mask_frame_stride, size_t mask_row_stride)
+{
+    const Geom &g = h->geom;
+    const bool bits = gate_bits_mode() == 1;
+    if (bits) {
+        const int words = (g.W + 63) / 64;
+        const size_t bitsStride = (size_t)h->maskWords * h->maxH;
+        hipLaunchKernelGGL(k_bits_pack, dim3((words + 3) / 4, (g.H + kBitsPackRows - 1) / kBitsPackRows, h->nFrames), dim3(256), 0, h->stream, d_masks,
+                           mask_frame_stride, mask_row_stride, h->dMaskBits, bitsStride, words, g.W, g.H);
+        hipLaunchKernelGGL(k_bits_dilate, dim3((g.H * words + 255) / 256, 1, h->nFrames), dim3(256), 0, h->stream, h->dMaskBits, h->dMaskBitsDil,
+                           bitsStride, words, g.W, g.H);
+    } else {
+        const size_t planeStride = (size_t)h->maskPitch * h->maxH;
+        dim3 grid((g.W + kMorphTileW - 1) / kMorphTileW, (g.H + kMorphTileH - 1) / kMorphTileH, h->nFrames);
+        hipLaunchKernelGGL(k_morph31<true>, grid, dim3(256), 0, h->stream, d_masks, mask_frame_stride, (int)mask_row_stride, h->dMaskTmp, planeStride,
+                           h->maskPitch, g.W, g.H);
+        hipLaunchKernelGGL(k_morph31<false>, grid, dim3(256), 0, h->stream, h->dMaskTmp, planeStride, h->maskPitch, h->dMaskClosed, planeStride,
+                           h->maskPitch, g.W, g.H);
+    }
+    return bits;
+}
+
 int amos_orb_gate_batch_device(amos_orb *h, const uint8_t *d_masks, size_t mask_frame_stride, size_t mask_row_stride)
 {
     if (!h || !d_masks || mask_row_stride < 1) { set_error("amos_orb_gate_batch_device: invalid argument"); return AMOS_ERR_INVALID; }
@@ -977,16 +1025,18 @@
     AMOS_HIP_CHECK(hipSetDevice(h->device));
     const Geom &g = h->geom;
     const size_t planeStride = (size_t)h->maskPitch * h->maxH;
-    dim3 grid((g.W + kMorphTileW - 1) / kMorphTileW, (g.H + kMorphTileH - 1) / kMorphTileH, h->nFrames);
     AMOS_HIP_CHECK(hipMemsetAsync(h->dErr, 0, sizeof(int), h->stream));
-    hipLaunchKernelGGL(k_morph31<true>, grid, dim3(256), 0, h->stream, d_masks, mask_frame_stride, (int)mask_row_stride, h->dMaskTmp, planeStride,
-                       h->maskPitch, g.W, g.H);
-    hipLaunchKernelGGL(k_morph31<false>, grid, dim3(256), 0, h->stream, h->dMaskTmp, planeStride, h->maskPitch, h->dMaskClosed, planeStride,
-                       h->maskPitch, g.W, g.H);
-    hipLaunchKernelGGL(k_gate, dim3(h->nFrames), dim3(256), 0, h->stream, h->dGeom, h->dLvKps, h->dLvCount, h->dMaskClosed, planeStride, h->maskPitch,
-                       (const double *)nullptr, 0, (const int *)nullptr, 0, (const int *)nullptr, 0, h->dRemoved, h->dNRemoved, h->dErr);
+    const bool bits = launch_batch_closing(h, d_masks, mask_frame_stride, mask_row_stride);
+    if (bits)
+        hipLaunchKernelGGL(k_gate<true>, dim3(h->nFrames), dim3(256), 0, h->stream, h->dGeom, h->dLvKps, h->dLvCount, (const uint8_t *)nullptr, (size_t)0, 0,
+                           (const double *)nullptr, 0, (const int *)nullptr, 0, (const int *)nullptr, 0, h->dRemoved, h->dNRemoved, h->dErr,
+                           GateLabelStrides(), h->dMaskBitsDil, (size_t)h->maskWords * h->maxH, (g.W + 63) / 64);
+    else
+        hipLaunchKernelGGL(k_gate<false>, dim3(h->nFrames), dim3(256), 0, h->stream, h->dGeom, h->dLvKps, h->dLvCount, h->dMaskClosed, planeStride,
+                           h->maskPitch, (const double *)nullptr, 0, (const int *)nullptr, 0, (const int *)nullptr, 0, h->dRemoved, h->dNRemoved, h->dErr);
     AMOS_HIP_CHECK(hipGetLastError());
     h->gated = true;
+    h->gatedBits = bits;
     return AMOS_OK;
 }
 
@@ -1004,12 +1054,8 @@
     if (label_row_stride < (size_t)g.W) { set_error("amos_orb_gate_labels_batch_device: label rows shorter than the frame"); return AMOS_ERR_INVALID; }
     AMOS_HIP_CHECK(hipSetDevice(h->device));
     const size_t planeStride = (size_t)h->maskPitch * h->maxH;
-    dim3 grid((g.W + kMorphTileW - 1) / kMorphTileW, (g.H + kMorphTileH - 1) / kMorphTileH, h->nFrames);
     AMOS_HIP_CHECK(hipMemsetAsync(d_status, 0, sizeof(int32_t) * h->nFrames, h->stream));
-    hipLaunchKernelGGL(k_morph31<true>, grid, dim3(256), 0, h->stream, d_masks, mask_frame_stride, (int)mask_row_stride, h->dMaskTmp, planeStride,
-                       h->maskPitch, g.W, g.H);
-    hipLaunchKernelGGL(k_morph31<false>, grid, dim3(256), 0, h->stream, h->dMaskTmp, planeStride, h->maskPitch, h->dMaskClosed, planeStride,
-                       h->maskPitch, g.W, g.H);
+    const bool bits = launch_batch_closing(h, d_masks, mask_frame_stride, mask_row_stride);
     GateLabelStrides ls;
     constexpr int kRecInts = (int)(sizeof(amos_slic_center) / sizeof(int32_t));
     ls.labelFrame = label_frame_stride;
@@ -1018,10 +1064,36 @@
     ls.errFrame = 1;
     ls.centerStride = kRecInts;
     const int *ids = (const int *)d_centers + offsetof(amos_slic_center, id) / sizeof(int32_t);
-    hipLaunchKernelGGL(k_gate, dim3(h->nFrames), dim3(256), 0, h->stream, h->dGeom, h->dLvKps, h->dLvCount, h->dMaskClosed, planeStride, h->maskPitch,
-                       d_labels, (int)label_row_stride, ids, n_centers, (const int *)d_rm, n_rm, h->dRemoved, h->dNRemoved, (int *)d_status, ls);
+    if (bits)
+        hipLaunchKernelGGL(k_gate<true>, dim3(h->nFrames), dim3(256), 0, h->stream, h->dGeom, h->dLvKps, h->dLvCount, (const uint8_t *)nullptr, (size_t)0, 0,
+                           d_labels, (int)label_row_stride, ids, n_centers, (const int *)d_rm, n_rm, h->dRemoved, h->dNRemoved, (int *)d_status, ls,
+                           h->dMaskBitsDil, (size_t)h->maskWords * h->maxH, (g.W + 63) / 64);
+    else
+        hipLaunchKernelGGL(k_gate<false>, dim3(h->nFrames), dim3(256), 0, h->stream, h->dGeom, h->dLvKps, h->dLvCount, h->dMaskClosed, planeStride,
+                           h->maskPitch, d_labels, (int)label_row_stride, ids, n_centers, (const int *)d_rm, n_rm, h->dRemoved, h->dNRemoved,
+                           (int *)d_status, ls);
     AMOS_HIP_CHECK(hipGetLastError());
     h->gated = true;
+    h->gatedBits = bits;
+    return AMOS_OK;
+}
+
+int amos_orb_batch_removed(amos_orb *h, int frame, amos_keypoint *removed, int cap, int *n_removed)
+{
+    if (!h || !n_removed || frame < 0 || frame >= h->nFrames) { set_error("amos_orb_batch_removed: invalid argument"); return AMOS_ERR_INVALID; }
+    if (!h->gated) { set_error("amos_orb_batch_removed: no gate has run"); return AMOS_ERR_STATE; }
+    AMOS_HIP_CHECK(hipSetDevice(h->device));
+    int n = 0;
+    AMOS_HIP_CHECK(hipMemcpyAsync(&n, h->dNRemoved + frame, sizeof(int), hipMemcpyDeviceToHost, h->stream));
+    AMOS_HIP_CHECK(hipStreamSynchronize(h->stream));
+    *n_removed = n;
+    if (removed) {
+        if (n > cap) { set_error("%d keypoints removed, caller capacity %d", n, cap); return AMOS_ERR_CAPACITY; }
+        if (n > 0) {
+            AMOS_HIP_CHECK(hipMemcpyAsync(removed, h->dRemoved + (size_t)frame * h->geom.kpLevelTotal, sizeof(amos_keypoint) * n, hipMemcpyDeviceToHost, h->stream));
+            AMOS_HIP_CHECK(hipStreamSynchronize(h->stream));
+        }
+    }
     return AMOS_OK;
 }
 
@@ -1057,8 +1129,9 @@
         return AMOS_ERR_INVALID;
     }
     if (n_frames > h->maxB) { set_error("batch of %d frames exceeds the handle's max_batch %d", n_frames, h->maxB); return AMOS_ERR_CAPACITY; }
+    const bool onePass = mask_pre_one_pass(pre);
     MaskPreStageA a;
-    int rc = mask_pre_stage_a(pre, &a);
+    int rc = mask_pre_stage_a(pre, &a, !onePass);
     if (rc != AMOS_OK) return rc;
     if (a.width != width || a.height != height) { set_error("mask pre-processing handle made for %dx%d frames, got %dx%d", a.width, a.height, width, height); return AMOS_ERR_INVALID; }
     if (n_frames > a.maxBatch) { set_error("mask pre-processing handle made for %d frames, got %d", a.maxBatch, n_frames); return AMOS_ERR_CAPACITY; }
@@ -1066,8 +1139,9 @@
     AMOS_HIP_CHECK(hipSetDevice(h->device));
     rc = set_geometry(h, width, height);
     if (rc != AMOS_OK) return rc;
-    rc = launch_detect(h, d_color, frame_stride, row_stride, n_frames, channels, rgb_order != 0, &a);
-    if (rc != AMOS_OK) return rc;
+    rc = launch_detect(h, d_color, frame_stride, row_stride, n_frames, channels, rgb_order != 0, onePass ? nullptr : &a);
+    if (rc != AMOS_OK) return rc;
+    if (onePass) return mask_pre_run_one_pass(pre, h->stream, d_color, frame_stride, row_stride, channels, n_frames, d_net_input);
     return mask_pre_finish(pre, h->stream, n_frames, d_net_input);
 }
 
diff --git a/amos-slam_amd/csrc/orb_kernels.h b/amos-slam_amd/csrc/orb_kernels.h
--- a/amos-slam_amd/csrc/orb_kernels.h
+++ b/amos-slam_amd/csrc/orb_kernels.h
@@ -1361,11 +1361,86 @@
     }
 }
 
+constexpr int kBitsPackRows = 8;
+
+__global__ __launch_bounds__(256) void k_bits_pack(const uint8_t *__restrict__ src, size_t srcFrameStride, size_t srcStride,
+                                                  unsigned long long *__restrict__ dst, size_t dstFrameStride, int words, int w, int h)
+{
+    const int lane = threadIdx.x & 63, word = blockIdx.x * 4 + (threadIdx.x >> 6), y0 = blockIdx.y * kBitsPackRows;
+    if (word >= words) return;
+    const int x = word * 64 + lane;
+    src += (size_t)blockIdx.z * srcFrameStride;
+    unsigned long long mine = 0;
+#pragma unroll
+    for (int r = 0; r < kBitsPackRows; r++) {
+        const int y = y0 + r;
+        const int v = (x < w && y < h) ? src[(size_t)y * srcStride + x] : 0;
+        const unsigned long long b = __ballot(v != 0);
+        if (lane == r) mine = b;
+    }
+    if (lane < kBitsPackRows && y0 + lane < h) dst[(size_t)blockIdx.z * dstFrameStride + (size_t)(y0 + lane) * words + word] = mine;
+}
+
+__global__ __launch_bounds__(256) void k_bits_dilate(const unsigned long long *__restrict__ src, unsigned long long *__restrict__ dst,
+                                                    size_t frameStride, int words, int w, int h)
+{
+    const int t = blockIdx.x * 256 + threadIdx.x;
+    if (t >= h * words) return;
+    const int y = t / words, k = t - y * words;
+    src += (size_t)blockIdx.z * frameStride;
+    unsigned long long lo = 0, hi = 0;
+    auto take = [&](int yy) {
+        if (yy < 0 || yy >= h) return;
+        const unsigned long long *row = src + (size_t)yy * words;
+        const unsigned long long c = row[k], l = k > 0 ? row[k - 1] : 0ull, r = k < words - 1 ? row[k + 1] : 0ull;
+        lo |= (l >> 32) | (c << 32);
+        hi |= (c >> 32) | (r << 32);
+    };
+    auto widen = [&](int d) {
+        for (int r = 0; r < d;) {
+            const int s = min(d - r, 2 * r + 1);
+            const unsigned long long ll = lo << s, lh = (hi << s) | (lo >> (64 - s)), rl = (lo >> s) | (hi << (64 - s)), rh = hi >> s;
+            lo |= ll | rl;
+            hi |= lh | rh;
+            r += s;
+        }
+    };
+#pragma unroll
+    for (int a = 0; a <= 15; a++) {
+        if (a > 0 && kMorphDx[a] != kMorphDx[a - 1]) widen(kMorphDx[a - 1] - kMorphDx[a]);
+        take(y - a);
+        if (a > 0) take(y + a);
+    }
+    static_assert(kMorphDx[15] == 0, "the last element row is one pixel wide");
+    unsigned long long out = (lo >> 32) | (hi << 32);
+    const int valid = w - 64 * k;
+    if (valid < 64) out &= (1ull << valid) - 1ull;
+    dst[(size_t)blockIdx.z * frameStride + t] = out;
+}
+
+__device__ __forceinline__ bool bits_closed_at(const unsigned long long *__restrict__ dil, int words, int w, int h, int ix, int iy)
+{
+    bool all = true;
+#pragma unroll
+    for (int dy = -15; dy <= 15; dy++) {
+        const int r = kMorphDx[dy < 0 ? -dy : dy], yy = iy + dy;
+        const bool inside = yy >= 0 && yy < h;
+        const unsigned long long *row = dil + (size_t)(inside ? yy : iy) * words;
+        const int x0 = max(ix - r, 0), x1 = min(ix + r, w - 1), k0 = x0 >> 6, k1 = x1 >> 6;
+        const unsigned long long m0 = ~0ull << (x0 & 63), m1 = ~0ull >> (63 - (x1 & 63));
+        const unsigned long long a = k0 == k1 ? (m0 & m1) : m0, b = k0 == k1 ? (m0 & m1) : m1;
+        const bool ok = ((row[k0] & a) == a) & ((row[k1] & b) == b);
+        all = all & (ok | !inside);
+    }
+    return all;
+}
+
 struct GateLabelStrides {
     size_t labelFrame = 0, centerFrame = 0, rmFrame = 0, errFrame = 0;
     int centerStride = 1;
 };
 
+template <bool kBits>
 __global__ __launch_bounds__(256) void k_gate(const Geom *__restrict__ g, amos_keypoint *__restrict__ lvKps,
                                              int *__restrict__ lvCount, const uint8_t *__restrict__ closedBase,
                                              size_t closedFrameStride, int maskStride, const double *__restrict__ labelBase,
@@ -1373,12 +1448,14 @@
                                              const int *__restrict__ centerIdBase, int nCenters,
                                              const int *__restrict__ rmBase, int nRm,
                                              amos_keypoint *__restrict__ removed, int *__restrict__ nRemoved,
-                                             int *__restrict__ errBase, const GateLabelStrides ls = GateLabelStrides())
+                                             int *__restrict__ errBase, const GateLabelStrides ls = GateLabelStrides(),
+                                             const unsigned long long *__restrict__ dilBase = nullptr, size_t dilFrameStride = 0,
+                                             int dilWords = 0)
 {
     __shared__ int wkeep[4], wrem[4];
     const int tid = threadIdx.x, lane = tid & 63, wave = tid >> 6;
     const int frame = blockIdx.x;
-    const uint8_t *closed = closedBase + (size_t)frame * closedFrameStride;
+    const uint8_t *closed = kBits ? nullptr : closedBase + (size_t)frame * closedFrameStride;
     const double *labels = labelBase ? labelBase + (size_t)frame * ls.labelFrame : nullptr;
     const int *centerIds = centerIdBase ? centerIdBase + (size_t)frame * ls.centerFrame : nullptr;
     const int *rm = rmBase ? rmBase + (size_t)frame * ls.rmFrame : nullptr;
@@ -1409,7 +1486,9 @@
                             else if (rm[id] == 1) drop = true;
                         }
                     }
-                    if (closed[(size_t)iy * maskStride + ix] != 0) drop = true;
+                    if (kBits ? bits_closed_at(dilBase + (size_t)frame * dilFrameStride, dilWords, g->W, g->H, ix, iy)
+                              : closed[(size_t)iy * maskStride + ix] != 0)
+                        drop = true;
                 }
             }
             const unsigned long long bk = __ballot(valid && !drop), br = __ballot(valid && drop);
diff --git a/include/amos_frontend.h b/include/amos_frontend.h
--- a/include/amos_frontend.h
+++ b/include/amos_frontend.h
@@ -109,6 +109,8 @@
                                       const struct amos_slic_center *d_centers, size_t centers_frame_stride, int n_centers,
                                       const int32_t *d_rm, size_t rm_frame_stride, int n_rm, int32_t *d_status);
 int amos_orb_describe_batch_device(amos_orb *h);
+int amos_orb_gate_mode(int mode);
+int amos_orb_batch_removed(amos_orb *h, int frame, amos_keypoint *removed, int cap, int *n_removed);
 
 int amos_orb_extract_batch_device_color(amos_orb *h, const uint8_t *d_color, size_t frame_stride, size_t row_stride,
                                         int width, int height, int n_frames, int channels, int rgb_order);
@@ -432,6 +434,8 @@
 void amos_mask_pre_destroy(amos_mask_pre *p);
 void *amos_mask_pre_stream(amos_mask_pre *p);
 int amos_mask_preprocess_batch_device(amos_mask_pre *p, const uint8_t *d_bgr, int n_frames, float *d_out);
+int amos_mask_pre_mode(int mode);
+int amos_mask_pre_one_pass(const amos_mask_pre *p, int *source_window_bytes);
 
 int amos_orb_detect_color_with_mask_pre_batch_device(amos_orb *h, amos_mask_pre *pre, const uint8_t *d_color,
                                                      size_t frame_stride, size_t row_stride, int width, int height,
```

Result: faster. 1664 frames/s (median of 6 runs) (+1.1%).
